# dusanerdeljan/stereo-depth

Measured on AMD Instinct MI355X. Metric: disparity maps/sec (stereo pairs/sec) at 1242x375 D=128, higher is better.
Workload: dtype f32

## Files before the change

### stereo-depth_amd/csrc/k_match_capture.h

```cpp
#pragma once
#include "k_capture_pixel0.h"
#include "k_match_fast.h"

namespace smx {

#ifndef SMX_CAP_TH
#define SMX_CAP_TH 24
#endif
constexpr int CAP_TH = SMX_CAP_TH;
constexpr int CAP_TH_SMALL = 8;

template <int TH, int PR, int PK16>
__global__ __launch_bounds__(64 * FA_WAVES, SMX_FA_OCC) void k_match_capture(MatchParams p) {
    constexpr int WGCOLS = FA_WGCOLS;
    constexpr int ND = PR - WGCOLS + 1;
    const BlockIdx3 blk = xcd_block_index();
    const int b = blk.z;
    if (p.gate == 1 && p.flags[b] == p.epoch) return;
    if (p.gate == 2 && p.flags[b] != p.epoch) return;

    extern __shared__ __attribute__((aligned(16))) unsigned short fsmem[];
    unsigned short *Lt = fsmem;
    unsigned short *Rt = fsmem + (TH + 22) * FA_PL;
    unsigned *bits = (unsigned *)(Rt + (TH + 22) * PR);
    const int BW = fast_bitwords(p.Dd);

    const int tid = threadIdx.x, lane = tid & 63, wv = tid >> 6;
    const int h = p.h, w = p.w, Dd = p.Dd;
    const int cwg0 = blk.x * FA_WAVES * FA_VALID;
    const int cw0 = cwg0 + wv * FA_VALID;
    const int wcol = wv * FA_VALID;
    const bool active = cw0 < w;
    const int x0 = blk.y * TH;
    const int col = cw0 - FA_HALO + lane;
    const float *Lp = p.Ld + (size_t)b * h * w;
    const float *Rp = p.Rd + (size_t)b * h * w;
    const float unit = p.unit;

    FastLane ln;
    ln.xch = (float *)(bits + FA_WAVES * BW) + wv * FA_XCH_FLOATS;
    ln.c255 = (unsigned)(255.0f * unit);
    ln.inv = 1.0f / (unit * unit * unit);
    ln.store_ok = active && lane >= FA_HALO && lane < FA_HALO + FA_VALID && col < w;
    ln.rows_ok = min(TH, h - x0);
    ln.plane = (size_t)p.B * h * w;
    ln.row0 = ((size_t)b * h + x0) * w;
    ln.colidx = ln.store_ok ? col : 0;
    ln.lptr = Lt + wcol + lane;

    fast_stage<(WGCOLS + 63) / 64, FA_WAVES>(Lt, FA_PL, Lp, h, w, x0 - FA_HALO, cwg0 - FA_HALO, TH + 22, WGCOLS, unit, wv, lane);
    for (int e = tid; e < FA_WAVES * BW; e += 64 * FA_WAVES) bits[e] = 0u;
    __syncthreads();

    unsigned upk[(TH + 1) / 2], vpk[(TH + 1) / 2];
#pragma unroll
    for (int o = 0; o < (TH + 1) / 2; ++o) { upk[o] = 0u; vpk[o] = 0u; }
    const bool all_needed = Dd > FA_BITWORDS * 32;
    unsigned *wbits = bits + wv * BW;
    const int left_ok = __builtin_amdgcn_update_dpp(0, ln.store_ok ? 1 : 0, 0x138, 0xf, 0xf, false);
#pragma unroll
    for (int o = 0; o < TH; ++o) {
        unsigned U = 0xffffu, V = 0xffffu;
        int u = -1, us = -1;
        bool has_succ = false;
        size_t pix = 0;
        if (ln.store_ok && o < ln.rows_ok) {
            pix = ln.row0 + (size_t)o * w + ln.colidx;
            u = (int)p.wta[pix];
            has_succ = (size_t)(x0 + o) * w + ln.colidx + 1 < (size_t)h * w;
            us = has_succ ? (int)p.wta[pix + 1] : -1;
        }
        const int lu = __builtin_amdgcn_update_dpp(-2, u, 0x138, 0xf, 0xf, false);
        const bool dup = left_ok && lu == u && us == u;
        if (ln.store_ok && o < ln.rows_ok) {
            U = (unsigned)u;
            if (has_succ) V = (unsigned)(2 * Dd - us);
            if (!all_needed && !dup) {
#pragma unroll
                for (int dl = -1; dl <= 1; ++dl) {
                    const int t = u + dl;
                    if (t <= Dd) { const int i = t == Dd ? 0 : t; atomicOr(&wbits[i], 1u << o); }
                    const int ts = us + dl;
                    if (has_succ && ts > Dd && ts <= 2 * Dd) { const int i = 2 * Dd - ts; atomicOr(&wbits[i], 1u << o); }
                }
            }
        }
        upk[o >> 1] |= U << (16 * (o & 1));
        vpk[o >> 1] |= V << (16 * (o & 1));
    }

    auto stage_right = [&](int d0, int nd) {
        __syncthreads();
        const int cbase = cwg0 - FA_HALO - (p.dmin + d0 + nd - 1);
        fast_stage<(PR + 63) / 64, FA_WAVES>(Rt, PR, Rp, h, w, x0 - FA_HALO, cbase, TH + 22, WGCOLS + nd - 1, unit, wv, lane);
        __syncthreads();
    };

    float best[TH];
    int arg[TH];
    for (int d0 = 0; d0 < Dd; d0 += ND) {
        const int nd = min(ND, Dd - d0);
        stage_right(d0, nd);
        if (active) {
            const unsigned *mybits = bits + wv * BW;
            auto march = [&](int dda, int ddb, unsigned rows) {
                const int ia = d0 + dda, ib = d0 + ddb;
                ln.rptr = Rt + wcol + lane + (nd - 1 - dda);
                fast_pass_pair<TH, PR, false, PK16, 2>(p, ln, ia, false, best, arg, Rt + wcol + lane + (nd - 1 - ddb), ib, upk,
                                                       ia == 0 ? Dd : -0x40000000, 0, 0, 0, vpk, nullptr, rows);
            };
            int pend = -1;
            unsigned pend_rows = 0u;
            SMX_FOR_EACH_NEEDED(mybits + d0, 0, nd, all_needed, lane, dd, rows, {
                if (pend < 0) { pend = dd; pend_rows = rows; }
                else { march(pend, dd, pend_rows | rows); pend = -1; }
            })
            if (pend >= 0) march(pend, pend, pend_rows);
        }
    }
    if (blk.x == 0 && blk.y == 0) {
        __syncthreads();
        capture_pixel0_body(p, b, (float *)fsmem, 64 * FA_WAVES);
    }
}

#ifdef SMX_TU_CAPTURE
template <int TH, int PR>
inline void launch_match_capture_t(int pk, const MatchParams &p, int n, hipStream_t s) {
    const dim3 grid((p.w + FA_VALID * FA_WAVES - 1) / (FA_VALID * FA_WAVES), (p.h + TH - 1) / TH, n), block(64 * FA_WAVES);
    const size_t lds = fast_lds_bytes<PR>(TH, p.Dd, false);
    if (pk == 2) hipLaunchKernelGGL((k_match_capture<TH, PR, 2>), grid, block, lds, s, p);
    else if (pk == 1) hipLaunchKernelGGL((k_match_capture<TH, PR, 1>), grid, block, lds, s, p);
    else hipLaunchKernelGGL((k_match_capture<TH, PR, 0>), grid, block, lds, s, p);
}

inline void launch_match_capture(const FastCaptureLaunch &cl, const MatchParams &p, int n, hipStream_t s) {
    if (cl.small) {
        if (!cl.wide) launch_match_capture_t<CAP_TH_SMALL, 256>(cl.pk, p, n, s);
        else launch_match_capture_t<CAP_TH_SMALL, 320>(cl.pk, p, n, s);
    } else {
        if (!cl.wide) launch_match_capture_t<CAP_TH, 256>(cl.pk, p, n, s);
        else launch_match_capture_t<CAP_TH, 320>(cl.pk, p, n, s);
    }
}

#endif

inline bool capture_applicable(int dmin, int Dd) { return dmin > 0 && dmin <= Dd && dmin + Dd < 0xfff0; }

}
```

### stereo-depth_amd/csrc/k_match_fast.h

```cpp
#pragma once
#include "smx_common.h"

namespace smx {

constexpr int FA_HALO = 11;
constexpr int FA_VALID = 64 - 2 * FA_HALO;
#ifndef SMX_FA_WAVES
#define SMX_FA_WAVES 4
#endif
constexpr int FA_WAVES = SMX_FA_WAVES;
#ifndef SMX_FA_DS_WAVES
#define SMX_FA_DS_WAVES 8
#endif
constexpr int FA_DS_WAVES = SMX_FA_DS_WAVES;
#ifndef SMX_FA_TH
#define SMX_FA_TH 24
#endif
constexpr int FA_TH = SMX_FA_TH;
#ifndef SMX_FA_TH_SMALL
#define SMX_FA_TH_SMALL 8
#endif
constexpr int FA_TH_SMALL = SMX_FA_TH_SMALL;
constexpr int FA_TH_SMALL_TALL = 12;
constexpr int FA_TH_SMALL_MID = 10;
#ifndef SMX_FA_PF
#define SMX_FA_PF 2
#endif
constexpr int FA_PF = SMX_FA_PF;
#ifndef SMX_FA_SB_PERIOD
#define SMX_FA_SB_PERIOD 2
#endif
#ifndef SMX_FA_OCC
#define SMX_FA_OCC 3
#endif
#ifndef SMX_FA_DS_OCC
#define SMX_FA_DS_OCC 4
#endif
constexpr int FA_WGCOLS = FA_VALID * FA_WAVES + 2 * FA_HALO;
#ifndef SMX_FA_WIDE_FROM
#define SMX_FA_WIDE_FROM (256 - FA_WGCOLS + 1)
#endif
constexpr int FA_WIDE_FROM = SMX_FA_WIDE_FROM;
constexpr int FA_MID_PITCH = 288;
#ifdef SMX_FA_NO_MID_PITCH
constexpr int FA_MID_UPTO = 0;
#else
constexpr int FA_MID_UPTO = FA_MID_PITCH - FA_WGCOLS + 1;
#endif
constexpr int FA_PL = (FA_VALID * FA_WAVES + 2 * FA_HALO + 7) & ~7;
constexpr int FA_BITWORDS = 64;
__host__ __device__ inline int fast_bitwords(int Dd) {
    return Dd > FA_BITWORDS * 32 ? 2 : ((Dd + 1) & ~1);
}
#define SMX_FOR_EACH_NEEDED(tbl, lo, hi, all_needed, lane, dd, rows, BODY)                                      \
    for (int g_ = (lo); g_ < (hi); g_ += 64) {                                                                  \
        const int idx_ = g_ + (lane);                                                                           \
        unsigned word_ = 0u;                                                                                    \
        if (idx_ < (hi)) word_ = (all_needed) ? ~0u : (tbl)[idx_];                                              \
        unsigned long long m_ = __ballot(word_ != 0u);                                                          \
        while (m_ != 0ull) {                                                                                    \
            const int k_ = __builtin_ctzll(m_);                                                                 \
            m_ &= m_ - 1ull;                                                                                    \
            const int dd = g_ + k_;                                                                             \
            const unsigned rows = (unsigned)__builtin_amdgcn_readlane((int)word_, k_);                          \
            BODY                                                                                                \
        }                                                                                                       \
    }

constexpr int FA_DENSE_MAX_TH = 27;
constexpr int FA_XROW = 64 + 12;
#ifndef SMX_FA_XCH_ROWS
#define SMX_FA_XCH_ROWS 2
#endif
constexpr int FA_XCH_ROWS = SMX_FA_XCH_ROWS;
constexpr int FA_XCH_FLOATS = 2 * FA_XCH_ROWS * FA_XROW;

__host__ __device__ constexpr int fast_merge_rows(int th) { return th > 8 ? (th + 1) / 2 : th; }

__host__ __device__ constexpr bool fast_prefix_exact(int th, int k_max) {
    return (long long)(th + 11) * 48195 * k_max * k_max < (1LL << 24);
}
__host__ __device__ constexpr bool fast_prefix_form(int th, int pr, bool p1only, bool dsplit, int pk16, bool argb, bool dense) {
#ifdef SMX_FA_NO_PREFIX
    return false;
#else
    if (pk16 != 2 || !fast_prefix_exact(th, 2)) return false;
    if (dsplit) return th == FA_TH_SMALL_TALL;
    (void)pr; (void)p1only; (void)argb; (void)dense;
    return true;
#endif
}

template <int PR> inline size_t fast_lds_bytes(int th, int Dd, bool dsplit = false) {
    const size_t nw = dsplit ? FA_DS_WAVES : FA_WAVES;
    return (size_t)(th + 22) * (FA_PL + PR) * sizeof(unsigned short) + nw * fast_bitwords(Dd) * sizeof(unsigned) +
           nw * FA_XCH_FLOATS * sizeof(float) + (dsplit ? nw * fast_merge_rows(th) * 64 * 2 * sizeof(float) : 0);
}

__device__ __forceinline__ float dpp_shr1(float v) {
    return __int_as_float(__builtin_amdgcn_update_dpp(0, __float_as_int(v), 0x138, 0xf, 0xf, true));
}
__device__ __forceinline__ float dpp_shl1(float v) {
    return __int_as_float(__builtin_amdgcn_update_dpp(0, __float_as_int(v), 0x130, 0xf, 0xf, true));
}
__device__ __forceinline__ unsigned dppu_sum3(unsigned v) {
    unsigned t = (unsigned)__builtin_amdgcn_update_dpp(0, (int)v, 0x138, 0xf, 0xf, true) + v;
    asm("" : "+v"(t));
    return t + (unsigned)__builtin_amdgcn_update_dpp(0, (int)v, 0x130, 0xf, 0xf, true);
}

__device__ __forceinline__ void store_u32off(float *base_uniform, unsigned off_elems, float v) {
    *(float *)((char *)base_uniform + (size_t)(off_elems * 4u)) = v;
}

__device__ __forceinline__ void atomic_or_u32off(unsigned *base_uniform, unsigned off_words, unsigned bits) {
    atomicOr((unsigned *)((char *)base_uniform + (size_t)(off_words * 4u)), bits);
}

template <int NK, int NW, bool ROUND = false>
__device__ __forceinline__ void fast_stage(unsigned short *tile, int pitch, const float *img, int h, int w,
                                           int row0, int col0, int rows, int cols, float unit, int wv, int lane) {
    int cidx[NK];
    {
        int c = wrapi(col0 + lane, w);
        const int cstep = 64 % w;
#pragma unroll
        for (int k = 0; k < NK; ++k) {
            cidx[k] = c;
            c += cstep;
            c = c >= w ? c - w : c;
        }
    }
    int ra = wrapi(row0 + wv, h);
    const int rstep = (2 * NW) % h, rhalf = NW % h;
    for (int r = wv; r < rows; r += 2 * NW) {
        const int r2 = r + NW;
        int rb = ra + rhalf;
        rb = rb >= h ? rb - h : rb;
        const float *src = img + (size_t)ra * w;
        const float *src2 = img + (size_t)(r2 < rows ? rb : ra) * w;
        float v[NK], v2[NK];
#pragma unroll
        for (int k = 0; k < NK; ++k) {
            const bool in = lane + 64 * k < cols;
            v[k] = in ? src[cidx[k]] : 0.f;
            v2[k] = in ? src2[cidx[k]] : 0.f;
        }
        unsigned short *dst = tile + r * pitch, *dst2 = tile + r2 * pitch;
#pragma unroll
        for (int k = 0; k < NK; ++k) {
            if (lane + 64 * k < cols) {
                dst[lane + 64 * k] = (unsigned short)(ROUND ? unit * v[k] + 0.5f : unit * v[k]);
                if (r2 < rows) dst2[lane + 64 * k] = (unsigned short)(ROUND ? unit * v2[k] + 0.5f : unit * v2[k]);
            }
        }
        ra += rstep;
        ra = ra >= h ? ra - h : ra;
    }
}

struct FastLane {
    const unsigned short *lptr, *rptr;
    float *xch;
    unsigned c255;
    float inv;
    bool store_ok;
    int rows_ok;
    int colidx;
    size_t row0;
    size_t plane;
    unsigned *cand;
    unsigned cand_off_a, cand_off_b;
    unsigned long long cand_mask_a, cand_mask_b;
    unsigned cand_rstride;
    int x0;
};

typedef float f32x2 __attribute__((ext_vector_type(2)));
typedef __attribute__((address_space(3))) f32x2 fa_lds_f32x2;

__device__ __forceinline__ void argb_update(int kbyte, int &word, float m, float best, int dsel) {
    if (kbyte == 0)
        asm volatile("v_cmp_gt_f32 vcc, %1, %2\n\tv_cndmask_b32_sdwa %0, %0, %3, vcc dst_sel:BYTE_0 dst_unused:UNUSED_PRESERVE src0_sel:BYTE_0 src1_sel:BYTE_0"
                     : "+v"(word) : "v"(m), "v"(best), "v"(dsel) : "vcc");
    else if (kbyte == 1)
        asm volatile("v_cmp_gt_f32 vcc, %1, %2\n\tv_cndmask_b32_sdwa %0, %0, %3, vcc dst_sel:BYTE_1 dst_unused:UNUSED_PRESERVE src0_sel:BYTE_1 src1_sel:BYTE_0"
                     : "+v"(word) : "v"(m), "v"(best), "v"(dsel) : "vcc");
    else if (kbyte == 2)
        asm volatile("v_cmp_gt_f32 vcc, %1, %2\n\tv_cndmask_b32_sdwa %0, %0, %3, vcc dst_sel:BYTE_2 dst_unused:UNUSED_PRESERVE src0_sel:BYTE_2 src1_sel:BYTE_0"
                     : "+v"(word) : "v"(m), "v"(best), "v"(dsel) : "vcc");
    else
        asm volatile("v_cmp_gt_f32 vcc, %1, %2\n\tv_cndmask_b32_sdwa %0, %0, %3, vcc dst_sel:BYTE_3 dst_unused:UNUSED_PRESERVE src0_sel:BYTE_3 src1_sel:BYTE_0"
                     : "+v"(word) : "v"(m), "v"(best), "v"(dsel) : "vcc");
}

template <int TH, int PR, bool P1ONLY, int PK16, int MODE = 0, bool ARGB = false, bool DENSE = false, bool PREFIX = false>
__device__ __forceinline__ void fast_pass_pair(const MatchParams &p, const FastLane &ln, int d,
                                               bool valid_b, float (&best)[TH], int (&arg)[TH],
                                               const unsigned short *rptr_b_in = nullptr, int db = 0,
                                               const unsigned *argpk = nullptr, int am_a = 0, int ap_a = 0,
                                               int am_b = 0, int ap_b = 0, const unsigned *vpk = nullptr,
                                               unsigned *hits = nullptr, unsigned rowmask = ~0u,
                                               float *dmb = nullptr, float *dma = nullptr, float *dcp = nullptr,
                                               float *dfirst = nullptr) {
    static_assert(!PREFIX || (PK16 == 2 && fast_prefix_exact(TH, 2)), "prefix form: K <= 2 and every prefix below 2^24");
    constexpr int NQ = TH + 20;
    constexpr int Q9 = PREFIX ? 11 : 12, Q21 = PREFIX ? 17 : 18;
    f32x2 s1 = {0.f, 0.f}, s2 = {0.f, 0.f};
    unsigned k1 = 0u, k2 = 0u;
    const unsigned c255pk = ln.c255 * 0x10001u;
    f32x2 r3[NQ], r9[NQ], r21[NQ];
    unsigned lv[TH + 22], rva[TH + 22], rvb[TH + 22];
    f32x2 vs = {0.f, 0.f}, cs = {0.f, 0.f}, hs = {0.f, 0.f};
    f32x2 t_m3 = {0.f, 0.f}, t_p3 = {0.f, 0.f}, u_m6 = {0.f, 0.f}, u_p6 = {0.f, 0.f};
    const int lane_ = threadIdx.x & 63;
#ifdef SMX_FA_ARGMAX2
    int dva = d, dvb = d + 1;
    if (ARGB && MODE == 0) asm volatile("" : "+v"(dva), "+v"(dvb));
#endif
    const unsigned short *rptr_b = (MODE == 0 || MODE == 3) ? ln.rptr - (valid_b ? 1 : 0) : rptr_b_in;
    (void)db;
#pragma unroll
    for (int rr_ = 0; rr_ < TH + 22 + FA_PF; ++rr_) {
        if (rr_ < TH + 22) {
            lv[rr_] = ln.lptr[rr_ * FA_PL];
            rva[rr_] = ln.rptr[rr_ * PR];
            rvb[rr_] = rptr_b[rr_ * PR];
        }
        if (rr_ >= FA_PF) {
            const int r = rr_ - FA_PF;
            f32x2 s0 = {0.f, 0.f};
            unsigned k0 = 0u;
            if (PK16) {
                const unsigned sa = __builtin_amdgcn_sad_u16(lv[r], rva[r], 0u);
                const unsigned sb = __builtin_amdgcn_sad_u16(lv[r], rvb[r], 0u);
                k0 = c255pk - ((sb << 16) | sa);
            } else {
                s0.x = (float)(ln.c255 - __builtin_amdgcn_sad_u16(lv[r], rva[r], 0u));
                s0.y = (float)(ln.c255 - __builtin_amdgcn_sad_u16(lv[r], rvb[r], 0u));
            }
            if (r >= 2) {
                const int q = r - 2;
                f32x2 x3;
                if (PK16 == 2) {
                    const unsigned v3 = (k2 + k1) + k0;
                    const unsigned cv = dppu_sum3(v3);
                    const unsigned y3 = dppu_sum3(cv);
                    x3.x = (float)(y3 & 0xffffu);
                    x3.y = (float)(y3 >> 16);
                } else if (PK16 == 1) {
                    const unsigned v3 = (k2 + k1) + k0;
                    const unsigned cvp = dppu_sum3(v3);
                    f32x2 cv;
                    cv.x = (float)(cvp & 0xffffu);
                    cv.y = (float)(cvp >> 16);
                    x3.x = (dpp_shr1(cv.x) + cv.x) + dpp_shl1(cv.x);
                    x3.y = (dpp_shr1(cv.y) + cv.y) + dpp_shl1(cv.y);
                } else {
                    const f32x2 v3 = (s2 + s1) + s0;
                    f32x2 cv;
                    cv.x = (dpp_shr1(v3.x) + v3.x) + dpp_shl1(v3.x);
                    cv.y = (dpp_shr1(v3.y) + v3.y) + dpp_shl1(v3.y);
                    x3.x = (dpp_shr1(cv.x) + cv.x) + dpp_shl1(cv.x);
                    x3.y = (dpp_shr1(cv.y) + cv.y) + dpp_shl1(cv.y);
                }
                if (PREFIX && q > 0) r3[q] = r3[q > 0 ? q - 1 : 0] + x3;
                else r3[q] = x3;
                if (q >= Q9) r9[q - 6] = (t_m3 + r3[q - 6]) + t_p3;
                if (q >= Q21) r21[q - 9] = (u_m6 + u_p6) + r3[q - 9];
#ifdef SMX_EXP_NOXCH
                if (q >= Q9 - 1 && q + 1 < NQ) { t_m3 = r3[q - 5]; t_p3 = r3[q - 4]; }
                if (q >= Q21 - 1 && q + 1 < NQ) { u_m6 = r9[q - 8]; u_p6 = r9[q - 7]; }
#else
                if (q >= Q9 - 1 && q + 1 < NQ) {
                    f32x2 *x3b = (f32x2 *)ln.xch + lane_;
                    x3b[6] = r3[q - 5];
                    __builtin_amdgcn_wave_barrier();
                    {
                        const volatile fa_lds_f32x2 *xr = (const volatile fa_lds_f32x2 *)x3b;
                        t_m3 = xr[3]; t_p3 = xr[9];
                    }
                }
                if (q >= Q21 - 1 && q + 1 < NQ) {
                    f32x2 *x9b = (f32x2 *)(ln.xch + (FA_XCH_ROWS > 1 ? 2 * FA_XROW : 0)) + lane_;
                    x9b[6] = r9[q - 8];
                    __builtin_amdgcn_wave_barrier();
                    {
                        const volatile fa_lds_f32x2 *xr = (const volatile fa_lds_f32x2 *)x9b;
                        u_m6 = xr[0]; u_p6 = xr[12];
                    }
                }
#endif
                if (PREFIX) {
                    if (q >= 20) {
                        vs = q >= 21 ? r3[q] - r3[q - 21] : r3[q];
                        cs = r9[q - 6] - r9[q - 15];
                        hs = r21[q - 9] - r21[q - 12];
                    }
                } else {
                    vs += r3[q];
                    if (q >= 21) vs -= r3[q - 21];
                    if (q >= 12) cs += r9[q - 6];
                    if (q >= 21) cs -= r9[q - 15];
                    if (q >= 18) hs += r21[q - 9];
                    if (q >= 21) hs -= r21[q - 12];
                }
                if (q >= 20) {
                    const int o = q - 20;
                    const f32x2 agg = (hs * vs) * cs;
                    if ((MODE == 1 || MODE == 2) && !((rowmask >> o) & 1u)) {
                    } else if (MODE == 2) {
                        unsigned upk_w = argpk[o >> 1], vpk_w = vpk[o >> 1];
                        asm volatile("" : "+v"(upk_w), "+v"(vpk_w));
                        const unsigned U = (upk_w >> (16 * (o & 1))) & 0xffffu;
                        const unsigned V = (vpk_w >> (16 * (o & 1))) & 0xffffu;
                        int ci = ln.colidx;
                        asm volatile("" : "+v"(ci));
                        const unsigned off = (unsigned)(o * p.w + ci);
                        float *cp = p.costs + ln.row0;
                        auto put = [&](unsigned dl1, unsigned o2, float v) {
                            const size_t pl = dl1 == 1u ? 0 : (dl1 == 2u ? 1 : 2);
                            cp[pl * ln.plane + o2] = v * ln.inv;
                        };
                        const unsigned a1 = (unsigned)(d + 1) - U, a2 = V + 1u - (unsigned)d, a3 = (unsigned)(am_a + 1) - U;
                        const unsigned b1 = (unsigned)(db + 1) - U, b2 = V + 1u - (unsigned)db;
                        if (a1 < 3u) put(a1, off, agg.x);
                        if (a2 < 3u) put(a2, off + 1u, agg.x);
                        if (a3 < 3u) put(a3, off, agg.x);
                        if (b1 < 3u) put(b1, off, agg.y);
                        if (b2 < 3u) put(b2, off + 1u, agg.y);
                    } else if (MODE == 4) {
                        best[o] = __builtin_fmaxf(__builtin_fmaxf(best[o], agg.x), agg.y);
                    } else if (MODE == 3) {
                        const bool okp = ln.store_ok && o < ln.rows_ok;
                        const unsigned long long ma = __ballot(okp && agg.x >= best[o]);
                        const unsigned long long mb = __ballot(okp && agg.y >= best[o]);
                        const unsigned tr = (unsigned)(((ln.x0 + o) >> 4) - (ln.x0 >> 4));
                        const unsigned h4 = ((ma & ln.cand_mask_a) != 0ull ? 1u : 0u) | ((ma & ln.cand_mask_b) != 0ull ? 2u : 0u) |
                                            ((mb & ln.cand_mask_a) != 0ull ? 4u : 0u) | ((mb & ln.cand_mask_b) != 0ull ? 8u : 0u);
                        *hits |= h4 << (4u * tr);
                    } else if (MODE == 1) {
                        const int a = (int)((argpk[o >> 1] >> (16 * (o & 1))) & 0xffffu);
                        int ci = ln.colidx;
                        asm volatile("" : "+v"(ci));
                        const unsigned off = (unsigned)(o * p.w + ci);
                        const bool xa = a == am_a, xb = a == ap_a;
                        if (xa || a == am_b) store_u32off(p.costs + ln.row0 + ln.plane, off, (xa ? agg.x : agg.y) * ln.inv);
                        if (xb || a == ap_b) store_u32off(p.costs + ln.row0 + 2 * ln.plane, off, (xb ? agg.x : agg.y) * ln.inv);
                    } else {
                        if constexpr (DENSE) {
                            const float after_d = valid_b ? agg.y : __builtin_nanf("");
                            dma[o] = (dma[o] != dma[o]) ? agg.x : dma[o];
                            const bool ca = (agg.x > best[o]) | (d == 0);
                            const float b1 = __builtin_fmaxf(best[o], agg.x);
                            dmb[o] = ca ? dcp[o] : dmb[o];
                            dma[o] = ca ? after_d : dma[o];
                            const bool cb = agg.y > b1;
                            dmb[o] = cb ? agg.x : dmb[o];
                            dma[o] = cb ? __builtin_nanf("") : dma[o];
                            dcp[o] = agg.y;
                            if (dfirst) dfirst[o] = agg.x;
                        }
#if !defined(SMX_FA_ARGMAX2)
                        const float m = __builtin_fmaxf(__builtin_fmaxf(best[o], agg.x), agg.y);
                        const int dsel = (agg.x == m) ? d : d + 1;
#ifndef SMX_EXP_NOARG
                        if (ARGB) {
                            argb_update(o & 3, arg[o >> 2], m, best[o], dsel);
                        } else {
                            const bool changed = m > best[o];
                            arg[o] = changed ? dsel : arg[o];
                        }
#else
                        (void)dsel;
#endif
                        best[o] = m;
#else
                        if (ARGB) {
                            argb_update(o & 3, arg[o >> 2], agg.x, best[o], dva);
                            best[o] = __builtin_fmaxf(best[o], agg.x);
                            argb_update(o & 3, arg[o >> 2], agg.y, best[o], dvb);
                            best[o] = __builtin_fmaxf(best[o], agg.y);
                        } else {
                            const float m = __builtin_fmaxf(__builtin_fmaxf(best[o], agg.x), agg.y);
                            const int dsel = (agg.x == m) ? d : d + 1;
                            arg[o] = m > best[o] ? dsel : arg[o];
                            best[o] = m;
                        }
#endif
                    }
                }
            }
            s2 = s1;
            s1 = s0;
            k2 = k1;
            k1 = k0;
        }
        if ((rr_ % SMX_FA_SB_PERIOD) == SMX_FA_SB_PERIOD - 1)
            __builtin_amdgcn_sched_barrier(0);
    }
}

constexpr int FA_STAT_WG_STRIDE_DS = 16;
template <bool DSPLIT>
__device__ __forceinline__ void fast_stats_report(const MatchParams &p, int b, int wg_lin, int wv, int marches, bool window) {
    if (!p.fast_stats || b % p.fast_stride != 0) return;
    if (DSPLIT && wg_lin % FA_STAT_WG_STRIDE_DS != 0) return;
    const bool win = window && (!DSPLIT || wv == 0);
    const unsigned long long v = ((unsigned long long)(unsigned)marches << 24) | (win ? 1ull : 0ull);
    if (v != 0ull) (void)__hip_atomic_fetch_add(p.fast_stats, v, __ATOMIC_RELAXED, __HIP_MEMORY_SCOPE_AGENT);
}

template <int TU, int NH, int PR, int PK16, bool PREFIX, class StageRight>
__device__ __forceinline__ void fast_stacked_tail(const MatchParams &p, const BlockIdx3 &blk, const FastLane &ln, const float (&best)[TU * NH],
                                                  const int (&argb)[TU * NH], const unsigned short *Rt, unsigned *bits, int wcol, int x0,
                                                  bool active, StageRight &&stage_right) {
    constexpr int ND = PR - FA_WGCOLS + 1;
    const int lane = threadIdx.x & 63, wv = threadIdx.x >> 6;
    const int h = p.h, w = p.w, Dd = p.Dd, BW = fast_bitwords(Dd);
    const bool all_needed = Dd > FA_BITWORDS * 32;
    unsigned *wbits = bits + wv * BW;
#pragma unroll
    for (int hh = 0; hh < NH; ++hh) {
        float bh[TU];
        int ah[TU];
#pragma unroll
        for (int o = 0; o < TU; ++o) {
            bh[o] = best[hh * TU + o];
            ah[o] = (argb[(hh * TU + o) >> 2] >> (8 * ((hh * TU + o) & 3))) & 0xff;
        }
        FastLane lh = ln;
        lh.lptr = ln.lptr + hh * TU * FA_PL;
        lh.row0 = ln.row0 + (size_t)(hh * TU) * w;
        lh.rows_ok = max(0, min(TU, h - x0 - hh * TU));
        const unsigned short *Rh = Rt + hh * TU * PR;
        unsigned dup_left = 0u;
#ifndef SMX_FA_NO_DEDUP
        if (!all_needed) {
#pragma unroll
            for (int o = 0; o < TU; ++o) {
                const int la = __builtin_amdgcn_update_dpp(-1, ah[o], 0x138, 0xf, 0xf, false);
                dup_left |= (la == ah[o] ? 1u : 0u) << o;
            }
            const int left_ok = __builtin_amdgcn_update_dpp(0, lh.store_ok ? 1 : 0, 0x138, 0xf, 0xf, false);
            if (!left_ok) dup_left = 0u;
        }
#endif
        if (lh.store_ok) {
#pragma unroll
            for (int o = 0; o < TU; ++o) {
                if (o < lh.rows_ok) {
                    const unsigned off = (unsigned)(o * w + lh.colidx);
                    store_u32off(p.wta + lh.row0, off, (float)ah[o] + (float)p.dmin);
                    const bool nv = !(bh[o] > SMX_FLT_MIN);
                    store_u32off(p.costs + lh.row0, off, nv ? 0.0f : bh[o] * lh.inv);
                    if (!all_needed && !((dup_left >> o) & 1u)) {
                        const int dn = (ah[o] + 1 == Dd) ? 0 : ah[o] + 1;
                        const int dp = (ah[o] == 0) ? Dd - 1 : ah[o] - 1;
                        atomicOr(&wbits[dn], 1u << o);
                        atomicOr(&wbits[dp], 1u << o);
                    }
                }
            }
        }
        int marches2 = 0;
        unsigned argpk[(TU + 1) / 2];
#pragma unroll
        for (int o = 0; o < (TU + 1) / 2; ++o) argpk[o] = 0u;
#pragma unroll
        for (int o = 0; o < TU; ++o)
            argpk[o >> 1] |= ((lh.store_ok && o < lh.rows_ok) ? (unsigned)ah[o] : 0xffffu) << (16 * (o & 1));
        for (int d0 = 0; d0 < Dd; d0 += ND) {
            const int nd = min(ND, Dd - d0);
            if (Dd > ND) stage_right(d0, nd);
            else __syncthreads();
            if (active) {
                auto march = [&](int dda, int ddb, unsigned rows) {
                    const int da = d0 + dda, db = d0 + ddb;
                    ++marches2;
                    lh.rptr = Rh + wcol + lane + (nd - 1 - dda);
                    fast_pass_pair<TU, PR, false, PK16, 1, false, false, PREFIX>(p, lh, da, false, bh, ah, Rh + wcol + lane + (nd - 1 - ddb), db, argpk,
                                                           da == 0 ? Dd - 1 : da - 1, da + 1 == Dd ? 0 : da + 1,
                                                           db == 0 ? Dd - 1 : db - 1, db + 1 == Dd ? 0 : db + 1, nullptr, nullptr, rows);
                };
                int pend = -1;
                unsigned pend_rows = 0u;
                SMX_FOR_EACH_NEEDED(wbits + d0, 0, nd, all_needed, lane, dd, rows, {
                    if (pend < 0) { pend = dd; pend_rows = rows; }
                    else { march(pend, dd, pend_rows | rows); pend = -1; }
                })
                if (pend >= 0) march(pend, pend, pend_rows);
            }
        }
        if (lane == 0) fast_stats_report<false>(p, blk.z, (int)(blk.x + gridDim.x * blk.y), wv, marches2, active && lh.rows_ok > 0);
        if (hh + 1 < NH)
            for (int e = lane; e < BW; e += 64) wbits[e] = 0u;
    }
}

template <int TH, int PR, bool P1ONLY, bool DSPLIT, int PK16, bool ARGB = false, bool DENSE = false>
__device__ __forceinline__ void match_fast_body(const MatchParams &p, const BlockIdx3 &blk) {
    static_assert(!DENSE || !P1ONLY, "the dense form is a pass 1 with neighbours: min_disparity = 0");
    static_assert(!DENSE || !DSPLIT || !ARGB, "latency shape: one register per winner");
    constexpr int NW = DSPLIT ? FA_DS_WAVES : FA_WAVES;
    constexpr int WGCOLS = DSPLIT ? 64 : FA_WGCOLS;
    constexpr int ND = PR - WGCOLS + 1;
    constexpr int NH = TH > 32 ? 2 : 1;
    constexpr int TU = TH / NH;
    constexpr bool PREFIX = fast_prefix_form(TH, PR, P1ONLY, DSPLIT, PK16, ARGB, DENSE);
    static_assert(NH == 1 || (TH == 2 * TU && TU <= 32 && ARGB && !DSPLIT && !DENSE && !P1ONLY),
                  "stacked bands: two unit bands, byte-packed winners, throughput shape, sparse form");
    const int b = blk.z;

    extern __shared__ __attribute__((aligned(16))) unsigned short fsmem[];
    unsigned short *Lt = fsmem;
    unsigned short *Rt = fsmem + (TH + 22) * FA_PL;
    unsigned *bits = (unsigned *)(Rt + (TH + 22) * PR);
    const int BW = fast_bitwords(p.Dd);

    const int tid = threadIdx.x;
    const int lane = tid & 63;
    const int wv = tid >> 6;
    const int h = p.h, w = p.w, Dd = p.Dd;
    const int cwg0 = blk.x * (DSPLIT ? 1 : FA_WAVES) * FA_VALID;
    const int cw0 = cwg0 + (DSPLIT ? 0 : wv * FA_VALID);
    const int wcol = DSPLIT ? 0 : wv * FA_VALID;
    const bool active = cw0 < w;
    const int x0 = blk.y * TH;
    const int col = cw0 - FA_HALO + lane;
    const float *Lp = p.Ld + (size_t)b * h * w;
    const float *Rp = p.Rd + (size_t)b * h * w;
    const float unit = p.unit;

    FastLane ln;
    ln.xch = (float *)(bits + NW * BW) + wv * FA_XCH_FLOATS;
    ln.c255 = (unsigned)(255.0f * unit);
    ln.inv = 1.0f / (unit * unit * unit);
    ln.store_ok = active && lane >= FA_HALO && lane < FA_HALO + FA_VALID && col < w;
    ln.rows_ok = min(TH, h - x0);
    ln.plane = (size_t)p.B * h * w;
    ln.row0 = ((size_t)b * h + x0) * w;
    ln.colidx = ln.store_ok ? col : 0;
    ln.lptr = Lt + wcol + lane;

    float best[TH];
    int arg[TH];
#pragma unroll
    for (int o = 0; o < TH; ++o) { best[o] = SMX_FLT_MIN; arg[o] = 0; }
    float dmb[DENSE ? TH : 1], dma[DENSE ? TH : 1], dcp[DENSE ? TH : 1];
    float dfirst[DENSE && DSPLIT ? TH : 1];
#pragma unroll
    for (int o = 0; o < (DENSE ? TH : 1); ++o) { dmb[o] = 0.f; dma[o] = 0.f; dcp[o] = 0.f; }
#pragma unroll
    for (int o = 0; o < (DENSE && DSPLIT ? TH : 1); ++o) dfirst[o] = 0.f;

    fast_stage<(WGCOLS + 63) / 64, NW>(Lt, FA_PL, Lp, h, w, x0 - FA_HALO, cwg0 - FA_HALO, TH + 22, WGCOLS, unit, wv, lane);
    for (int e = tid; e < NW * BW; e += 64 * NW) bits[e] = 0u;

    auto stage_right = [&](int d0, int nd) {
        __syncthreads();
        const int cbase = cwg0 - FA_HALO - (p.dmin + d0 + nd - 1);
        fast_stage<(PR + 63) / 64, NW>(Rt, PR, Rp, h, w, x0 - FA_HALO, cbase, TH + 22, WGCOLS + nd - 1, unit, wv, lane);
        __syncthreads();
    };

    for (int d0 = 0; d0 < Dd; d0 += ND) {
        const int nd = min(ND, Dd - d0);
        stage_right(d0, nd);
        if (active) {
            const int q4 = ((nd + 2 * NW - 1) / (2 * NW)) * 2;
            const int dd_lo = DSPLIT ? min(nd, wv * q4) : 0;
            const int dd_hi = DSPLIT ? min(nd, dd_lo + q4) : nd;
            for (int dd = dd_lo; dd < dd_hi; dd += 2) {
                ln.rptr = Rt + wcol + lane + (nd - 1 - dd);
                if constexpr (DENSE)
                    fast_pass_pair<TH, PR, P1ONLY, PK16, 0, ARGB, true, PREFIX>(p, ln, d0 + dd, dd + 1 < dd_hi, best, arg, nullptr, 0, nullptr,
                                                                         0, 0, 0, 0, nullptr, nullptr, ~0u, dmb, dma, dcp,
                                                                         DSPLIT && dd == dd_lo ? dfirst : nullptr);
                else
                    fast_pass_pair<TH, PR, P1ONLY, PK16, 0, ARGB, false, PREFIX>(p, ln, d0 + dd, dd + 1 < dd_hi, best, arg);
            }
        }
    }
    if constexpr (NH > 1) {
        fast_stacked_tail<TU, NH, PR, PK16, PREFIX>(p, blk, ln, best, arg, Rt, bits, wcol, x0, active, stage_right);
        return;
    }
    if (ARGB) {
        int packed[(TH + 3) / 4];
#pragma unroll
        for (int o = 0; o < (TH + 3) / 4; ++o) packed[o] = arg[o];
#pragma unroll
        for (int o = 0; o < TH; ++o) arg[o] = (packed[o >> 2] >> (8 * (o & 3))) & 0xff;
    }
    float *mrg = (float *)(bits + NW * BW) + NW * FA_XCH_FLOATS;
    if constexpr (DSPLIT && DENSE) {
        constexpr int MR = fast_merge_rows(TH), R2 = (NW * MR * 2) / (NW * 6);
        static_assert(R2 >= 1 && R2 <= NW, "merge buffer: at least one row of six values per wave");
        const int q4 = ((Dd + 2 * NW - 1) / (2 * NW)) * 2;
        const int nk = (Dd + q4 - 1) / q4;
#pragma unroll 1
        for (int o0 = 0; o0 < TH; o0 += R2) {
            __syncthreads();
#pragma unroll
            for (int o = 0; o < TH; ++o) {
                if (o >= o0 && o < o0 + R2) {
                    float *q = mrg + ((size_t)(wv * R2 + (o - o0)) * 64 + lane) * 6;
                    q[0] = best[o]; q[1] = __int_as_float(arg[o]); q[2] = dmb[o]; q[3] = dma[o]; q[4] = dfirst[o]; q[5] = dcp[o];
                }
            }
            __syncthreads();
            const int j = wv;
            if (j < R2 && o0 + j < ln.rows_ok && ln.store_ok) {
                auto M = [&](int k, int f) { return mrg[((size_t)(k * R2 + j) * 64 + lane) * 6 + f]; };
                float bb = SMX_FLT_MIN;
                int aa = 0, kw = 0;
                for (int k = 0; k < nk; ++k) {
                    const float bk = M(k, 0);
                    const bool g = bk > bb;
                    aa = g ? __float_as_int(M(k, 1)) : aa;
                    kw = g ? k : kw;
                    bb = g ? bk : bb;
                }
                float mb = M(kw, 2), ma = M(kw, 3);
                if (aa == kw * q4) mb = M(kw > 0 ? kw - 1 : nk - 1, 5);
                if (ma != ma) ma = M(kw + 1 < nk ? kw + 1 : 0, 4);
                const unsigned off = (unsigned)((o0 + j) * w + ln.colidx);
                store_u32off(p.wta + ln.row0, off, (float)aa + (float)p.dmin);
                store_u32off(p.costs + ln.row0, off, !(bb > SMX_FLT_MIN) ? 0.0f : bb * ln.inv);
                store_u32off(p.costs + ln.row0 + ln.plane, off, ma * ln.inv);
                store_u32off(p.costs + ln.row0 + 2 * ln.plane, off, mb * ln.inv);
            }
        }
        return;
    }
    if (DSPLIT) {
        constexpr int MR = fast_merge_rows(TH);
#pragma unroll
        for (int o0 = 0; o0 < TH; o0 += MR) {
            __syncthreads();
#pragma unroll
            for (int o = o0; o < o0 + MR && o < TH; ++o) {
                mrg[((wv * MR + (o - o0)) * 64 + lane) * 2] = best[o];
                mrg[((wv * MR + (o - o0)) * 64 + lane) * 2 + 1] = __int_as_float(arg[o]);
            }
            __syncthreads();
#pragma unroll
            for (int o = o0; o < o0 + MR && o < TH; ++o) {
                float bb = SMX_FLT_MIN;
                int aa = 0;
#pragma unroll
                for (int k = 0; k < NW; ++k) {
                    const float bk = mrg[((k * MR + (o - o0)) * 64 + lane) * 2];
                    const int ak = __float_as_int(mrg[((k * MR + (o - o0)) * 64 + lane) * 2 + 1]);
                    const bool g = bk > bb;
                    aa = g ? ak : aa;
                    bb = g ? bk : bb;
                }
                best[o] = bb;
                arg[o] = aa;
            }
        }
    }

    const bool all_needed = Dd > FA_BITWORDS * 32;
    unsigned dup_left = 0u;
#ifndef SMX_FA_NO_DEDUP
    if (!DENSE && !P1ONLY && !all_needed) {
#pragma unroll
        for (int o = 0; o < TH; ++o) {
            const int la = __builtin_amdgcn_update_dpp(-1, arg[o], 0x138, 0xf, 0xf, false);
            dup_left |= (la == arg[o] ? 1u : 0u) << o;
        }
        const int left_ok = __builtin_amdgcn_update_dpp(0, ln.store_ok ? 1 : 0, 0x138, 0xf, 0xf, false);
        if (!left_ok) dup_left = 0u;
    }
#endif
    if (ln.store_ok) {
        unsigned *wbits = bits + (DSPLIT ? 0 : wv) * BW;
#pragma unroll
        for (int o = 0; o < TH; ++o) {
            if (o < ln.rows_ok && (!DSPLIT || o % NW == wv)) {
                const unsigned off = (unsigned)(o * w + ln.colidx);
                store_u32off(p.wta + ln.row0, off, (float)arg[o] + (float)p.dmin);
                const bool nv = !(best[o] > SMX_FLT_MIN);
                store_u32off(p.costs + ln.row0, off, nv ? 0.0f : best[o] * ln.inv);
                if constexpr (DENSE) {
                    store_u32off(p.costs + ln.row0 + 2 * ln.plane, off, (arg[o] == 0 ? dcp[o] : dmb[o]) * ln.inv);
                    if (dma[o] != dma[o]) {
                        if (!all_needed) atomicOr(&wbits[0], 1u << o);
                    } else {
                        store_u32off(p.costs + ln.row0 + ln.plane, off, dma[o] * ln.inv);
                    }
                } else
                if (!P1ONLY && !all_needed && !((dup_left >> o) & 1u)) {
                    const int dn = (arg[o] + 1 == Dd) ? 0 : arg[o] + 1;
                    const int dp = (arg[o] == 0) ? Dd - 1 : arg[o] - 1;
                    atomicOr(&wbits[dn], 1u << o);
                    atomicOr(&wbits[dp], 1u << o);
                }
            }
        }
    }
    if (P1ONLY) return;

    int marches2 = 0;
    unsigned argpk[(TH + 1) / 2];
#pragma unroll
    for (int o = 0; o < (TH + 1) / 2; ++o) argpk[o] = 0u;
#pragma unroll
    for (int o = 0; o < TH; ++o)
        argpk[o >> 1] |= ((ln.store_ok && o < ln.rows_ok) ? (unsigned)arg[o] : 0xffffu) << (16 * (o & 1));
    for (int d0 = 0; d0 < (DENSE ? 1 : Dd); d0 += ND) {
        const int nd = min(ND, Dd - d0);
        if (Dd > ND) stage_right(d0, nd);
        else __syncthreads();
        if (active) {
            const unsigned *mybits = bits + (DSPLIT ? 0 : wv) * BW;
            const int q4 = ((nd + 2 * NW - 1) / (2 * NW)) * 2;
            const int dd_lo = DSPLIT ? min(nd, wv * q4) : 0;
            const int dd_hi = DSPLIT ? min(nd, dd_lo + q4) : nd;
            auto march = [&](int dda, int ddb, unsigned rows) {
                const int da = d0 + dda, db = d0 + ddb;
                ++marches2;
                ln.rptr = Rt + wcol + lane + (nd - 1 - dda);
                fast_pass_pair<TH, PR, false, PK16, 1, false, false, PREFIX>(p, ln, da, false, best, arg, Rt + wcol + lane + (nd - 1 - ddb), db, argpk,
                                                       da == 0 ? Dd - 1 : da - 1, da + 1 == Dd ? 0 : da + 1,
                                                       db == 0 ? Dd - 1 : db - 1, db + 1 == Dd ? 0 : db + 1, nullptr, nullptr, rows);
            };
            int pend = -1;
            unsigned pend_rows = 0u;
#ifndef SMX_EXP_NOPASS2
            if constexpr (DSPLIT) {
                (void)dd_lo; (void)dd_hi;
                int seen = 0;
                SMX_FOR_EACH_NEEDED(mybits + d0, 0, nd, all_needed, lane, dd, rows, {
                    const bool mine = (seen >> 1) % NW == wv;
                    ++seen;
                    if (mine) {
                        if (pend < 0) { pend = dd; pend_rows = rows; }
                        else { march(pend, dd, pend_rows | rows); pend = -1; }
                    }
                })
            } else {
                SMX_FOR_EACH_NEEDED(mybits + d0, dd_lo, dd_hi, all_needed, lane, dd, rows, {
                    if (pend < 0) { pend = dd; pend_rows = rows; }
                    else { march(pend, dd, pend_rows | rows); pend = -1; }
                })
            }
#endif
            if (pend >= 0) march(pend, pend, pend_rows);
        }
    }
    if constexpr (!DENSE) {
        if (lane == 0) fast_stats_report<DSPLIT>(p, b, (int)(blk.x + gridDim.x * blk.y), wv, marches2, active);
    }
}

#ifdef SMX_FA_NUM_VGPR
#define SMX_FA_VGPR_ATTR __attribute__((amdgpu_num_vgpr(SMX_FA_NUM_VGPR)))
#else
#define SMX_FA_VGPR_ATTR
#endif
template <int TH, int PR, bool P1ONLY, bool DSPLIT, int PK16, bool ARGB, bool DENSE = false>
__global__ __launch_bounds__(64 * (DSPLIT ? FA_DS_WAVES : FA_WAVES), DENSE ? 2 : (DSPLIT ? (TH >= FA_TH_SMALL_TALL ? 2 : SMX_FA_DS_OCC) : SMX_FA_OCC)) SMX_FA_VGPR_ATTR void k_match_fast(MatchParams p) {
    const BlockIdx3 blk = xcd_block_index();
    if ((p.gate == 1 && p.flags[blk.z] == p.epoch) || (p.gate == 2 && p.flags[blk.z] != p.epoch)) {
        return;
    }
    match_fast_body<TH, PR, P1ONLY, DSPLIT, PK16, ARGB, DENSE>(p, blk);
}

inline int fast_pk(int unit) { return unit <= 4 ? 2 : (unit <= 16 ? 1 : 0); }
inline bool fast_small_wide(int Dd) { return Dd > 256 - 64 + 1; }

template <int TH, int PR, bool P1ONLY, bool DSPLIT, bool ARGB, bool DENSE>
inline void launch_match_fast_k(int pk, dim3 grid, dim3 block, size_t lds, const MatchParams &p, hipStream_t s) {
    if (pk == 2) hipLaunchKernelGGL((k_match_fast<TH, PR, P1ONLY, DSPLIT, 2, ARGB, DENSE>), grid, block, lds, s, p);
    else if (pk == 1) hipLaunchKernelGGL((k_match_fast<TH, PR, P1ONLY, DSPLIT, 1, ARGB, DENSE>), grid, block, lds, s, p);
    else hipLaunchKernelGGL((k_match_fast<TH, PR, P1ONLY, DSPLIT, 0, ARGB, DENSE>), grid, block, lds, s, p);
}

template <int TH, int PR, bool DSPLIT, bool ARGB>
inline void launch_match_fast_a(const FastLaunch &fl, const MatchParams &p, int n, hipStream_t s) {
    const int win_per_wg = DSPLIT ? 1 : FA_WAVES;
    const dim3 grid((p.w + FA_VALID * win_per_wg - 1) / (FA_VALID * win_per_wg), (p.h + TH - 1) / TH, n);
    const size_t lds = fast_lds_bytes<PR>(TH, p.Dd, DSPLIT);
    const dim3 block(64 * (DSPLIT ? FA_DS_WAVES : FA_WAVES));
#ifdef SMX_FA_FORCE_TH
    if (lds > 64 * 1024) {
        (void)hipFuncSetAttribute(reinterpret_cast<const void *>(&k_match_fast<TH, PR, false, DSPLIT, 2, ARGB>),
                                  hipFuncAttributeMaxDynamicSharedMemorySize, (int)lds);
    }
#endif
    if (fl.form == FAST_DENSE_SMALL) {
        if constexpr (DSPLIT && TH == FA_TH_SMALL_TALL) launch_match_fast_k<TH, PR, false, true, false, true>(fl.pk, grid, block, lds, p, s);
    } else if (fl.form == FAST_DENSE) {
        if constexpr (!DSPLIT && ARGB && TH <= FA_DENSE_MAX_TH) launch_match_fast_k<TH, PR, false, false, ARGB, true>(fl.pk, grid, block, lds, p, s);
    } else if (fl.form == FAST_PASS1_ONLY) {
        launch_match_fast_k<TH, PR, true, DSPLIT, ARGB, false>(fl.pk, grid, block, lds, p, s);
    } else {
        launch_match_fast_k<TH, PR, false, DSPLIT, ARGB, false>(fl.pk, grid, block, lds, p, s);
    }
}

template <int TH, int PR, bool DSPLIT>
inline void launch_match_fast_t(const FastLaunch &fl, const MatchParams &p, int n, hipStream_t s) {
    if constexpr (DSPLIT) {
        launch_match_fast_a<TH, PR, true, false>(fl, p, n, s);
    } else if constexpr (PR == 256 || PR == FA_MID_PITCH) {
        launch_match_fast_a<TH, PR, false, true>(fl, p, n, s);
    } else {
        if (fl.argb) launch_match_fast_a<TH, PR, false, true>(fl, p, n, s);
        else launch_match_fast_a<TH, PR, false, false>(fl, p, n, s);
    }
}

__host__ __device__ constexpr int fast_tall_pitch(int Dd) { return Dd <= FA_WIDE_FROM ? 256 : (Dd <= FA_MID_UPTO ? FA_MID_PITCH : 320); }

template <int TH>
inline void launch_match_fast_tall(const FastLaunch &fl, const MatchParams &p, int n, hipStream_t s) {
    if (fl.pitch == 256) launch_match_fast_t<TH, 256, false>(fl, p, n, s);
    else if (fl.pitch == FA_MID_PITCH) launch_match_fast_t<TH, FA_MID_PITCH, false>(fl, p, n, s);
    else launch_match_fast_t<TH, 320, false>(fl, p, n, s);
}

constexpr int FA_STACK = 2;
constexpr int FA_STACK_TH = FA_STACK * FA_TH;
template <int PR> inline bool fast_stack_fits(int Dd) {
    const size_t granule = 1280, lds = fast_lds_bytes<PR>(FA_STACK_TH, Dd);
    return 2 * ((lds + granule - 1) / granule * granule) <= 160 * 1024;
}
inline bool fast_stack_instantiated(int pitch, int Dd) { return pitch == 256 && fast_stack_fits<256>(Dd); }

template <int PR>
inline void launch_match_fast_stacked(const FastLaunch &fl, const MatchParams &p, int n, hipStream_t s) {
    const dim3 grid((p.w + FA_VALID * FA_WAVES - 1) / (FA_VALID * FA_WAVES), (p.h + FA_STACK_TH - 1) / FA_STACK_TH, n);
    const size_t lds = fast_lds_bytes<PR>(FA_STACK_TH, p.Dd);
    const dim3 block(64 * FA_WAVES);
    if (fl.pk == 2) hipLaunchKernelGGL((k_match_fast<FA_STACK_TH, PR, false, false, 2, true, false>), grid, block, lds, s, p);
    else if (fl.pk == 1) hipLaunchKernelGGL((k_match_fast<FA_STACK_TH, PR, false, false, 1, true, false>), grid, block, lds, s, p);
    else hipLaunchKernelGGL((k_match_fast<FA_STACK_TH, PR, false, false, 0, true, false>), grid, block, lds, s, p);
}
template <int PR>
inline hipError_t fast_stacked_raise_lds_caps() {
    const int cap = (int)fast_lds_bytes<PR>(FA_STACK_TH, PR - FA_WGCOLS + 1);
    const void *kernels[3] = {reinterpret_cast<const void *>(&k_match_fast<FA_STACK_TH, PR, false, false, 2, true, false>),
                              reinterpret_cast<const void *>(&k_match_fast<FA_STACK_TH, PR, false, false, 1, true, false>),
                              reinterpret_cast<const void *>(&k_match_fast<FA_STACK_TH, PR, false, false, 0, true, false>)};
    for (const void *k : kernels)
        if (hipError_t e = hipFuncSetAttribute(k, hipFuncAttributeMaxDynamicSharedMemorySize, cap); e != hipSuccess) return e;
    return hipSuccess;
}

struct FastPlan {
    bool small;
    int th;
    bool wide;
    int stack = 1;
};

inline FastPlan match_fast_plan(const MatchParams &p, int n, int cus, int stack_opt = -1) {
    FastPlan pl{};
    const long wgs_tall = (long)((p.w + FA_VALID * FA_WAVES - 1) / (FA_VALID * FA_WAVES)) * ((p.h + FA_TH - 1) / FA_TH) * n;
    pl.small = 8 * wgs_tall < (p.on_lanes ? 8L : 13L) * cus;
    if (pl.small) {
        pl.th = FA_TH_SMALL;
        pl.wide = fast_small_wide(p.Dd);
        const long windows = (long)((p.w + FA_VALID - 1) / FA_VALID) * n;
        const long wg_small = windows * ((p.h + FA_TH_SMALL - 1) / FA_TH_SMALL), wg_tall = windows * ((p.h + FA_TH_SMALL_TALL - 1) / FA_TH_SMALL_TALL);
        if (wg_small > cus && wg_tall <= cus) {
            pl.th = FA_TH_SMALL_TALL;
#ifndef SMX_FA_NO_MID
#ifdef SMX_FA_MID_P1
        } else {
#else
        } else if (!p.pass1_only) {
#endif
            const long wg_mid = windows * ((p.h + FA_TH_SMALL_MID - 1) / FA_TH_SMALL_MID), slots = 2L * cus;
            const long r_small = (wg_small + slots - 1) / slots, r_mid = (wg_mid + slots - 1) / slots;
            if (r_mid * (FA_TH_SMALL_MID + 22) < r_small * (FA_TH_SMALL + 22)) pl.th = FA_TH_SMALL_MID;
#endif
        }
        return pl;
    }
    pl.wide = p.Dd > FA_WIDE_FROM;
    const int cand[3] = {24, 27, 32};
    int best = 24;
    long best_rows = -1;
    for (int th : cand) {
        const int pr = fast_tall_pitch(p.Dd);
        const size_t lds = pr == 256 ? fast_lds_bytes<256>(th, p.Dd) : (pr == FA_MID_PITCH ? fast_lds_bytes<FA_MID_PITCH>(th, p.Dd) : fast_lds_bytes<320>(th, p.Dd));
        const size_t granule = 1280;
        const bool three_per_cu = 3 * ((lds + granule - 1) / granule * granule) <= 160 * 1024;
        const long rows = (long)((p.h + th - 1) / th) * (th + 22) * (th == 32 ? 106 : 100) * (three_per_cu ? 100 : 130);
        if (best_rows < 0 || rows < best_rows) { best_rows = rows; best = th; }
    }
    pl.th = best;
#ifdef SMX_FA_FORCE_TH
    pl.th = SMX_FA_FORCE_TH;
#endif
    if (stack_opt != 0 && !p.dense && !p.pass1_only && fast_stack_instantiated(fast_tall_pitch(p.Dd), p.Dd)) {
        const long rows_stack = (long)((p.h + FA_STACK_TH - 1) / FA_STACK_TH) * (FA_STACK_TH + 22);
        if (stack_opt == 1 || (p.on_lanes && rows_stack < (long)((p.h + pl.th - 1) / pl.th) * (pl.th + 22))) {
            pl.th = FA_TH;
            pl.stack = FA_STACK;
        }
    }
    return pl;
}

}
```

### stereo-depth_amd/csrc/k_prologue.h

```cpp
#pragma once
#include "smx_common.h"

namespace smx {

enum { IN_GRAY_F32 = 0, IN_RGB_F32 = 1, IN_GRAY_U8 = 2, IN_RGB_U8 = 3 };

template <int MODE>
__device__ __forceinline__ float load_gray(const void *img, size_t plane, size_t idx, int fp_conv) {
    if (MODE == IN_RGB_F32 || MODE == IN_RGB_U8) {
        float r, g, b;
        if (MODE == IN_RGB_F32) {
            const float *p = (const float *)img;
            r = p[idx]; g = p[plane + idx]; b = p[2 * plane + idx];
        } else {
            const uint8_t *p = (const uint8_t *)img;
            r = (float)p[idx]; g = (float)p[plane + idx]; b = (float)p[2 * plane + idx];
        }
        if (fp_conv != 0) return sum3_products(0.2989f, r, 0.5870f, g, 0.1140f, b, fp_conv);
        float R = 0.2989f * r;
        float G = 0.5870f * g;
        float B = 0.1140f * b;
        return (R + G) + B;
    } else if (MODE == IN_GRAY_U8) {
        return (float)((const uint8_t *)img)[idx];
    } else {
        return ((const float *)img)[idx];
    }
}

template <int MODE>
__global__ __launch_bounds__(256) void k_prologue(const void *left, const void *right,
                                                  float *gray_l, float *gray_r,
                                                  float *down_l, float *down_r, int *flags,
                                                  uint8_t *g8_l, uint8_t *g8_r, int *flags2,
                                                  int H, int W, int K, int h, int w, int grid_capable,
                                                  int pitch8, int padl, int padr, int epoch,
                                                  int gpitch, int gpadl, int fp_conv) {
    const int y = blockIdx.x * 64 + threadIdx.x;
    const int x = blockIdx.y * 4 + threadIdx.y;
    const int b = blockIdx.z;
    const size_t plane = (size_t)H * W;
    const size_t in_elems = (MODE == IN_RGB_F32 || MODE == IN_RGB_U8) ? 3 * plane : plane;
    const size_t in_bytes = (MODE == IN_GRAY_U8 || MODE == IN_RGB_U8) ? 1 : 4;
    bool bad = (grid_capable == 0);
    bool bad8 = false;
    if (x < h && y < w) {
        const float area = (float)(K * K);
        const float unit = area;
#pragma unroll
        for (int side = 0; side < 2; ++side) {
            const char *base = (const char *)(side ? right : left) + (size_t)b * in_elems * in_bytes;
            float *gout = (side ? gray_r : gray_l);
            uint8_t *g8 = (side ? g8_r : g8_l);
            float sum = 0.0f;
            uint32_t pk = 0u;
            for (int i = 0; i < K; ++i) {
                int xi = x * K + i;
                const bool xin = xi < H;
                if (!xin) xi = H - 1;
                for (int j = 0; j < K; ++j) {
                    int yj = y * K + j;
                    const bool yin = yj < W;
                    if (!yin) yj = W - 1;
                    const size_t idx = (size_t)xi * W + yj;
                    const float v = load_gray<MODE>(base, plane, idx, fp_conv);
                    if (MODE == IN_RGB_F32) bad8 = bad8 || !(v >= 0.0f && v <= 255.0f);
                    if (MODE != IN_GRAY_F32 && xin && yin) {
                        float *grow = gout + ((size_t)b * H + xi) * gpitch + gpadl;
                        grow[yj] = v;
                        if (gpadl > 0) {
                            if (yj >= W - gpadl) grow[yj - W] = v;
                            if (yj < padr) grow[W + yj] = v;
                        }
                    }
                    if ((MODE == IN_GRAY_F32 || MODE == IN_GRAY_U8) && pitch8 > 0 && xin && yin) {
                        if (MODE == IN_GRAY_F32) bad8 = bad8 || !(v == rintf(v) && v >= 0.0f && v <= 255.0f);
                        uint8_t *row8 = g8 + ((size_t)b * H + xi) * pitch8;
                        if (K == 2) {
                            if (j == 0) pk = (uint32_t)(uint8_t)v;
                            else if (yj & 1) *(uint16_t *)(row8 + padl + yj - 1) = (uint16_t)(pk | ((uint32_t)(uint8_t)v << 8));
                            if (j == 0 && yj + 1 >= W) row8[padl + yj] = (uint8_t)v;
                        } else {
                            row8[padl + yj] = (uint8_t)v;
                        }
                        if (yj >= W - padl) row8[yj - (W - padl)] = (uint8_t)v;
                        if (yj < padr) row8[padl + W + yj] = (uint8_t)v;
                    }
                    sum += v;
                }
            }
            const float pooled = grid_capable ? sum * (1.0f / area) : sum / area;
            (side ? down_r : down_l)[((size_t)b * h + x) * w + y] = pooled;
            const float s = pooled * unit;
            bad = bad || !(s == rintf(s) && pooled >= 0.0f && pooled <= 255.0f);
        }
    }
    const unsigned long long m = __ballot(bad);
    if (m != 0ull && (int)threadIdx.x == __ffsll((long long)m) - 1) flags[b] = epoch;
    if (MODE == IN_GRAY_F32 || MODE == IN_RGB_F32) {
        const unsigned long long m8 = __ballot(bad8);
        if (m8 != 0ull && (int)threadIdx.x == __ffsll((long long)m8) - 1) flags2[b] = epoch;
    }
}

template <int MODE>
__global__ __launch_bounds__(256) void k_prologue_k2(const void *left, const void *right,
                                                     float *gray_l, float *gray_r,
                                                     float *down_l, float *down_r, int *flags,
                                                     uint8_t *g8_l, uint8_t *g8_r, int *flags2,
                                                     int H, int W, int h, int w,
                                                     int pitch8, int padl, int padr, int epoch,
                                                     int gpitch, int gpadl) {
    const int yp = (blockIdx.x * 64 + threadIdx.x) * 2;
    const int x = blockIdx.y * 4 + threadIdx.y;
    const int b = blockIdx.z;
    const size_t plane = (size_t)H * W;
    bool bad = false, bad8 = false;
    if (x < h && yp < w) {
        const int Y0 = yp * 2;
        const int ncol = min(4, W - Y0);
        const int x0 = x * 2, x1 = min(x * 2 + 1, H - 1);
        const bool row1_in = x * 2 + 1 < H;
#pragma unroll
        for (int side = 0; side < 2; ++side) {
            const void *img = side ? right : left;
            float v0[4], v1[4];
            if (MODE == IN_GRAY_F32) {
                const float *p0 = (const float *)img + (size_t)b * plane + (size_t)x0 * W + Y0;
                const float *p1 = (const float *)img + (size_t)b * plane + (size_t)x1 * W + Y0;
                if (ncol == 4) {
                    __builtin_memcpy(v0, __builtin_assume_aligned(p0, 4), 16);
                    __builtin_memcpy(v1, __builtin_assume_aligned(p1, 4), 16);
                } else {
                    v0[0] = p0[0]; v0[1] = p0[1]; v1[0] = p1[0]; v1[1] = p1[1];
                    v0[2] = v0[3] = v1[2] = v1[3] = 0.f;
                }
            } else {
                const uint8_t *p0 = (const uint8_t *)img + (size_t)b * plane + (size_t)x0 * W + Y0;
                const uint8_t *p1 = (const uint8_t *)img + (size_t)b * plane + (size_t)x1 * W + Y0;
#pragma unroll
                for (int j = 0; j < 4; ++j) {
                    v0[j] = (j < ncol) ? (float)p0[j] : 0.f;
                    v1[j] = (j < ncol) ? (float)p1[j] : 0.f;
                }
                float *g = (side ? gray_r : gray_l) + (size_t)b * H * gpitch + gpadl;
#pragma unroll
                for (int j = 0; j < 4; ++j) {
                    if (j < ncol) {
                        g[(size_t)x0 * gpitch + Y0 + j] = v0[j];
                        if (row1_in) g[(size_t)(x0 + 1) * gpitch + Y0 + j] = v1[j];
                    }
                }
            }
            float pooled[2];
            pooled[0] = (((v0[0] + v0[1]) + v1[0]) + v1[1]) * 0.25f;
            pooled[1] = (((v0[2] + v0[3]) + v1[2]) + v1[3]) * 0.25f;
            float *dn = (side ? down_r : down_l) + ((size_t)b * h + x) * w + yp;
            dn[0] = pooled[0];
            if (ncol == 4) dn[1] = pooled[1];
#pragma unroll
            for (int k = 0; k < 2; ++k) {
                if (k == 0 || ncol == 4) {
                    const float s4 = pooled[k] * 4.0f;
                    bad = bad || !(s4 == rintf(s4) && pooled[k] >= 0.0f && pooled[k] <= 255.0f);
                }
            }
            if (pitch8 > 0) {
                uint8_t *g8 = (side ? g8_r : g8_l);
                uint32_t w0 = 0u, w1 = 0u;
#pragma unroll
                for (int j = 0; j < 4; ++j) {
                    if (j < ncol) {
                        if (MODE == IN_GRAY_F32)
                            bad8 = bad8 || !(v0[j] == rintf(v0[j]) && v0[j] >= 0.f && v0[j] <= 255.f) ||
                                   (row1_in && !(v1[j] == rintf(v1[j]) && v1[j] >= 0.f && v1[j] <= 255.f));
                        w0 |= (uint32_t)(uint8_t)v0[j] << (8 * j);
                        w1 |= (uint32_t)(uint8_t)v1[j] << (8 * j);
                    }
                }
                uint8_t *r0 = g8 + ((size_t)b * H + x0) * pitch8, *r1 = r0 + pitch8;
                if (ncol == 4) {
                    *(uint32_t *)(r0 + padl + Y0) = w0;
                    if (row1_in) *(uint32_t *)(r1 + padl + Y0) = w1;
                } else {
                    *(uint16_t *)(r0 + padl + Y0) = (uint16_t)w0;
                    if (row1_in) *(uint16_t *)(r1 + padl + Y0) = (uint16_t)w1;
                }
                if (Y0 + 3 >= W - padl || Y0 < padr) {
#pragma unroll
                    for (int j = 0; j < 4; ++j) {
                        const int yj = Y0 + j;
                        if (j < ncol) {
                            const uint8_t a = (uint8_t)(w0 >> (8 * j)), c = (uint8_t)(w1 >> (8 * j));
                            if (yj >= W - padl) { r0[yj - (W - padl)] = a; if (row1_in) r1[yj - (W - padl)] = c; }
                            if (yj < padr) { r0[padl + W + yj] = a; if (row1_in) r1[padl + W + yj] = c; }
                        }
                    }
                }
            }
        }
    }
    const unsigned long long m = __ballot(bad);
    if (m != 0ull && (int)threadIdx.x == __ffsll((long long)m) - 1) flags[b] = epoch;
    if (MODE == IN_GRAY_F32) {
        const unsigned long long m8 = __ballot(bad8);
        if (m8 != 0ull && (int)threadIdx.x == __ffsll((long long)m8) - 1) flags2[b] = epoch;
    }
}

template <int MODE>
__global__ __launch_bounds__(256) void k_prologue_k4(const void *left, const void *right,
                                                     float *gray_l, float *gray_r,
                                                     float *down_l, float *down_r, int *flags,
                                                     uint8_t *g8_l, uint8_t *g8_r, int *flags2,
                                                     int H, int W, int h, int w,
                                                     int pitch8, int padl, int padr, int epoch,
                                                     int gpitch, int gpadl, int fp_conv) {
    constexpr bool RGB = MODE == IN_RGB_F32 || MODE == IN_RGB_U8;
    constexpr bool U8 = MODE == IN_GRAY_U8 || MODE == IN_RGB_U8;
    const int y = blockIdx.x * 64 + threadIdx.x;
    const int x = blockIdx.y * 4 + threadIdx.y;
    const int b = blockIdx.z;
    const size_t plane = (size_t)H * W;
    const size_t pair_elems = RGB ? 3 * plane : plane;
    bool bad = false, bad8 = false;
    if (x < h && y < w) {
        const int Y0 = y * 4;
#pragma unroll
        for (int side = 0; side < 2; ++side) {
            const void *img = side ? right : left;
            float v[4][4];
            bool rin[4];
#pragma unroll
            for (int i = 0; i < 4; ++i) {
                rin[i] = x * 4 + i < H;
                const int xi = rin[i] ? x * 4 + i : H - 1;
                const size_t at = (size_t)b * pair_elems + (size_t)xi * W + Y0;
                float c[RGB ? 3 : 1][4];
#pragma unroll
                for (int ch = 0; ch < (RGB ? 3 : 1); ++ch) {
                    if (!U8) {
                        const float *p = (const float *)img + at + ch * plane;
                        __builtin_memcpy(c[ch], __builtin_assume_aligned(p, 4), 16);
                    } else {
                        const uint8_t *p = (const uint8_t *)img + at + ch * plane;
                        uint32_t wd;
                        __builtin_memcpy(&wd, __builtin_assume_aligned(p, 4), 4);
#pragma unroll
                        for (int j = 0; j < 4; ++j) c[ch][j] = (float)((wd >> (8 * j)) & 0xffu);
                    }
                }
#pragma unroll
                for (int j = 0; j < 4; ++j) {
                    if (RGB) {
                        if (fp_conv != 0) {
                            v[i][j] = sum3_products(0.2989f, c[0][j], 0.5870f, c[RGB ? 1 : 0][j], 0.1140f, c[RGB ? 2 : 0][j], fp_conv);
                        } else {
                            const float R = 0.2989f * c[0][j];
                            const float G = 0.5870f * c[RGB ? 1 : 0][j];
                            const float B = 0.1140f * c[RGB ? 2 : 0][j];
                            v[i][j] = (R + G) + B;
                        }
                        if (MODE == IN_RGB_F32) bad8 = bad8 || !(v[i][j] >= 0.0f && v[i][j] <= 255.0f);
                    } else {
                        v[i][j] = c[0][j];
                    }
                }
                if (MODE != IN_GRAY_F32 && rin[i]) {
                    float *grow = (side ? gray_r : gray_l) + ((size_t)b * H + xi) * gpitch + gpadl;
                    __builtin_memcpy(__builtin_assume_aligned(grow + Y0, 16), v[i], 16);
                    if (RGB && gpadl > 0 && (Y0 + 3 >= W - gpadl || Y0 < padr)) {
#pragma unroll
                        for (int j = 0; j < 4; ++j) {
                            const int yj = Y0 + j;
                            if (yj >= W - gpadl) grow[yj - W] = v[i][j];
                            if (yj < padr) grow[W + yj] = v[i][j];
                        }
                    }
                }
            }
            float sum = 0.0f;
#pragma unroll
            for (int i = 0; i < 4; ++i) {
#pragma unroll
                for (int j = 0; j < 4; ++j) sum += v[i][j];
            }
            const float pooled = sum * 0.0625f;
            (side ? down_r : down_l)[((size_t)b * h + x) * w + y] = pooled;
            const float s16 = pooled * 16.0f;
            bad = bad || !(s16 == rintf(s16) && pooled >= 0.0f && pooled <= 255.0f);
            if (!RGB && pitch8 > 0) {
                uint8_t *g8 = (side ? g8_r : g8_l);
#pragma unroll
                for (int i = 0; i < 4; ++i) {
                    if (!rin[i]) continue;
                    uint32_t wd = 0u;
#pragma unroll
                    for (int j = 0; j < 4; ++j) {
                        if (MODE == IN_GRAY_F32) bad8 = bad8 || !(v[i][j] == rintf(v[i][j]) && v[i][j] >= 0.f && v[i][j] <= 255.f);
                        wd |= (uint32_t)(uint8_t)v[i][j] << (8 * j);
                    }
                    uint8_t *r8 = g8 + ((size_t)b * H + x * 4 + i) * pitch8;
                    *(uint32_t *)(r8 + padl + Y0) = wd;
                    if (Y0 + 3 >= W - padl || Y0 < padr) {
#pragma unroll
                        for (int j = 0; j < 4; ++j) {
                            const int yj = Y0 + j;
                            const uint8_t a = (uint8_t)(wd >> (8 * j));
                            if (yj >= W - padl) r8[yj - (W - padl)] = a;
                            if (yj < padr) r8[padl + W + yj] = a;
                        }
                    }
                }
            }
        }
    }
    const unsigned long long m = __ballot(bad);
    if (m != 0ull && (int)threadIdx.x == __ffsll((long long)m) - 1) flags[b] = epoch;
    if (MODE == IN_GRAY_F32 || MODE == IN_RGB_F32) {
        const unsigned long long m8 = __ballot(bad8);
        if (m8 != 0ull && (int)threadIdx.x == __ffsll((long long)m8) - 1) flags2[b] = epoch;
    }
}

}
```

### stereo-depth_amd/csrc/smx_common.h

```cpp
#pragma once

#include <hip/hip_runtime.h>
#include <stdint.h>

#define SMX_FLT_MIN 1.17549435e-38f

namespace smx {

__device__ __forceinline__ int wrapi(int g, int n) {
    g %= n;
    return g < 0 ? g + n : g;
}

__device__ __forceinline__ int pad_index_ref(int index, int n) {
    if (index >= 0 && index < n) return index;
    if (index < 0) return n + index;
    if (index == n) return 0;
    return n - index;
}

__device__ __forceinline__ float sum3_products(float a1, float b1, float a2, float b2, float a3, float b3, int conv) {
    float inner;
    if (conv == 1 || conv == 4) inner = __builtin_fmaf(a1, b1, a2 * b2);
    else if (conv == 2 || conv == 5) inner = __builtin_fmaf(a2, b2, a1 * b1);
    else inner = a1 * b1 + a2 * b2;
    if (conv >= 1 && conv <= 3) return __builtin_fmaf(a3, b3, inner);
    return inner + a3 * b3;
}

__device__ __forceinline__ float quadratic_peak_conv(float x1, float y1, float x2, float y2,
                                                     float x3, float y3, int conv) {
    float denominator = (x1 - x2) * (x2 - x3) * (x1 - x3);
    float min_value;
    if (y1 > y2) {
        min_value = (y1 > y3) ? x1 : x3;
    } else {
        min_value = (y2 > y3) ? x2 : x3;
    }
    if (denominator != 0) {
        const float a = sum3_products(x3, y2 - y1, x2, y1 - y3, x1, y3 - y2, conv);
        const float b = sum3_products(x1 * x1, y2 - y3, x3 * x3, y1 - y2, x2 * x2, y3 - y1, conv);
        if (a < 0) {
            min_value = -b / (2 * a);
        }
    }
    return min_value;
}

__device__ __forceinline__ float quadratic_peak(float x1, float y1, float x2, float y2,
                                                float x3, float y3) {
    float denominator = (x1 - x2) * (x2 - x3) * (x1 - x3);
    float min_value;
    if (y1 > y2) {
        min_value = (y1 > y3) ? x1 : x3;
    } else {
        min_value = (y2 > y3) ? x2 : x3;
    }
    if (denominator != 0) {
        float a = x3 * (y2 - y1) + x2 * (y1 - y3) + x1 * (y3 - y2);
        float b = x1 * x1 * (y2 - y3) + x3 * x3 * (y1 - y2) + x2 * x2 * (y3 - y1);
        if (a < 0) {
            min_value = -b / (2 * a);
        }
    }
    return min_value;
}

__device__ __forceinline__ float quadratic_peak_unit(float x1, float y1, float y2, float y3, int conv) {
    const float x2 = x1 + 1.0f, x3 = x1 - 1.0f;
    float min_value;
    if (y1 > y2) {
        min_value = (y1 > y3) ? x1 : x3;
    } else {
        min_value = (y2 > y3) ? x2 : x3;
    }
    float a, b;
    if (conv == 0) {
        a = x3 * (y2 - y1) + x2 * (y1 - y3) + x1 * (y3 - y2);
        b = x1 * x1 * (y2 - y3) + x3 * x3 * (y1 - y2) + x2 * x2 * (y3 - y1);
    } else {
        a = sum3_products(x3, y2 - y1, x2, y1 - y3, x1, y3 - y2, conv);
        b = sum3_products(x1 * x1, y2 - y3, x3 * x3, y1 - y2, x2 * x2, y3 - y1, conv);
    }
    if (a < 0) min_value = -b / (2 * a);
    return min_value;
}

struct WtaState {
    float best, m0, mb, ma, cprev, first;
    int arg;
    bool pend;
    __device__ __forceinline__ void init() {
        best = SMX_FLT_MIN; m0 = 0.f; mb = 0.f; ma = 0.f; cprev = 0.f; first = 0.f;
        arg = 0; pend = false;
    }
    __device__ __forceinline__ void step(int d, float c) {
        if (d == 0) { first = c; m0 = c; pend = true; }
        else if (pend) { ma = c; pend = false; }
        if (c > best) {
            best = c; arg = d; m0 = c; mb = cprev; pend = true;
        }
        cprev = c;
    }
    __device__ __forceinline__ void finish() {
        if (arg == 0) mb = cprev;
        if (pend) ma = first;
    }
};

struct BlockIdx3 { unsigned x, y, z; };
__device__ __forceinline__ BlockIdx3 xcd_block_index() {
    const unsigned nx = gridDim.x, ny = gridDim.y, nz = gridDim.z;
    const unsigned total = nx * ny * nz, per = total >> 3;
    const unsigned lin = blockIdx.x + nx * (blockIdx.y + ny * blockIdx.z);
    const unsigned t = lin < (per << 3) ? (lin & 7u) * per + (lin >> 3) : lin;
    BlockIdx3 b;
    b.x = t % nx;
    const unsigned q = t / nx;
    b.y = q % ny;
    b.z = q / ny;
    return b;
}

struct WtaSlice {
    float best, m0, mb, ma, cprev, first;
    int arg;
    bool pend;
    __device__ __forceinline__ void init(int lo) {
        best = SMX_FLT_MIN; m0 = 0.f; mb = 0.f; ma = 0.f; cprev = 0.f; first = 0.f;
        arg = lo; pend = false;
    }
    __device__ __forceinline__ void step(int d, int lo, float c) {
        if (d == lo) { first = c; m0 = c; pend = true; }
        else if (pend) { ma = c; pend = false; }
        if (c > best) {
            best = c; arg = d; m0 = c; mb = cprev; pend = true;
        }
        cprev = c;
    }
};

enum { SMX_SL_BEST = 0, SMX_SL_ARG, SMX_SL_M0, SMX_SL_MA, SMX_SL_MB, SMX_SL_FIRST, SMX_SL_LAST, SMX_SL_PEND, SMX_SLICE_WORDS };

struct MatchParams {
    const float *Ld, *Rd;
    float *wta;
    float *costs;
    float *vol;
    const int *flags;
    int epoch;
    int B, h, w, dmin, Dd;
    int rn, rs, rm, rl;
    int gate;
    int nd_chunk;
    float unit;
    int nsplit;
    int pairs;
    float *slices;
    int pass1_only;
    int dense;
    int dense_small;
    unsigned long long *fast_stats;
    int fast_stride;
    int on_lanes;
    unsigned *tickets;
};

enum GateFlag { GATE_GRID_FLAG = 0, GATE_RANGE_FLAG };
enum ExactKernel { EXACT_GENERIC = 0, EXACT_GENERIC_VOLUME, EXACT_TILED };
struct ExactLaunch {
    int kernel = EXACT_GENERIC;
    int split = 1;
    int rows_per_thread = 4;
    int nd_chunk = 0;
    size_t lds_bytes = 0;
    size_t slice_floats = 0;
    int gate = 0, gate_flag = GATE_GRID_FLAG;
};
struct ExactCaptureLaunch { int split = 1, rows_per_thread = 4, nd_chunk = 0; size_t lds_bytes = 0; int gate = 0; };
enum FastForm { FAST_SPARSE = 0, FAST_PASS1_ONLY, FAST_DENSE, FAST_DENSE_SMALL, FAST_FORMS };
struct FastLaunch {
    int th = 0;
    bool small = false;
    int pitch = 0;
    int pk = 0;
    bool argb = false;
    int form = FAST_SPARSE;
    int gate = 0;
    int stack = 1;
};
struct FastCaptureLaunch { bool small = false, wide = false; int pk = 0, gate = 0; };
struct AutoLaunch { int th = 0; bool wide = false; int pk = 0, nsplit = 1, nd_chunk = 0; size_t lds_bytes = 0; };
struct FilterLaunch { int th = 0; bool wide = false; int pk = 0; };
enum PrologueKernel { PROLOGUE_GENERIC = 0, PROLOGUE_K2, PROLOGUE_K4 };
struct PrologueLaunch { int in_mode = 0, kernel = PROLOGUE_GENERIC; };
enum RefineKind {
    REFINE_FLOAT = 0,
    REFINE_INT = 1,
    REFINE_INT_V = 2,
    REFINE_AUTO = 3,
    REFINE_AUTO_V = 4
};
struct RefineLaunch {
    int kind = REFINE_FLOAT;
    int kt = 0;
    bool apron = false;
    bool sad_exact = true;
};
enum FillKernel { FILL_4 = 0, FILL_POW2, FILL_GENERIC };
struct FillLaunch {
    int kernel = FILL_GENERIC, K = 1;
    int px = 8;
    int log2k = 0;
};

}
```

### stereo-depth_amd/csrc/smx_engine.hip

```cpp
#include <hip/hip_runtime.h>

#include <cstdarg>
#include <cstdio>
#include <cstdlib>
#include <cstring>
#include <mutex>
#include <new>
#include <string>
#include <vector>

#include "../../include/stereo_mi355x.h"
#include "k_fill.h"
#include "k_match_exact.h"
#include "k_match_exact2.h"
#include "k_match_auto.h"
#include "k_match_filter.h"
#include "k_match_capture.h"
#include "k_match_fast.h"
#include "k_prologue.h"
#include "k_refine.h"
#include "smx_common.h"
#include "smx_launch.h"
#include "smx_plan.h"
#include "smx_route.h"
#include "smx_status.h"

namespace {

using smx::check_lr_scalars, smx::DeviceGuard, smx::fail, smx::ranges_overlap;

int compute_dims(const smx_config *c, smx_dims *d) {
    if (c->height == 0 || c->width == 0 || c->downscale_factor == 0)
        return fail(SMX_ERR_INVALID_CONFIG, "height, width and downscale_factor must be positive");
    if (c->height > (1u << 15) || c->width > (1u << 15) || c->downscale_factor > 64)
        return fail(SMX_ERR_INVALID_CONFIG, "image larger than 32768 or downscale_factor > 64");
    if (c->min_disparity < 0 || c->max_disparity < c->min_disparity)
        return fail(SMX_ERR_INVALID_CONFIG, "need 0 <= min_disparity <= max_disparity");
    if (c->small_mbm_radius < 0 || c->mid_mbm_radius < 0 || c->large_mbm_radius < 0)
        return fail(SMX_ERR_INVALID_CONFIG, "block-matching radii must be non-negative");
    if (c->small_mbm_radius > c->large_mbm_radius || c->mid_mbm_radius > c->large_mbm_radius)
        return fail(SMX_ERR_INVALID_CONFIG,
                    "small_mbm_radius and mid_mbm_radius must not exceed large_mbm_radius "
                    "(the reference's shared tile has a halo of large_mbm_radius)");
    if (c->ncc_patch_radius > 16 || c->sad_patch_radius > 32 || c->large_mbm_radius > 32)
        return fail(SMX_ERR_INVALID_CONFIG, "patch radius out of the supported range");
    const int K = (int)c->downscale_factor;
    d->H = (int)c->height;
    d->W = (int)c->width;
    d->K = K;
    d->h = (d->H + K - 1) / K;
    d->w = (d->W + K - 1) / K;
    d->dmin = c->min_disparity / K;
    d->dmax = c->max_disparity / K;
    d->Dd = d->dmax - d->dmin + 1;
    return SMX_OK;
}

}

using smx::HostHints, smx::ContentSwitch, smx::LaneLedger;

struct smx_engine {
    smx_config cfg;
    smx_dims dm;
    int B;
    smx::EngineFacts facts;
    float *gray_l = nullptr, *gray_r = nullptr;
    float *down_l = nullptr, *down_r = nullptr;
    float *wta = nullptr, *refined = nullptr;
    float *costs = nullptr;
    float *vol = nullptr;
    float *slices = nullptr;
    unsigned *tickets = nullptr;
    int *flags = nullptr;
    int epoch = 0;
    uint8_t *gray8_l = nullptr, *gray8_r = nullptr;
    unsigned *cand = nullptr;
    struct LastCall {
        smx::CallFacts call;
        smx::RangePlan plan;
        int first = 0;
    } last_call;
    int next_small_lane = 0;
    const float *last_gray_l = nullptr, *last_gray_r = nullptr;
    int last_gpitch = 0;
    bool last_gray_owned = false;
    size_t last_gplane = 0;
    int opt_lane_priority = 1;
    bool opt_debug_hints = false;
    HostHints *hints = nullptr, *hints_dev = nullptr;
    smx::RouteState route;
    unsigned *stats_dev = nullptr;
    unsigned long long *fast_stats_dev = nullptr;
    std::vector<hipEvent_t> prof_events;
    std::vector<unsigned char> prof_used;
    int prof_calls = 0, prof_max = 0;
    bool prof_on = false;
    static constexpr int LANES = 2;
    hipStream_t lane_stream[LANES] = {};
    hipEvent_t ev_join[LANES] = {};
    hipEvent_t ev_cross[LANES] = {};
    hipEvent_t ev_caller = nullptr;
    bool caller_tail_live = false;
    bool caller_calls_unrecorded = false;
    hipStream_t last_caller_stream = nullptr;
    LaneLedger ledger;
    bool detached_pending = false;
    int overlap_min = 0;
    void *lr_in_l = nullptr, *lr_in_r = nullptr;
    size_t lr_pair_bytes = 0;
    float *lr_raw = nullptr;
};
static_assert(ContentSwitch::LANES == smx_engine::LANES && LaneLedger::LANES == smx_engine::LANES, "one report word and one ledger entry per stream lane");

namespace {

void free_events(smx_engine *e) {
    for (hipEvent_t ev : e->prof_events) (void)hipEventDestroy(ev);
    e->prof_events.clear();
    e->prof_used.clear();
    e->prof_calls = e->prof_max = 0;
    e->prof_on = false;
}

void free_buffers(smx_engine *e) {
    void *ptrs[] = {e->gray_l, e->gray_r, e->down_l, e->down_r, e->wta,     e->refined,  e->costs,
                    e->vol,    e->flags,  e->gray8_l, e->gray8_r, e->slices, e->cand,    e->stats_dev, e->tickets, e->fast_stats_dev,
                    e->lr_in_l, e->lr_in_r, e->lr_raw};
    for (void *p : ptrs)
        if (p) (void)hipFree(p);
    if (e->hints) (void)hipHostFree(e->hints);
    e->hints = e->hints_dev = nullptr;
}

struct SlotTimer {
    smx_engine *e;
    hipStream_t s;
    int lane, slot;
    bool on;
    SlotTimer(smx_engine *e_, hipStream_t s_, int lane_, int slot_) : e(e_), s(s_), lane(lane_), slot(slot_) {
        on = e->prof_on && e->prof_calls < e->prof_max;
        if (on) (void)hipEventRecord(e->prof_events[index() * 2], s);
    }
    size_t index() const { return ((size_t)e->prof_calls * smx_engine::LANES + lane) * SMX_KERNEL_SLOTS + slot; }
    ~SlotTimer() {
        if (on) {
            (void)hipEventRecord(e->prof_events[index() * 2 + 1], s);
            e->prof_used[index()] = 1;
        }
    }
};

using smx::SMX_EXACT2_LDS_CAP;
hipError_t raise_lds_caps(int device) {
    static std::mutex mu;
    static std::vector<int> done;
    std::lock_guard<std::mutex> lock(mu);
    for (int d : done)
        if (d == device) return hipSuccess;
    if (hipError_t e = smx::exact_raise_lds_caps(SMX_EXACT2_LDS_CAP + (int)((smx::E2_CAPBITS + 2 * smx::E2_SPARSE_WORDS) * sizeof(unsigned)));
        e != hipSuccess) return e;
    if (hipError_t e = smx::match_auto_raise_caps(); e != hipSuccess) return e;
    if (hipError_t e = smx::fast_stack_raise_caps(); e != hipSuccess) return e;
    done.push_back(device);
    return hipSuccess;
}

bool env_is(const char *name, char c) {
    const char *v = std::getenv(name);
    return v && v[0] == c;
}

struct PairView {
    float *gray_l, *gray_r, *down_l, *down_r, *wta, *refined, *costs, *vol;
    int *flags, *flags2;
    uint8_t *gray8_l, *gray8_r;
    unsigned *cand;
};
PairView view_from(const smx_engine *e, int first) {
    const smx_dims &d = e->dm;
    const smx::EngineFacts &ef = e->facts;
    const size_t f = (size_t)first, hw = (size_t)d.h * d.w;
    PairView v{};
    v.gray_l = e->gray_l + f * d.H * ef.gpitch;
    v.gray_r = e->gray_r + f * d.H * ef.gpitch;
    v.down_l = e->down_l + f * hw;
    v.down_r = e->down_r + f * hw;
    v.wta = e->wta + f * hw;
    v.refined = e->refined + f * hw;
    v.costs = e->costs + f * hw;
    v.vol = e->vol ? e->vol + f * hw * d.Dd : nullptr;
    v.flags = e->flags + first;
    v.flags2 = e->flags + e->B + first;
    v.gray8_l = e->gray8_l ? e->gray8_l + f * d.H * ef.pitch8 : nullptr;
    v.gray8_r = e->gray8_r ? e->gray8_r + f * d.H * ef.pitch8 : nullptr;
    v.cand = e->cand ? e->cand + f * ef.cand_tiles_x * ef.cand_tiles_y * ef.cand_cw : nullptr;
    return v;
}

int join_into(smx_engine *e, hipStream_t s) {
    for (int k = 0; k < smx_engine::LANES; ++k) {
        if (!e->lane_stream[k] || !e->ev_join[k]) continue;
        SMX_HIP(hipEventRecord(e->ev_join[k], e->lane_stream[k]));
        SMX_HIP(hipStreamWaitEvent(s, e->ev_join[k], 0));
    }
    e->detached_pending = false;
    return SMX_OK;
}

bool stream_capturing(hipStream_t s) {
    hipStreamCaptureStatus st = hipStreamCaptureStatusNone;
    if (hipStreamIsCapturing(s, &st) != hipSuccess) {
        (void)hipGetLastError();
        return false;
    }
    return st != hipStreamCaptureStatusNone;
}

void read_hints(smx_engine *e) {
    if (!e->hints) return;
    const bool was_dense = e->route.fast.on;
    if (e->route.read_hints(*e->hints) && e->opt_debug_hints)
        std::fprintf(stderr, "[smx] fast kernel: second pass / first pass = %.3f (dense %d)\n", e->route.fast.last, was_dense ? 1 : 0);
}

smx::PrologueArgs prologue_args(const smx_engine *e, const PairView &v, bool owns_gray, const void *left, const void *right) {
    const smx_dims &d = e->dm;
    const smx::EngineFacts &f = e->facts;
    smx::PrologueArgs a{};
    a.left = left; a.right = right; a.gray_l = owns_gray ? v.gray_l : nullptr; a.gray_r = owns_gray ? v.gray_r : nullptr;
    a.down_l = v.down_l; a.down_r = v.down_r;
    a.flags = v.flags; a.flags2 = v.flags2; a.g8_l = v.gray8_l; a.g8_r = v.gray8_r;
    a.H = d.H; a.W = d.W; a.K = d.K; a.h = d.h; a.w = d.w; a.grid_capable = f.grid_capable ? 1 : 0;
    a.pitch8 = f.pitch8; a.padl = f.padl; a.padr = f.padr; a.epoch = e->epoch; a.gpitch = f.gpitch; a.gpadl = f.gpadl;
    a.fp_conv = SMX_FP_STEP1(e->cfg.fp_convention);
    return a;
}
smx::RangeParams range_params(const smx_engine *e, const PairView &v, const smx::CallFacts &call, const smx::RangePlan &pl, int lane, int first) {
    const smx_dims &d = e->dm;
    const smx::EngineFacts &f = e->facts;
    smx::RangeParams b;
    smx::MatchParams &mp = b.mp;
    mp.Ld = v.down_l; mp.Rd = v.down_r; mp.wta = v.wta; mp.costs = v.costs; mp.vol = v.vol;
    mp.flags = v.flags; mp.epoch = e->epoch; mp.B = e->B; mp.h = d.h; mp.w = d.w; mp.dmin = d.dmin; mp.Dd = d.Dd;
    mp.rn = (int)e->cfg.ncc_patch_radius; mp.rs = e->cfg.small_mbm_radius;
    mp.rm = e->cfg.mid_mbm_radius; mp.rl = e->cfg.large_mbm_radius;
    mp.unit = (float)(d.K * d.K);
    mp.on_lanes = call.on_lanes ? 1 : 0;
    mp.tickets = e->tickets ? e->tickets + (size_t)first * f.e2_tiles : nullptr;
    mp.pass1_only = pl.capture_follows ? 1 : 0;
    mp.slices = e->slices ? e->slices + (size_t)lane * f.slices_floats : nullptr;
    b.range_flags = v.flags2;
    b.fast_stats = e->fast_stats_dev + lane;
    return b;
}
struct GrayView { const float *l, *r; int pitch; size_t plane; };
GrayView gray_view(smx_engine *e, const PairView &v, bool owns_gray, int first, const void *left, const void *right) {
    const smx::EngineFacts &f = e->facts;
    GrayView g{owns_gray ? v.gray_l + f.gpadl : (const float *)left, owns_gray ? v.gray_r + f.gpadl : (const float *)right,
               owns_gray ? f.gpitch : e->dm.W, 0};
    g.plane = (size_t)e->dm.H * g.pitch;
    e->last_gray_l = g.l - (size_t)first * g.plane;
    e->last_gray_r = g.r - (size_t)first * g.plane;
    e->last_gray_owned = owns_gray;
    e->last_gpitch = g.pitch;
    e->last_gplane = g.plane;
    return g;
}
smx::RefineParams refine_params(const smx_engine *e, const PairView &v, const smx::RangePlan &pl, const GrayView &g) {
    const smx_dims &d = e->dm;
    const smx::EngineFacts &f = e->facts;
    smx::RefineParams rp{};
    rp.Lg = g.l; rp.Rg = g.r; rp.gpitch = g.pitch; rp.gplane = g.plane; rp.wta = v.wta; rp.costs = v.costs; rp.vol = v.vol;
    rp.refined = v.refined; rp.B = e->B; rp.H = d.H; rp.W = d.W; rp.K = d.K; rp.h = d.h;
    rp.w = d.w; rp.Dd = d.Dd; rp.R = (int)e->cfg.sad_patch_radius;
    rp.flags2 = v.flags2;
    rp.epoch = e->epoch;
    rp.L8 = v.gray8_l; rp.R8 = v.gray8_r; rp.pitch8 = f.pitch8; rp.padl = f.padl;
    rp.fp_conv = SMX_FP_PARABOLA(e->cfg.fp_convention);
    rp.sad_exact = pl.refine.sad_exact ? 1 : 0;
    if (pl.refine.kind == smx::REFINE_AUTO) rp.grid_flags = v.flags;
    if (pl.refine_reports_grid) rp.grid_hint = &e->hints_dev->grid;
    return rp;
}
smx::FillParams fill_params(smx_engine *e, const PairView &v, const smx::RangePlan &pl, int lane, const GrayView &g, float *out) {
    const smx_dims &d = e->dm;
    smx::FillParams fp{};
    fp.Lg = g.l; fp.lpitch = g.pitch; fp.lplane = g.plane; fp.refined = v.refined; fp.out = out; fp.B = e->B; fp.H = d.H; fp.W = d.W;
    fp.K = d.K; fp.h = d.h; fp.w = d.w; fp.thr = (float)e->cfg.threshold;
    fp.log2k = pl.fill.log2k;
    if (pl.fill_publishes) {
        fp.fast_stats = e->fast_stats_dev + lane;
        fp.fast_stats_host = &e->hints_dev->fast_density[lane];
        fp.fast_seq = e->route.fast.next_seq();
        fp.fast_pass1 = (d.Dd + 1) / 2;
    }
    return fp;
}

void enqueue_exact(const smx::RangeParams &b, const smx::RangePlan &pl, int n, hipStream_t s) {
    smx::launch_exact(pl.exact, smx::exact_params(b, pl.exact, n), n, s);
    if (pl.capture_follows) smx::launch_exact2_capture(pl.exact_capture, smx::exact_capture_params(b, pl.exact_capture), n, s);
}
void enqueue_fast(const smx::RangeParams &b, const smx::RangePlan &pl, int n, hipStream_t s) {
    smx::launch_match_fast(pl.fast_launch, smx::fast_params(b, pl, pl.fast_launch.gate), n, s);
    if (pl.capture_follows) smx::launch_match_capture_tu(pl.fast_capture, smx::fast_params(b, pl, pl.fast_capture.gate), n, s);
}

int enqueue_range(smx_engine *e, const smx::CallFacts &call, const smx::RangePlan &pl, int lane, int first, int n,
                  const void *left, const void *right, float *out, hipStream_t s) {
    const smx::EngineFacts &f = e->facts;
    const PairView v = view_from(e, first);
    const GrayView g = gray_view(e, v, pl.owns_gray, first, left, right);
    {
        SlotTimer tm(e, s, lane, SMX_KERNEL_PROLOGUE);
        smx::launch_prologue(pl.prologue, prologue_args(e, v, pl.owns_gray, left, right), n, s);
    }
    if (pl.status != SMX_OK) return fail(pl.status, "%s", pl.refusal);
    if (pl.exact.slice_floats > f.slices_floats)
        return fail(SMX_ERR_HIP, "internal: slice buffer too small for the disparity split of %d pairs", n);

    const smx::RangeParams b = range_params(e, v, call, pl, lane, first);
    switch (pl.route) {
    case smx::AGG_FILTERED: {
        smx::FilterParams fp{};
        fp.cand = v.cand; fp.tiles_x = f.cand_tiles_x; fp.tiles_y = f.cand_tiles_y; fp.cw = f.cand_cw;
        fp.two_e = f.filter_two_e; fp.range_flags = v.flags2;
        {
            SlotTimer tm(e, s, lane, SMX_KERNEL_MATCH_FAST);
            if (pl.gated_dense_first) smx::launch_exact(pl.exact, smx::exact_params(b, pl.exact, n), n, s);
            smx::launch_match_filter_tu(pl.filter, smx::filter_params(b, f), fp, n, s);
        }
        SlotTimer tm(e, s, lane, SMX_KERNEL_MATCH_EXACT);
        smx::launch_exact2_sparse(smx::sparse_params(b, f), n, v.cand, f.cand_cw, (const int *)v.flags2, e->stats_dev + 2 * lane,
                                  &e->hints_dev->filter_density[lane], e->route.filt.next_seq(), s);
        if (pl.capture_follows) smx::launch_exact2_capture(pl.exact_capture, smx::exact_capture_params(b, pl.exact_capture), n, s);
        break;
    }
    case smx::AGG_EXACT: {
        SlotTimer tm(e, s, lane, SMX_KERNEL_MATCH_EXACT);
        enqueue_exact(b, pl, n, s);
        break;
    }
    case smx::AGG_FAST: {
        SlotTimer tm(e, s, lane, SMX_KERNEL_MATCH_FAST);
        enqueue_fast(b, pl, n, s);
        break;
    }
    case smx::AGG_AUTO_ONE_LAUNCH: {
        SlotTimer tm(e, s, lane, SMX_KERNEL_MATCH_FAST);
        smx::launch_match_auto_small_tu(pl.auto_launch, smx::auto_params(b, pl, n), n, s);
        break;
    }
    default: {
        {
            SlotTimer tm(e, s, lane, SMX_KERNEL_MATCH_EXACT);
            enqueue_exact(b, pl, n, s);
        }
        SlotTimer tm(e, s, lane, SMX_KERNEL_MATCH_FAST);
        enqueue_fast(b, pl, n, s);
        break;
    }
    }
    e->last_call.plan = pl;
    {
        SlotTimer tm(e, s, lane, SMX_KERNEL_REFINE);
        smx::launch_refine(pl.refine, refine_params(e, v, pl, g), n, s);
    }
    {
        SlotTimer tm(e, s, lane, SMX_KERNEL_FILL);
        smx::launch_fill(pl.fill, fill_params(e, v, pl, lane, g, out), n, s);
    }
    SMX_HIP(hipGetLastError());
    return SMX_OK;
}

struct LanePool {
    int device;
    int users;
    hipStream_t stream[smx_engine::LANES];
};
std::mutex g_lane_mu;
std::vector<LanePool> g_lane_pools;

int acquire_lane_streams(smx_engine *e) {
    std::lock_guard<std::mutex> lock(g_lane_mu);
    for (LanePool &p : g_lane_pools)
        if (p.device == e->cfg.device_id) {
            p.users++;
            for (int k = 0; k < smx_engine::LANES; ++k) e->lane_stream[k] = p.stream[k];
            return SMX_OK;
        }
    LanePool p{};
    p.device = e->cfg.device_id;
    p.users = 1;
    int prio_least = 0, prio_greatest = 0;
    (void)hipDeviceGetStreamPriorityRange(&prio_least, &prio_greatest);
    for (int k = 0; k < smx_engine::LANES; ++k) {
        const hipError_t err = (e->opt_lane_priority && prio_greatest != prio_least)
                                   ? hipStreamCreateWithPriority(&p.stream[k], hipStreamNonBlocking, prio_greatest)
                                   : hipStreamCreateWithFlags(&p.stream[k], hipStreamNonBlocking);
        if (err != hipSuccess) {
            for (int j = 0; j < k; ++j) (void)hipStreamDestroy(p.stream[j]);
            return fail(SMX_ERR_HIP, "creating the stream lanes failed: %s", hipGetErrorString(err));
        }
    }
    g_lane_pools.push_back(p);
    for (int k = 0; k < smx_engine::LANES; ++k) e->lane_stream[k] = p.stream[k];
    return SMX_OK;
}

void release_lane_streams(smx_engine *e) {
    if (!e->lane_stream[0]) return;
    std::lock_guard<std::mutex> lock(g_lane_mu);
    for (size_t i = 0; i < g_lane_pools.size(); ++i) {
        LanePool &p = g_lane_pools[i];
        if (p.device != e->cfg.device_id || p.stream[0] != e->lane_stream[0]) continue;
        if (--p.users == 0) {
            for (int k = 0; k < smx_engine::LANES; ++k) (void)hipStreamDestroy(p.stream[k]);
            g_lane_pools.erase(g_lane_pools.begin() + (long)i);
        }
        break;
    }
    for (int k = 0; k < smx_engine::LANES; ++k) e->lane_stream[k] = nullptr;
}

int create_lanes(smx_engine *e) {
    if (!e->lane_stream[0]) {
        if (int rc = acquire_lane_streams(e)) return rc;
        for (int k = 0; k < smx_engine::LANES; ++k) {
            SMX_HIP(hipEventCreateWithFlags(&e->ev_join[k], hipEventDisableTiming));
            SMX_HIP(hipEventCreateWithFlags(&e->ev_cross[k], hipEventDisableTiming));
        }
    }
    if (!e->ev_caller) SMX_HIP(hipEventCreateWithFlags(&e->ev_caller, hipEventDisableTiming));
    if (e->caller_calls_unrecorded) {
        hipStream_t last = e->last_caller_stream;
        if (stream_capturing(last))
            return fail(SMX_ERR_UNSUPPORTED, "stream capture: the stream of the engine's last call is being captured; "
                                             "the first SMX_STREAM_ENGINE call cannot be ordered behind it");
        if (hipEventRecord(e->ev_caller, last) == hipSuccess) {
            e->caller_tail_live = true;
        } else {
            (void)hipGetLastError();
            SMX_HIP(hipDeviceSynchronize());
        }
        e->caller_calls_unrecorded = false;
    }
    return SMX_OK;
}

int enqueue(smx_engine *e, int in_mode, int n, const void *left, const void *right, float *out, void *stream) {
    if (!e) return fail(SMX_ERR_INVALID_ARG, "engine is NULL");
    if (!left || !right || !out) return fail(SMX_ERR_INVALID_ARG, "left, right and out must be non-NULL");
    if (n < 1 || n > e->B)
        return fail(SMX_ERR_INVALID_ARG, "batch size %d outside [1, max_batch=%d]", n, e->B);
    DeviceGuard guard(e->cfg.device_id);
    if (!guard.ok) return fail(SMX_ERR_HIP, "cannot select HIP device %d", e->cfg.device_id);
    const smx_dims &d = e->dm;
    const bool detached = stream == SMX_STREAM_ENGINE;
    const bool capturing = !detached && stream_capturing((hipStream_t)stream);
    if (capturing && (e->detached_pending || e->epoch == 0x7fffffff))
        return fail(SMX_ERR_UNSUPPORTED,
                    "stream capture: the engine has work on its own streams that is not joined yet (call smx_join on a "
                    "stream outside the capture first), or its call counter is about to wrap");
    if (detached) {
        if (int rc = create_lanes(e)) return rc;
        if (e->caller_tail_live) {
            for (int k = 0; k < smx_engine::LANES; ++k) SMX_HIP(hipStreamWaitEvent(e->lane_stream[k], e->ev_caller, 0));
            e->caller_tail_live = false;
        }
    } else if (e->detached_pending) {
        if (int rc = join_into(e, (hipStream_t)stream)) return rc;
    }
    if (e->epoch == 0x7fffffff) {
        e->epoch = 0;
        SMX_HIP(hipDeviceSynchronize());
        SMX_HIP(hipMemsetAsync(e->flags, 0, sizeof(int) * 2 * (size_t)e->B, nullptr));
        SMX_HIP(hipStreamSynchronize(nullptr));
    }
    e->epoch++;
    read_hints(e);
    const smx::EngineFacts &f = e->facts;
    const bool split = detached && e->overlap_min > 0 && n >= e->overlap_min;
    const int n0 = split ? (n + 1) / 2 : n;
    smx::CallFacts call;
    call.in_mode = in_mode;
    call.on_lanes = detached;
    call.u8_aligned = (((uintptr_t)left | (uintptr_t)right) & 3u) == 0;
    call.route = e->route.decide_call(smx::call_kind(f, in_mode, detached, n0, n - n0), f.opt.fast_dense, f.exact_filter);
    e->last_call.call = call;
    e->last_call.first = 0;
    const size_t out_pair_bytes = (size_t)d.H * d.W * sizeof(float);
    auto lane_enter = [&](int k, int lo, int hi, const float *out_first, int pairs) -> int {
        const uintptr_t olo = (uintptr_t)out_first, ohi = olo + (size_t)pairs * out_pair_bytes;
        if (e->ledger.enter(k, lo, hi, olo, ohi)) {
            const int o = 1 - k;
            SMX_HIP(hipEventRecord(e->ev_cross[o], e->lane_stream[o]));
            SMX_HIP(hipStreamWaitEvent(e->lane_stream[k], e->ev_cross[o], 0));
        }
        return SMX_OK;
    };
    int rc;
    if (split) {
        const bool rgb = in_mode == smx::IN_RGB_F32 || in_mode == smx::IN_RGB_U8;
        const bool u8 = in_mode == smx::IN_GRAY_U8 || in_mode == smx::IN_RGB_U8;
        const size_t in_pair = (size_t)d.H * d.W * (rgb ? 3 : 1) * (u8 ? 1 : sizeof(float));
        if (int lrc = lane_enter(1, n0, n, out + (size_t)n0 * d.H * d.W, n - n0)) return lrc;
        rc = enqueue_range(e, call, smx::plan_range(f, call, n - n0, false), 1, n0, n - n0, (const char *)left + n0 * in_pair,
                           (const char *)right + n0 * in_pair, out + (size_t)n0 * d.H * d.W, e->lane_stream[1]);
        if (rc == SMX_OK) rc = lane_enter(0, 0, n0, out, n0);
        if (rc == SMX_OK) rc = enqueue_range(e, call, smx::plan_range(f, call, n0, false), 0, 0, n0, left, right, out, e->lane_stream[0]);
    } else {
        int lane = 0, first = 0;
        if (detached && 2 * n <= e->B) {
            lane = e->next_small_lane;
            e->next_small_lane ^= 1;
            first = lane * (e->B / 2);
        }
        e->last_call.first = first;
        if (detached)
            if (int lrc = lane_enter(lane, first, first + n, out, n)) return lrc;
        rc = enqueue_range(e, call, smx::plan_range(f, call, n, true), lane, first, n, left, right, out,
                           detached ? e->lane_stream[lane] : (hipStream_t)stream);
        if (!detached && !capturing) {
            if (e->ev_caller) {
                SMX_HIP(hipEventRecord(e->ev_caller, (hipStream_t)stream));
                e->caller_tail_live = true;
            } else {
                e->caller_calls_unrecorded = true;
                e->last_caller_stream = (hipStream_t)stream;
            }
        }
    }
    if (detached) e->detached_pending = true;
    if (e->prof_on && e->prof_calls < e->prof_max) e->prof_calls++;
    return rc;
}

int enqueue_lr(smx_engine *e, int in_mode, int n, const void *left, const void *right, float *out, float *right_out,
               float max_diff, float invalid, void *stream) {
    if (int rc = check_lr_scalars(max_diff, invalid)) return rc;
    if (!e) return fail(SMX_ERR_INVALID_ARG, "engine is NULL");
    if (!left || !right || !out) return fail(SMX_ERR_INVALID_ARG, "left, right and out must be non-NULL");
    if (n < 1 || 2L * n > e->B)
        return fail(SMX_ERR_INVALID_ARG,
                    "LR batch size %d: the check runs the mirrored problem too, i.e. 2n = %ld internal pairs, which must "
                    "lie in [2, max_batch=%d] (n <= max_batch / 2)", n, 2L * n, e->B);
    if (stream == SMX_STREAM_ENGINE)
        return fail(SMX_ERR_UNSUPPORTED, "LR calls run on a caller's stream only (SMX_STREAM_ENGINE is not supported)");
    const smx_dims &d = e->dm;
    const bool rgb = in_mode == smx::IN_RGB_F32 || in_mode == smx::IN_RGB_U8;
    const bool u8 = in_mode == smx::IN_GRAY_U8 || in_mode == smx::IN_RGB_U8;
    const int planes = rgb ? 3 : 1, es = u8 ? 1 : (int)sizeof(float);
    const size_t hw = (size_t)d.H * d.W, pair_bytes = hw * planes * es;
    const size_t in_bytes = (size_t)n * pair_bytes, out_bytes = (size_t)n * hw * sizeof(float);
    if (ranges_overlap(left, in_bytes, out, out_bytes) || ranges_overlap(right, in_bytes, out, out_bytes) ||
        ranges_overlap(left, in_bytes, right_out, out_bytes) || ranges_overlap(right, in_bytes, right_out, out_bytes) ||
        ranges_overlap(out, out_bytes, right_out, out_bytes))
        return fail(SMX_ERR_INVALID_ARG, "LR call: the inputs, out and right_out must not overlap");
    DeviceGuard guard(e->cfg.device_id);
    if (!guard.ok) return fail(SMX_ERR_HIP, "cannot select HIP device %d", e->cfg.device_id);
    hipStream_t s = (hipStream_t)stream;
    const bool capturing = stream_capturing(s);
    if (!e->lr_raw || e->lr_pair_bytes < pair_bytes) {
        if (capturing)
            return fail(SMX_ERR_UNSUPPORTED, "stream capture: the LR scratch of this input format is not allocated yet "
                                             "(make one LR call outside capture first)");
        if (e->lr_pair_bytes < pair_bytes) {
            if (e->lr_in_l || e->lr_in_r) {
                SMX_HIP(hipDeviceSynchronize());
                (void)hipFree(e->lr_in_l);
                (void)hipFree(e->lr_in_r);
                e->lr_in_l = e->lr_in_r = nullptr;
                e->lr_pair_bytes = 0;
            }
            SMX_HIP(hipMalloc(&e->lr_in_l, (size_t)e->B * pair_bytes));
            SMX_HIP(hipMalloc(&e->lr_in_r, (size_t)e->B * pair_bytes));
            e->lr_pair_bytes = pair_bytes;
        }
        if (!e->lr_raw) SMX_HIP(hipMalloc((void **)&e->lr_raw, (size_t)e->B * hw * sizeof(float)));
    }
    if (capturing && (e->detached_pending || e->epoch == 0x7fffffff))
        return fail(SMX_ERR_UNSUPPORTED,
                    "stream capture: the engine has work on its own streams that is not joined yet (call smx_join on a "
                    "stream outside the capture first), or its call counter is about to wrap");
    smx::launch_lr_pack(es, left, right, e->lr_in_l, e->lr_in_r, (long)n * planes * d.H, d.W, s);
    SMX_HIP(hipGetLastError());
    if (int rc = enqueue(e, in_mode, 2 * n, e->lr_in_l, e->lr_in_r, e->lr_raw, stream)) return rc;
    smx::launch_lr_check(true, e->lr_raw, e->lr_raw + (size_t)n * hw, out, right_out, n, d.H, d.W, max_diff, invalid, s);
    SMX_HIP(hipGetLastError());
    return SMX_OK;
}

}

static thread_local std::string g_last_error;

int smx::fail(int code, const char *fmt, ...) {
    char buf[512];
    va_list ap;
    va_start(ap, fmt);
    vsnprintf(buf, sizeof(buf), fmt, ap);
    va_end(ap);
    g_last_error = buf;
    return code;
}

extern "C" {

int smx_abi_version(void) { return SMX_ABI_VERSION; }

const char *smx_last_error(void) { return g_last_error.c_str(); }

void smx_config_default(smx_config *cfg) {
    if (!cfg) return;
    std::memset(cfg, 0, sizeof(*cfg));
    cfg->height = 1080;
    cfg->width = 1920;
    cfg->downscale_factor = 2;
    cfg->min_disparity = 75;
    cfg->max_disparity = 262;
    cfg->ncc_patch_radius = 1;
    cfg->sad_patch_radius = 5;
    cfg->threshold = 5;
    cfg->small_mbm_radius = 1;
    cfg->mid_mbm_radius = 4;
    cfg->large_mbm_radius = 10;
    cfg->device_id = 0;
    cfg->max_batch = 1;
    cfg->match_mode = SMX_MATCH_AUTO;
}

int smx_get_dims(const smx_config *cfg, smx_dims *dims) {
    if (!cfg || !dims) return fail(SMX_ERR_INVALID_ARG, "cfg and dims must be non-NULL");
    return compute_dims(cfg, dims);
}

static int overlap_min_pairs_default(const smx::EngineFacts &f) {
    const char *v = std::getenv("SMX_OVERLAP_MIN_PAIRS");
    if (v && *v) {
        const int k = std::atoi(v);
        return k < 0 ? 0 : (k == 1 ? 2 : k);
    }
    int n_tall = 1;
    while (n_tall < 4096 && smx::range_fast_plan(f, false, n_tall).small) ++n_tall;
    return 2 * n_tall;
}

static void destroy_lanes(smx_engine *e) {
    for (int k = 0; k < smx_engine::LANES; ++k) {
        if (e->ev_join[k]) (void)hipEventDestroy(e->ev_join[k]);
        if (e->ev_cross[k]) (void)hipEventDestroy(e->ev_cross[k]);
        e->ev_join[k] = e->ev_cross[k] = nullptr;
    }
    release_lane_streams(e);
    if (e->ev_caller) (void)hipEventDestroy(e->ev_caller);
    e->ev_caller = nullptr;
}

int smx_create(const smx_config *cfg, smx_engine **out_engine) {
    if (!cfg || !out_engine) return fail(SMX_ERR_INVALID_ARG, "cfg and out_engine must be non-NULL");
    *out_engine = nullptr;
    smx_dims d;
    int rc = compute_dims(cfg, &d);
    if (rc) return rc;
    if (cfg->match_mode < SMX_MATCH_AUTO || cfg->match_mode > SMX_MATCH_FAST_GRID)
        return fail(SMX_ERR_INVALID_CONFIG, "unknown match_mode %d", cfg->match_mode);
    if (!SMX_FP_VALID(cfg->fp_convention))
        return fail(SMX_ERR_INVALID_CONFIG, "unknown fp_convention %d (smx_fp_convention: 0 .. %d, or SMX_FP_MIXED of two)",
                    cfg->fp_convention, SMX_FP_CONVENTIONS - 1);
    for (int v : cfg->reserved)
        if (v != 0) return fail(SMX_ERR_INVALID_CONFIG, "reserved fields must be 0");
    int ndev = 0;
    SMX_HIP(hipGetDeviceCount(&ndev));
    if (ndev <= 0)
        return fail(SMX_ERR_HIP, "no HIP device visible: libstereo_mi355x has no CPU fallback");
    if (cfg->device_id < 0 || cfg->device_id >= ndev)
        return fail(SMX_ERR_INVALID_CONFIG, "device_id %d outside [0, %d)", cfg->device_id, ndev);

    smx_engine *e = new (std::nothrow) smx_engine();
    if (!e) return fail(SMX_ERR_OUT_OF_MEMORY, "host allocation failed");
    e->cfg = *cfg;
    e->dm = d;
    e->B = cfg->max_batch > 0 ? cfg->max_batch : 1;
    {
        int nd = 0;
        const size_t need = smx::exact_tile_lds(*cfg, d.Dd, &nd);
        if (need > 64 * 1024) {
            delete e;
            return fail(SMX_ERR_UNSUPPORTED,
                        "radii too large for the LDS tile: ncc_patch_radius %u + large_mbm_radius %d need %zu bytes "
                        "of the 65536 available to the exact-order kernel",
                        cfg->ncc_patch_radius, cfg->large_mbm_radius, need);
        }
    }

    DeviceGuard guard(cfg->device_id);
    if (!guard.ok) {
        delete e;
        return fail(SMX_ERR_HIP, "cannot select HIP device %d", cfg->device_id);
    }
    int cus = 0;
    if (hipDeviceGetAttribute(&cus, hipDeviceAttributeMultiprocessorCount, cfg->device_id) != hipSuccess || cus <= 0) cus = 256;
    smx::PlanOptions opt;
    opt.fast_dense = env_is("SMX_FAST_DENSE", '1') ? 1 : (env_is("SMX_FAST_DENSE", '0') ? 0 : -1);
    opt.fast_stack = env_is("SMX_FAST_STACK", '1') ? 1 : (env_is("SMX_FAST_STACK", '0') ? 0 : -1);
    opt.fast_dense_small = env_is("SMX_FAST_DENSE_SMALL", '1') ? 1 : (env_is("SMX_FAST_DENSE_SMALL", '0') ? 0 : -1);
    e->opt_lane_priority = env_is("SMX_LANE_PRIORITY", '0') ? 0 : 1;
    e->opt_debug_hints = std::getenv("SMX_DEBUG_HINTS") != nullptr;
    if (const char *v = std::getenv("SMX_TEST_EPOCH_START")) {
        const long k = std::atol(v);
        if (k > 0 && k < 0x7fffffffL) e->epoch = (int)k;
    }
    e->facts = smx::derive_facts(*cfg, d, cus, opt);
    const smx::EngineFacts &f = e->facts;
    e->overlap_min = cfg->overlap_min_pairs < 0 ? 0
                     : (cfg->overlap_min_pairs > 0 ? (cfg->overlap_min_pairs < 2 ? 2 : cfg->overlap_min_pairs) : overlap_min_pairs_default(f));
    const size_t B = (size_t)e->B, hw = (size_t)d.h * d.w;
    hipError_t err = hipSuccess;
    auto alloc = [&](void **p, size_t bytes) {
        if (err == hipSuccess) err = hipMalloc(p, bytes);
        if (err == hipSuccess) err = hipMemset(*p, 0, bytes);
    };
    alloc((void **)&e->gray_l, B * (size_t)d.H * f.gpitch * sizeof(float));
    alloc((void **)&e->gray_r, B * (size_t)d.H * f.gpitch * sizeof(float));
    alloc((void **)&e->down_l, B * hw * sizeof(float));
    alloc((void **)&e->down_r, B * hw * sizeof(float));
    alloc((void **)&e->wta, B * hw * sizeof(float));
    alloc((void **)&e->refined, B * hw * sizeof(float));
    alloc((void **)&e->costs, 3 * B * hw * sizeof(float));
    alloc((void **)&e->flags, 2 * B * sizeof(int));
    alloc((void **)&e->fast_stats_dev, smx_engine::LANES * sizeof(unsigned long long));
    if (f.has_u8_planes()) {
        alloc((void **)&e->gray8_l, B * (size_t)d.H * f.pitch8);
        alloc((void **)&e->gray8_r, B * (size_t)d.H * f.pitch8);
    }
    if (f.has_tickets()) alloc((void **)&e->tickets, B * (size_t)f.e2_tiles * sizeof(unsigned));
    if (f.has_slices()) {
        alloc((void **)&e->slices, smx_engine::LANES * f.slices_floats * sizeof(float));
    }
    if (f.filter_ok) {
        alloc((void **)&e->cand, B * (size_t)f.cand_tiles_x * f.cand_tiles_y * f.cand_cw * sizeof(unsigned));
        alloc((void **)&e->stats_dev, 2 * smx_engine::LANES * sizeof(unsigned));
    }
    if (f.has_volume) alloc((void **)&e->vol, B * hw * (size_t)d.Dd * sizeof(float));
    if (err == hipSuccess) {
        err = hipHostMalloc((void **)&e->hints, sizeof(HostHints), hipHostMallocDefault);
        if (err == hipSuccess) {
            std::memset(e->hints, 0, sizeof(HostHints));
            err = hipHostGetDevicePointer((void **)&e->hints_dev, e->hints, 0);
        }
    }
    if (err == hipSuccess) err = hipStreamSynchronize(nullptr);
    if (err != hipSuccess) {
        free_buffers(e);
        delete e;
        return fail(err == hipErrorOutOfMemory ? SMX_ERR_OUT_OF_MEMORY : SMX_ERR_HIP,
                    "device allocation failed: %s", hipGetErrorString(err));
    }
    if (hipError_t aerr = raise_lds_caps(cfg->device_id); aerr != hipSuccess) {
        free_buffers(e);
        delete e;
        return fail(SMX_ERR_HIP, "hipFuncSetAttribute(MaxDynamicSharedMemorySize) failed: %s", hipGetErrorString(aerr));
    }
    *out_engine = e;
    return SMX_OK;
}

void smx_destroy(smx_engine *e) {
    if (!e) return;
    {
        DeviceGuard guard(e->cfg.device_id);
        (void)hipDeviceSynchronize();
        destroy_lanes(e);
        free_events(e);
        free_buffers(e);
    }
    delete e;
}

int smx_compute_rgb(smx_engine *e, const float *l, const float *r, float *out, void *stream) {
    return enqueue(e, smx::IN_RGB_F32, 1, l, r, out, stream);
}
int smx_compute_rgb_u8(smx_engine *e, const uint8_t *l, const uint8_t *r, float *out, void *stream) {
    return enqueue(e, smx::IN_RGB_U8, 1, l, r, out, stream);
}
int smx_compute_gray(smx_engine *e, const float *l, const float *r, float *out, void *stream) {
    return enqueue(e, smx::IN_GRAY_F32, 1, l, r, out, stream);
}
int smx_compute_gray_u8(smx_engine *e, const uint8_t *l, const uint8_t *r, float *out, void *stream) {
    return enqueue(e, smx::IN_GRAY_U8, 1, l, r, out, stream);
}
int smx_compute_gray_batch(smx_engine *e, int n, const float *l, const float *r, float *out, void *stream) {
    return enqueue(e, smx::IN_GRAY_F32, n, l, r, out, stream);
}
int smx_compute_rgb_batch(smx_engine *e, int n, const float *l, const float *r, float *out, void *stream) {
    return enqueue(e, smx::IN_RGB_F32, n, l, r, out, stream);
}
int smx_compute_gray_u8_batch(smx_engine *e, int n, const uint8_t *l, const uint8_t *r, float *out, void *stream) {
    return enqueue(e, smx::IN_GRAY_U8, n, l, r, out, stream);
}
int smx_compute_rgb_u8_batch(smx_engine *e, int n, const uint8_t *l, const uint8_t *r, float *out, void *stream) {
    return enqueue(e, smx::IN_RGB_U8, n, l, r, out, stream);
}

int smx_compute_lr_gray_batch(smx_engine *e, int n, const float *l, const float *r, float *out, float *right_out,
                              float max_diff, float invalid, void *stream) {
    return enqueue_lr(e, smx::IN_GRAY_F32, n, l, r, out, right_out, max_diff, invalid, stream);
}
int smx_compute_lr_gray_u8_batch(smx_engine *e, int n, const uint8_t *l, const uint8_t *r, float *out, float *right_out,
                                 float max_diff, float invalid, void *stream) {
    return enqueue_lr(e, smx::IN_GRAY_U8, n, l, r, out, right_out, max_diff, invalid, stream);
}
int smx_compute_lr_rgb_batch(smx_engine *e, int n, const float *l, const float *r, float *out, float *right_out,
                             float max_diff, float invalid, void *stream) {
    return enqueue_lr(e, smx::IN_RGB_F32, n, l, r, out, right_out, max_diff, invalid, stream);
}
int smx_compute_lr_rgb_u8_batch(smx_engine *e, int n, const uint8_t *l, const uint8_t *r, float *out, float *right_out,
                                float max_diff, float invalid, void *stream) {
    return enqueue_lr(e, smx::IN_RGB_U8, n, l, r, out, right_out, max_diff, invalid, stream);
}

size_t smx_stage_bytes(const smx_engine *e, int stage) {
    if (!e) return 0;
    const smx_dims &d = e->dm;
    const size_t HW = (size_t)d.H * d.W * sizeof(float), hw = (size_t)d.h * d.w * sizeof(float);
    switch (stage) {
        case SMX_STAGE_GRAY_LEFT: case SMX_STAGE_GRAY_RIGHT: return HW;
        case SMX_STAGE_DOWN_LEFT: case SMX_STAGE_DOWN_RIGHT: return hw;
        case SMX_STAGE_WTA: case SMX_STAGE_REFINED: return hw;
        case SMX_STAGE_MBM_COSTS: return 3 * hw;
        case SMX_STAGE_AGG_VOLUME: return e->vol ? hw * (size_t)d.Dd : 0;
        case SMX_STAGE_GRID_FLAG: return sizeof(int);
        default: return 0;
    }
}

int smx_get_intermediate(smx_engine *e, int stage, int pair, void *dst, size_t bytes, void *stream) {
    if (!e || !dst) return fail(SMX_ERR_INVALID_ARG, "engine and dst must be non-NULL");
    if (pair < 0 || pair >= e->B) return fail(SMX_ERR_INVALID_ARG, "pair_index out of range");
    if (stream == SMX_STREAM_ENGINE) return fail(SMX_ERR_INVALID_ARG, "smx_get_intermediate needs a caller stream");
    if (e->detached_pending && stream_capturing((hipStream_t)stream))
        return fail(SMX_ERR_UNSUPPORTED, "stream capture: the engine has unjoined work on its own streams");
    if (e->detached_pending) {
        DeviceGuard jg(e->cfg.device_id);
        if (!jg.ok) return fail(SMX_ERR_HIP, "cannot select HIP device %d", e->cfg.device_id);
        if (int rc = join_into(e, (hipStream_t)stream)) return rc;
    }
    const size_t need = smx_stage_bytes(e, stage);
    if (need == 0) return fail(SMX_ERR_INVALID_ARG, "stage %d not available for this engine", stage);
    if (bytes != need) return fail(SMX_ERR_INVALID_ARG, "stage %d needs %zu bytes, got %zu", stage, need, bytes);
    DeviceGuard guard(e->cfg.device_id);
    if (!guard.ok) return fail(SMX_ERR_HIP, "cannot select HIP device %d", e->cfg.device_id);
    hipStream_t s = (hipStream_t)stream;
    const smx_dims &d = e->dm;
    if (pair + e->last_call.first >= e->B) return fail(SMX_ERR_INVALID_ARG, "pair_index out of range");
    const size_t hw = (size_t)d.h * d.w, p = (size_t)(pair + e->last_call.first);
    const void *src = nullptr;
    switch (stage) {
        case SMX_STAGE_GRAY_LEFT:
        case SMX_STAGE_GRAY_RIGHT: {
            const float *g = stage == SMX_STAGE_GRAY_LEFT ? e->last_gray_l : e->last_gray_r;
            if (!g) return fail(SMX_ERR_INVALID_ARG, "no call has been made yet");
            if (!e->last_gray_owned)
                return fail(SMX_ERR_INVALID_ARG,
                            "the f32 gray entry keeps no gray planes: steps 6-9 read the caller's own buffers, which "
                            "the engine does not own after the call");
            SMX_HIP(hipMemcpy2DAsync(dst, (size_t)d.W * sizeof(float), g + p * e->last_gplane,
                                     (size_t)e->last_gpitch * sizeof(float), (size_t)d.W * sizeof(float), d.H,
                                     hipMemcpyDefault, s));
            return SMX_OK;
        }
        case SMX_STAGE_DOWN_LEFT: src = e->down_l + p * hw; break;
        case SMX_STAGE_DOWN_RIGHT: src = e->down_r + p * hw; break;
        case SMX_STAGE_WTA: src = e->wta + p * hw; break;
        case SMX_STAGE_REFINED: src = e->refined + p * hw; break;
        case SMX_STAGE_AGG_VOLUME: src = e->vol + p * hw * (size_t)d.Dd; break;
        case SMX_STAGE_GRID_FLAG:
            smx::launch_flag_to_bool(e->flags + p, e->epoch, (int *)dst, s);
            SMX_HIP(hipGetLastError());
            return SMX_OK;
        case SMX_STAGE_MBM_COSTS: {
            for (int k = 0; k < 3; ++k)
                SMX_HIP(hipMemcpyAsync((char *)dst + k * hw * sizeof(float),
                                       e->costs + ((size_t)k * e->B + p) * hw, hw * sizeof(float),
                                       hipMemcpyDefault, s));
            return SMX_OK;
        }
        default: return fail(SMX_ERR_INVALID_ARG, "unknown stage %d", stage);
    }
    SMX_HIP(hipMemcpyAsync(dst, src, bytes, hipMemcpyDefault, s));
    return SMX_OK;
}

int smx_get_match_geometry(const smx_engine *e, int n, smx_match_geometry *g) {
    if (!e || !g || n < 1) return fail(SMX_ERR_INVALID_ARG, "smx_get_match_geometry: NULL argument or n < 1");
    std::memset(g, 0, sizeof(*g));
    const bool on_lanes = e->last_call.call.on_lanes;
    if (on_lanes && smx_overlap_lanes(e, n) == 2) n = (n + 1) / 2;
    smx::match_geometry(e->facts, on_lanes, n, g);
    return SMX_OK;
}

int smx_build_features(void) { return 0; }

int smx_get_route_info(smx_engine *e, smx_route_info *info) {
    if (!e || !info) return fail(SMX_ERR_INVALID_ARG, "smx_get_route_info: NULL argument");
    read_hints(e);
    std::memset(info, 0, sizeof(*info));
    info->filter_available = e->facts.filter_ok ? 1 : 0;
    info->route_dense = e->route.filt.on ? 1 : 0;
    info->last_call_filtered = e->last_call.call.route.use_filter ? 1 : 0;
    info->probe_period = e->route.filt.period;
    info->candidate_density = e->route.filt.last;
    info->offgrid_hint = e->route.grid_hint;
    info->compute_units = e->facts.cus;
    info->fast_dense = e->route.fast.on ? 1 : 0;
    return SMX_OK;
}

int smx_last_match_mode(const smx_engine *e) {
    return e ? e->last_call.plan.mode : SMX_ERR_INVALID_ARG;
}

int smx_join(smx_engine *e, void *stream) {
    if (!e || stream == SMX_STREAM_ENGINE) return fail(SMX_ERR_INVALID_ARG, "smx_join: engine NULL or no caller stream");
    if (!e->detached_pending) return SMX_OK;
    DeviceGuard guard(e->cfg.device_id);
    if (!guard.ok) return fail(SMX_ERR_HIP, "cannot select HIP device %d", e->cfg.device_id);
    if (stream_capturing((hipStream_t)stream))
        return fail(SMX_ERR_UNSUPPORTED, "stream capture: smx_join would make the captured stream wait for work outside the capture");
    return join_into(e, (hipStream_t)stream);
}

int smx_overlap_lanes(const smx_engine *e, int n) {
    if (!e || n < 1) return SMX_ERR_INVALID_ARG;
    return (e->overlap_min > 0 && n >= e->overlap_min && n <= e->B) ? smx_engine::LANES : 1;
}

int smx_profile_begin(smx_engine *e, int max_calls) {
    if (!e || max_calls < 1 || max_calls > 4096)
        return fail(SMX_ERR_INVALID_ARG, "smx_profile_begin: engine NULL or max_calls outside [1, 4096]");
    DeviceGuard guard(e->cfg.device_id);
    if (!guard.ok) return fail(SMX_ERR_HIP, "cannot select HIP device %d", e->cfg.device_id);
    free_events(e);
    const size_t n = (size_t)max_calls * smx_engine::LANES * SMX_KERNEL_SLOTS * 2;
    e->prof_events.reserve(n);
    for (size_t i = 0; i < n; ++i) {
        hipEvent_t ev;
        SMX_HIP(hipEventCreate(&ev));
        e->prof_events.push_back(ev);
    }
    e->prof_used.assign((size_t)max_calls * smx_engine::LANES * SMX_KERNEL_SLOTS, 0);
    e->prof_max = max_calls;
    e->prof_calls = 0;
    e->prof_on = true;
    return SMX_OK;
}

int smx_profile_end(smx_engine *e, float mean_ms[SMX_KERNEL_SLOTS], int launches[SMX_KERNEL_SLOTS]) {
    if (!e || !mean_ms || !launches) return fail(SMX_ERR_INVALID_ARG, "smx_profile_end: NULL argument");
    if (!e->prof_on) return fail(SMX_ERR_INVALID_ARG, "smx_profile_end without smx_profile_begin");
    DeviceGuard guard(e->cfg.device_id);
    if (!guard.ok) return fail(SMX_ERR_HIP, "cannot select HIP device %d", e->cfg.device_id);
    double sum[SMX_KERNEL_SLOTS] = {0};
    for (int k = 0; k < SMX_KERNEL_SLOTS; ++k) launches[k] = 0;
    for (int c = 0; c < e->prof_calls * smx_engine::LANES; ++c) {
        for (int k = 0; k < SMX_KERNEL_SLOTS; ++k) {
            if (!e->prof_used[(size_t)c * SMX_KERNEL_SLOTS + k]) continue;
            hipEvent_t a = e->prof_events[((size_t)c * SMX_KERNEL_SLOTS + k) * 2];
            hipEvent_t b = e->prof_events[((size_t)c * SMX_KERNEL_SLOTS + k) * 2 + 1];
            SMX_HIP(hipEventSynchronize(b));
            float ms = 0.f;
            SMX_HIP(hipEventElapsedTime(&ms, a, b));
            sum[k] += ms;
            launches[k]++;
        }
    }
    for (int k = 0; k < SMX_KERNEL_SLOTS; ++k) mean_ms[k] = launches[k] ? (float)(sum[k] / launches[k]) : 0.f;
    free_events(e);
    return SMX_OK;
}

}
```

### stereo-depth_amd/csrc/smx_launch.h

```cpp
#pragma once
#include <hip/hip_runtime.h>
#include <stdint.h>

#include "smx_common.h"

namespace smx {

struct RefineParams;
struct FillParams;
struct FilterParams;

struct PrologueArgs {
    const void *left, *right;
    float *gray_l, *gray_r, *down_l, *down_r;
    int *flags, *flags2;
    uint8_t *g8_l, *g8_r;
    int H, W, K, h, w, grid_capable, pitch8, padl, padr, epoch, gpitch, gpadl;
    int fp_conv;
};
void launch_prologue(const PrologueLaunch &x, const PrologueArgs &a, int n, hipStream_t s);
void launch_refine(const RefineLaunch &x, const RefineParams &p, int n, hipStream_t s);
void launch_fill(const FillLaunch &x, const FillParams &p, int n, hipStream_t s);
void launch_flag_to_bool(const int *flag, int epoch, int *out, hipStream_t s);
void launch_metrics(int n, const float *est, const float *gt, const uint8_t *mask, size_t pixels, float max_disparity,
                    const float thresholds[4], double *out_sums, hipStream_t s);
void launch_points(const float *disp, int H, int W, float bf, float invalid, float *depth, float *points, int *count_dev,
                   int *workspace, hipStream_t s);

void launch_exact(const ExactLaunch &x, const MatchParams &p, int n, hipStream_t s);
void launch_exact2_capture(const ExactCaptureLaunch &x, const MatchParams &p, int n, hipStream_t s);
void launch_exact2_sparse(const MatchParams &p, int n, unsigned *cand, int cw, const int *range_flags, unsigned *stats_dev,
                          unsigned long long *stats_host, unsigned seq, hipStream_t s);
hipError_t exact_raise_lds_caps(int cap_bytes);

void launch_match_fast(const FastLaunch &fl, const MatchParams &p, int n, hipStream_t s);
void launch_match_fast_tall_24(const FastLaunch &fl, const MatchParams &p, int n, hipStream_t s);
void launch_match_fast_tall_27(const FastLaunch &fl, const MatchParams &p, int n, hipStream_t s);
void launch_match_fast_tall_32(const FastLaunch &fl, const MatchParams &p, int n, hipStream_t s);
void launch_match_fast_stack(const FastLaunch &fl, const MatchParams &p, int n, hipStream_t s);
hipError_t fast_stack_raise_caps();
void launch_match_auto_small_tu(const AutoLaunch &al, const MatchParams &p, int n, hipStream_t s);
hipError_t match_auto_raise_caps();

void launch_match_capture_tu(const FastCaptureLaunch &cl, const MatchParams &p, int n, hipStream_t s);

void launch_match_filter_tu(const FilterLaunch &fl, const MatchParams &p, const FilterParams &f, int n, hipStream_t s);
void launch_match_filter_24(const FilterLaunch &fl, const MatchParams &p, const FilterParams &f, int n, hipStream_t s);
void launch_match_filter_27(const FilterLaunch &fl, const MatchParams &p, const FilterParams &f, int n, hipStream_t s);
void launch_match_filter_32(const FilterLaunch &fl, const MatchParams &p, const FilterParams &f, int n, hipStream_t s);

void launch_lr_pack(int elem_bytes, const void *l, const void *r, void *pl, void *pr, long rows, int W, hipStream_t s);
void launch_lr_check(bool mirrored, const float *left, const float *right, float *out, float *right_out, int n, int H, int W,
                     float max_diff, float invalid, hipStream_t s);

void launch_filter_speckles(int n, int H, int W, const float *in, float *out, int max_size, float max_diff, float invalid,
                            void *workspace, hipStream_t s);
void launch_fill_invalid(int n, int H, int W, const float *in, float *out, float invalid, void *workspace, hipStream_t s);

size_t median_workspace_bytes(int n, int H, int W);
void launch_weighted_median(int n, int H, int W, const float *in, const float *holes, const float *guide, float *out,
                            int radius, const uint16_t *range, const uint16_t *spatial, float invalid, hipStream_t s);

void launch_wls(int n, int H, int W, const float *in, const float *conf, const float *guide, float *out, int iterations,
                const float *lambdas, const float *range, float min_weight, float invalid, void *workspace,
                hipStream_t s);

void launch_confidence(int n, int H, int W, const float *left, const float *right, const float *guide, int radius,
                       float lr_scale, float texture_scale, float invalid, float *out, hipStream_t s);

void launch_temporal(int n, int H, int W, const float *disp, const float *conf, const float *guide,
                     const float *prev_guide, float *state_disp, float *state_weight, float *guide_out, float *out,
                     int radius, float threshold, float decay, float max_diff, float max_weight, float min_weight,
                     float invalid, hipStream_t s);

void launch_remap_pairs(int n, int C, bool f32, int Hi, int Wi, int Ho, int Wo, const void *in_l, const void *in_r,
                        const int32_t *map_l, const int32_t *map_r, void *out_l, void *out_r, bool replicate,
                        float border_value, hipStream_t s);

void launch_synthesis(int n, int C, bool f32, int D, int h, int w, int S, const float *prob, const void *left, float *out,
                      hipStream_t s);

void launch_sgm(int n, int C, bool f32, int H, int W, const void *left, const void *right, int dmin, int D, int paths,
                int P1, int P2, int uniqueness, float lr_max_diff, bool subpixel, float invalid, float *out,
                float *gray_out, float *right_out, void *workspace, hipStream_t s);

void launch_reproject(int n, int H, int W, const float *disp, const float q[16], const float *conf, float min_conf,
                      float zmin, float zmax, float invalid, const void *image, int channels, bool img_f32,
                      float *points, uint8_t *colors, int32_t *indices, float *xyz_map, int32_t *offsets,
                      void *workspace, hipStream_t s);
hipError_t launch_voxel_downsample(int n, int capacity, const float *points, const uint8_t *colors,
                                   const int32_t *offsets, float voxel_size, int min_points, float *out_points,
                                   uint8_t *out_colors, int32_t *out_counts, int32_t *out_offsets, int32_t *dropped,
                                   void *workspace, hipStream_t s);
void launch_scan(const int *in, int *out, long L, int *block_sums, const int *gate, int pass, hipStream_t s);

void launch_tsdf_integrate(int nx, int ny, int nz, const float origin[3], float voxel_size, float truncation,
                           float max_weight, float *tsdf, float *weight, uint8_t *color, int n, int H, int W,
                           const float *disp, const float q[16], const float p[16], const float *world_to_camera,
                           const float *conf, float min_conf, float zmin, float zmax, float invalid, const void *image,
                           int channels, bool img_f32, void *workspace, hipStream_t s);
void launch_tsdf_extract(int nx, int ny, int nz, const float origin[3], float voxel_size, const float *tsdf,
                         const float *weight, const uint8_t *color, float min_weight, int capacity, float *points,
                         float *normals, uint8_t *colors, int32_t *count, void *workspace, hipStream_t s);
void launch_tsdf_triangles(int nx, int ny, int nz, const float *tsdf, const float *weight, float min_weight,
                           int capacity, int32_t *triangles, int32_t *count, void *workspace, hipStream_t s);

void launch_tsdf_raycast(int nx, int ny, int nz, const float origin[3], float voxel_size, const float *tsdf,
                         const float *weight, const uint8_t *color, float min_weight, int n, int H, int W,
                         const float q[16], const float *camera_to_world, float step, float zmin, int M, float invalid,
                         float *disp, float *depth, float *normals, uint8_t *colors, float *out_weight, void *workspace,
                         hipStream_t s);

void launch_track_camera(int n, int H, int W, const float *disp, const float *confidence, const float q[16],
                         float min_confidence, float zmin, float zmax, float invalid, int Hm, int Wm,
                         const float *model_depth, const float *model_normals, const float qm[16], const float pm[16],
                         const float *model_camera_to_world, const float *model_world_to_camera, const float *pose_in,
                         int pairs, const int32_t *schedule, float max_distance, int min_inliers, float min_pivot,
                         float rot_eps, float trans_eps, float *pose_out, int32_t *info, float *rms,
                         double *normal_equations, void *workspace, hipStream_t s);

}
```

### stereo-depth_amd/csrc/smx_plan.h

```cpp
#pragma once

#include "../../include/stereo_mi355x.h"
#include "k_match_auto.h"
#include "k_match_capture.h"
#include "k_match_exact.h"
#include "k_match_exact2.h"
#include "k_match_fast.h"
#include "k_match_filter.h"
#include "k_prologue.h"
#include "smx_common.h"
#include "smx_launch.h"
#include "smx_route.h"

namespace smx {

constexpr int SMX_EXACT2_LDS_CAP = 80 * 1024;

struct PlanOptions {
    int fast_dense = -1;
    int fast_dense_small = -1;
    int fast_stack = -1;
};

struct EngineFacts {
    int match_mode = SMX_MATCH_AUTO, exact_filter = 0;
    int B = 1, h = 0, w = 0, dmin = 0, Dd = 0, K = 1;
    int sad_patch_radius = 5;
    int cus = 256;
    PlanOptions opt;
    bool grid_capable = false;
    bool default_radii = false;
    bool fast_ok = false;
    bool filter_ok = false;
    bool capture = false;
    bool has_volume = false;
    int kt = 0;
    int pitch8 = 0, padl = 0, padr = 0;
    int gpitch = 0, gpadl = 0;
    bool prologue_k2 = false;
    bool prologue_k4 = false;
    bool sad_exact = true;
    int exact_nd = 0, exact2_nd = 0;
    size_t exact_lds = 0, exact2_lds = 0;
    int e2_tiles = 0;
    size_t slices_floats = 0;
    int cand_tiles_x = 0, cand_tiles_y = 0, cand_cw = 0;
    int filter_unit = 0;
    float filter_two_e = 0.f;
    bool filter_words = false, fast_words = false;

    bool has_u8_planes() const { return pitch8 != 0; }
    bool has_tickets() const { return default_radii; }
    bool has_slices() const { return slices_floats != 0; }
};

inline size_t exact_tile_lds(const smx_config &cfg, int Dd, int *nd) {
    *nd = Dd;
    while (*nd > 1 && exact_lds_floats((int)cfg.ncc_patch_radius, cfg.large_mbm_radius, *nd) * sizeof(float) > 64 * 1024)
        *nd = (*nd + 1) / 2;
    return exact_lds_floats((int)cfg.ncc_patch_radius, cfg.large_mbm_radius, *nd) * sizeof(float);
}

inline EngineFacts derive_facts(const smx_config &cfg, const smx_dims &d, int cus, PlanOptions opt) {
    EngineFacts f;
    f.match_mode = cfg.match_mode; f.exact_filter = cfg.exact_filter;
    f.B = cfg.max_batch > 0 ? cfg.max_batch : 1;
    f.h = d.h; f.w = d.w; f.dmin = d.dmin; f.Dd = d.Dd; f.K = d.K;
    f.sad_patch_radius = (int)cfg.sad_patch_radius;
    f.cus = cus;
    f.opt = opt;
    const int K = d.K;
    f.grid_capable = (K == 1 || K == 2 || K == 4 || K == 8);
    f.default_radii = cfg.ncc_patch_radius == 1 && cfg.small_mbm_radius == 1 && cfg.mid_mbm_radius == 4 &&
                      cfg.large_mbm_radius == 10;
    f.fast_ok = f.grid_capable && f.default_radii;
    f.exact_lds = exact_tile_lds(cfg, d.Dd, &f.exact_nd);
    int nd2 = d.Dd;
    while (nd2 > 1 && exact2_lds_floats(nd2) * sizeof(float) > (size_t)SMX_EXACT2_LDS_CAP) nd2 = (nd2 + 1) / 2;
    f.exact2_nd = nd2;
    f.exact2_lds = exact2_lds_floats(nd2) * sizeof(float);
    {
        const int padl = (8 + K * (d.dmax + 2) + 3) & ~3, padr = (32 + K + 3) & ~3;
        f.kt = (cfg.sad_patch_radius == 5 && (K == 1 || K == 2 || K == 4)) ? K : 0;
        if (f.kt != 0 && padl <= d.W && padr <= d.W) {
            f.padl = padl; f.padr = padr;
            f.pitch8 = (padl + d.W + padr + 3) & ~3;
            f.gpitch = f.pitch8;
            f.gpadl = padl;
        } else {
            f.gpitch = d.W;
            f.gpadl = 0;
        }
    }
    f.prologue_k2 = K == 2 && (d.W & 1) == 0;
    f.prologue_k4 = K == 4 && (d.W & 3) == 0 && f.grid_capable && (f.gpitch & 3) == 0 && (f.gpadl & 3) == 0 && (f.pitch8 & 3) == 0 &&
                    (f.padl & 3) == 0 && (f.gpadl == 0 || f.gpadl == f.padl);
    f.sad_exact = (long long)K * ((long long)cfg.min_disparity / K + d.Dd) <= 271;
    if (f.default_radii) {
        MatchParams sp{};
        sp.h = d.h; sp.w = d.w; sp.Dd = d.Dd;
        f.slices_floats = slice_region_floats(sp, f.B, cus, f.fast_ok);
        f.e2_tiles = ((d.w + E2_TW - 1) / E2_TW) * ((d.h + E2_TH - 1) / E2_TH);
    }
    f.capture = capture_applicable(d.dmin, d.Dd) && f.default_radii;
    f.has_volume = d.dmin > 0 && !f.capture;
    static_assert(FILTER_TILE_H == E2_TH && FILTER_TILE_W == E2_TW, "the filter marks exact-order tiles");
    f.filter_ok = cfg.exact_filter >= 0 && f.fast_ok && f.default_radii && K * K <= 64 &&
                  filter_cand_words(d.Dd) <= E2_SPARSE_WORDS && !f.has_volume;
    if (f.filter_ok) {
        f.cand_tiles_x = (d.w + E2_TW - 1) / E2_TW;
        f.cand_tiles_y = (d.h + E2_TH - 1) / E2_TH;
        f.cand_cw = filter_cand_words(d.Dd);
        f.filter_unit = K * K;
        f.filter_two_e = (float)(2.0 * filter_error_bound_units((double)f.filter_unit) * (1.0 + 1e-6));
    }
    f.filter_words = f.filter_ok;
    f.fast_words = true;
    return f;
}

struct CallFacts {
    int in_mode = IN_GRAY_F32;
    bool on_lanes = false;
    bool u8_aligned = true;
    CallRoute route{false, true, -1};
};

enum AggRoute {
    AGG_FILTERED = 0,
    AGG_EXACT,
    AGG_FAST,
    AGG_AUTO_ONE_LAUNCH,
    AGG_AUTO_GATED,
    AGG_ROUTES
};

struct RangePlan {
    int status = SMX_OK;
    const char *refusal = nullptr;
    int mode = SMX_MATCH_EXACT_ORDER;
    AggRoute route = AGG_EXACT;
    bool gated_dense_first = false;
    bool exact_split = false;
    bool capture_follows = false;
    FastPlan fast{};
    bool dense = false, dense_small = false;
    bool reports = false;
    int stride = 0;
    bool fill_publishes = false;
    bool owns_gray = true;
    bool refine_reports_grid = false;
    PrologueLaunch prologue{};
    RefineLaunch refine{};
    FillLaunch fill{};
    ExactLaunch exact{};
    ExactCaptureLaunch exact_capture{};
    FastLaunch fast_launch{};
    FastCaptureLaunch fast_capture{};
    AutoLaunch auto_launch{};
    FilterLaunch filter{};

    bool has_fast_launch() const { return route == AGG_FAST || route == AGG_AUTO_ONE_LAUNCH || route == AGG_AUTO_GATED; }
};

inline bool is_rgb(int in_mode) { return in_mode == IN_RGB_F32 || in_mode == IN_RGB_U8; }

inline MatchParams plan_params(const EngineFacts &f, bool on_lanes) {
    MatchParams mp{};
    mp.B = f.B; mp.h = f.h; mp.w = f.w; mp.dmin = f.dmin; mp.Dd = f.Dd;
    mp.on_lanes = on_lanes ? 1 : 0;
    mp.pass1_only = f.capture ? 1 : 0;
    return mp;
}
inline FastPlan range_fast_plan(const EngineFacts &f, bool on_lanes, int n) { return match_fast_plan(plan_params(f, on_lanes), n, f.cus, f.opt.fast_stack); }

inline ExactLaunch exact_launch(const EngineFacts &f, bool on_lanes, int n, bool allow_split) {
    ExactLaunch x;
    if (!f.default_radii || f.has_volume) {
        x.kernel = f.has_volume ? EXACT_GENERIC_VOLUME : EXACT_GENERIC;
        x.nd_chunk = f.exact_nd;
        x.lds_bytes = f.exact_lds;
        return x;
    }
    x.kernel = EXACT_TILED;
    x.nd_chunk = f.exact2_nd;
    x.lds_bytes = f.exact2_lds;
    x.split = allow_split ? exact_split(f.e2_tiles, n, f.Dd, f.cus) : 1;
    if (x.split > 1) {
        x.slice_floats = (size_t)x.split * SMX_SLICE_WORDS * n * f.h * f.w;
        const int per = (f.Dd + x.split - 1) / x.split;
        if (x.nd_chunk > per) x.nd_chunk = per;
        const long wgs = (long)f.e2_tiles * n * x.split, slots = 2L * f.cus;
        x.rows_per_thread = on_lanes && 2 * wgs > slots && wgs < 2 * slots ? 4 : 2;
    }
    return x;
}

inline ExactCaptureLaunch exact_capture_launch(const EngineFacts &f, int n, bool allow_split) {
    ExactCaptureLaunch x;
    x.split = allow_split ? capture_split(f.e2_tiles, n, f.Dd, f.cus) : 1;
    x.rows_per_thread = allow_split ? 2 : 4;
    x.nd_chunk = f.exact2_nd;
    x.lds_bytes = exact2_capture_lds_bytes(f.exact2_nd);
    return x;
}

inline FastLaunch fast_launch(const EngineFacts &f, const FastPlan &pl, bool dense, bool dense_small) {
    FastLaunch x;
    x.small = pl.small;
    x.th = pl.th;
    x.pk = fast_pk(f.K * f.K);
    bool dense_here;
    if (pl.small) {
        x.pitch = pl.wide ? 320 : 256;
        dense_here = dense_small && pl.th == FA_TH_SMALL_TALL && f.Dd <= x.pitch - 64 + 1;
    } else {
        x.pitch = fast_tall_pitch(f.Dd);
        x.argb = x.pitch != 320 || f.Dd <= 256;
        if (pl.th == 32 && dense && !f.capture && f.Dd <= 256) x.th = FA_DENSE_MAX_TH;
        dense_here = dense && x.argb && x.th <= FA_DENSE_MAX_TH;
    }
    x.form = f.capture ? FAST_PASS1_ONLY : (!dense_here ? FAST_SPARSE : (pl.small ? FAST_DENSE_SMALL : FAST_DENSE));
    x.stack = pl.stack;
    return x;
}

inline FastCaptureLaunch fast_capture_launch(const EngineFacts &f, const FastPlan &pl) {
    return FastCaptureLaunch{pl.small, f.Dd > FA_WIDE_FROM, fast_pk(f.K * f.K)};
}

inline AutoLaunch auto_launch(const EngineFacts &f, const MatchParams &mp, int th) {
    AutoLaunch x;
    x.th = th;
    x.wide = fast_small_wide(f.Dd);
    x.pk = fast_pk(f.K * f.K);
    x.nsplit = match_auto_nsplit(mp, th);
    x.nd_chunk = f.exact2_nd;
    const int per = (f.Dd + x.nsplit - 1) / x.nsplit;
    if (x.nd_chunk > per) x.nd_chunk = per;
    x.lds_bytes = x.wide ? fast_lds_bytes<320>(th, f.Dd, true) : fast_lds_bytes<256>(th, f.Dd, true);
    const size_t exact_lds = exact2_lds_floats(x.nd_chunk) * sizeof(float);
    if (exact_lds > x.lds_bytes) x.lds_bytes = exact_lds;
    return x;
}

inline FilterLaunch filter_launch(const EngineFacts &f, const MatchParams &mp, int n) {
    const FilterPlan pl = filter_plan(mp, n, f.cus);
    return FilterLaunch{pl.th, pl.wide, fast_pk(f.filter_unit)};
}

inline PrologueLaunch prologue_launch(const EngineFacts &f, const CallFacts &call) {
    const bool u8 = call.in_mode == IN_GRAY_U8 || call.in_mode == IN_RGB_U8;
    PrologueLaunch x;
    x.in_mode = call.in_mode;
    if (f.prologue_k2 && !is_rgb(call.in_mode)) x.kernel = PROLOGUE_K2;
    else if (f.prologue_k4 && (!u8 || call.u8_aligned)) x.kernel = PROLOGUE_K4;
    return x;
}

inline FillLaunch fill_launch(const EngineFacts &f, bool on_lanes, int n) {
    FillLaunch x;
    x.K = f.K;
    x.kernel = f.K == 1 || f.K == 2 || f.K == 4 ? FILL_4 : ((f.K & (f.K - 1)) == 0 ? FILL_POW2 : FILL_GENERIC);
    x.px = on_lanes && n > 4 ? 4 : 8;
    while ((1 << x.log2k) < f.K) x.log2k++;
    return x;
}

inline RangePlan plan_range(const EngineFacts &f, const CallFacts &call, int n, bool whole_call) {
    RangePlan p;
    p.owns_gray = call.in_mode != IN_GRAY_F32;
    p.prologue = prologue_launch(f, call);
    if (f.match_mode == SMX_MATCH_FAST_GRID && !f.fast_ok) {
        p.status = SMX_ERR_UNSUPPORTED;
        p.refusal = "SMX_MATCH_FAST_GRID needs downscale_factor in {1,2,4,8}, ncc radius 1 and "
                    "block-matching radii 1/4/10";
        return p;
    }
    if (f.has_volume && f.match_mode == SMX_MATCH_FAST_GRID) {
        p.status = SMX_ERR_UNSUPPORTED;
        p.refusal = "SMX_MATCH_FAST_GRID cannot serve min_disparity/K > disparity count or "
                    "non-default radii with min_disparity > 0 (aggregated volume needed)";
        return p;
    }
    const bool rgb = is_rgb(call.in_mode);
    p.mode = f.match_mode;
    if (f.has_volume) p.mode = SMX_MATCH_EXACT_ORDER;
    if (p.mode == SMX_MATCH_AUTO) {
        if (!f.fast_ok) p.mode = SMX_MATCH_EXACT_ORDER;
        else if (call.in_mode == IN_GRAY_U8) p.mode = SMX_MATCH_FAST_GRID;
        else if (rgb) p.mode = SMX_MATCH_EXACT_ORDER;
    }
    const MatchParams mp = plan_params(f, call.on_lanes);
    p.fast = match_fast_plan(mp, n, f.cus, f.opt.fast_stack);
    const bool small = p.fast.small;
    p.capture_follows = f.capture;

    if (p.mode == SMX_MATCH_EXACT_ORDER && f.filter_ok && rgb && !small && f.default_radii && call.route.use_filter) {
        p.route = AGG_FILTERED;
        p.gated_dense_first = call.in_mode == IN_RGB_F32;
        p.filter = filter_launch(f, mp, n);
    } else if (p.mode == SMX_MATCH_EXACT_ORDER) {
        p.route = AGG_EXACT;
        p.exact_split = whole_call;
    } else if (p.mode == SMX_MATCH_FAST_GRID) {
        p.route = AGG_FAST;
    } else {
        const bool one_launch = f.default_radii && small && call.route.grid_hint == 0 && !f.capture && !f.has_volume && f.has_tickets() &&
                                f.has_slices() && match_auto_small_applicable(mp, p.fast.th, n, f.slices_floats);
        if (one_launch) {
            p.route = AGG_AUTO_ONE_LAUNCH;
            p.auto_launch = auto_launch(f, mp, p.fast.th);
        } else {
            p.route = AGG_AUTO_GATED;
            p.exact_split = whole_call && small && call.route.grid_hint != 0;
        }
    }

    if (p.has_fast_launch() && !mp.pass1_only && f.Dd <= FA_BITWORDS * 32) {
        const bool tall12 = small && p.fast.th == FA_TH_SMALL_TALL;
        if (!small || tall12) {
            if (!(tall12 && f.opt.fast_dense_small == 1) && f.fast_words && f.opt.fast_dense < 0) {
                p.stride = n > 4 ? (n + 3) / 4 : 1;
                const long wgs_pair = tall12 ? (long)((f.w + FA_VALID - 1) / FA_VALID) * ((f.h + p.fast.th - 1) / p.fast.th)
                                             : (long)((f.w + FA_VALID * FA_WAVES - 1) / (FA_VALID * FA_WAVES)) * ((f.h + 23) / 24) * FA_WAVES;
                p.reports = ((n + p.stride - 1) / p.stride) * wgs_pair < (1L << 23);
            }
            const bool dense = tall12 && f.opt.fast_dense_small >= 0 ? f.opt.fast_dense_small == 1 : call.route.fast_dense;
            if (dense) (tall12 ? p.dense_small : p.dense) = true;
            else p.fill_publishes = p.reports;
        }
    }
    if (p.dense && p.fast.stack > 1) {
        MatchParams md = mp;
        md.dense = 1;
        p.fast = match_fast_plan(md, n, f.cus, f.opt.fast_stack);
    }

    if (p.route == AGG_FILTERED || p.route == AGG_EXACT || p.route == AGG_AUTO_GATED) {
        p.exact = exact_launch(f, call.on_lanes, n, p.exact_split);
        if (p.capture_follows) p.exact_capture = exact_capture_launch(f, n, p.exact_split);
    }
    if (p.route == AGG_FAST || p.route == AGG_AUTO_GATED) {
        p.fast_launch = fast_launch(f, p.fast, p.dense, p.dense_small);
        if (p.capture_follows) p.fast_capture = fast_capture_launch(f, p.fast);
    }
    if (p.route == AGG_FILTERED) {
        p.exact.gate = 2;
        p.exact.gate_flag = GATE_RANGE_FLAG;
    } else if (p.route == AGG_AUTO_GATED) {
        p.exact.gate = p.exact_capture.gate = 2;
        p.fast_launch.gate = p.fast_capture.gate = 1;
    }

    p.refine.kt = f.kt;
    p.refine.sad_exact = f.sad_exact;
    if (f.kt == 0 || !f.has_u8_planes() || rgb) {
        p.refine.kind = REFINE_FLOAT;
        p.refine.apron = p.owns_gray && f.gpadl > 0 && call.in_mode != IN_GRAY_U8;
    } else if (call.in_mode == IN_GRAY_U8) {
        p.refine.kind = n > 4 ? REFINE_INT_V : REFINE_INT;
    } else if (n <= 4) {
        p.refine.kind = REFINE_AUTO;
        p.refine_reports_grid = whole_call;
    } else {
        p.refine.kind = REFINE_AUTO_V;
    }
    p.fill = fill_launch(f, call.on_lanes, n);
    return p;
}

struct RangeParams {
    MatchParams mp{};
    const int *range_flags = nullptr;
    unsigned long long *fast_stats = nullptr;
};
inline MatchParams exact_params(const RangeParams &b, const ExactLaunch &x, int n) {
    MatchParams p = b.mp;
    p.gate = x.gate;
    if (x.gate_flag == GATE_RANGE_FLAG) p.flags = b.range_flags;
    p.nd_chunk = x.nd_chunk;
    if (x.split > 1) {
        p.nsplit = x.split;
        p.pairs = n;
        p.tickets = nullptr;
    }
    return p;
}
inline MatchParams exact_capture_params(const RangeParams &b, const ExactCaptureLaunch &x) {
    MatchParams p = b.mp;
    p.gate = x.gate;
    p.nd_chunk = x.nd_chunk;
    p.nsplit = x.split;
    return p;
}
inline MatchParams fast_params(const RangeParams &b, const RangePlan &pl, int gate) {
    MatchParams p = b.mp;
    p.gate = gate;
    p.dense = pl.dense ? 1 : 0;
    p.dense_small = pl.dense_small ? 1 : 0;
    if (pl.fill_publishes) {
        p.fast_stats = b.fast_stats;
        p.fast_stride = pl.stride;
    }
    return p;
}
inline MatchParams auto_params(const RangeParams &b, const RangePlan &pl, int n) {
    MatchParams p = fast_params(b, pl, 0);
    p.nsplit = pl.auto_launch.nsplit;
    p.pairs = n;
    p.nd_chunk = pl.auto_launch.nd_chunk;
    return p;
}
inline MatchParams filter_params(const RangeParams &b, const EngineFacts &f) {
    MatchParams p = b.mp;
    p.unit = (float)f.filter_unit;
    return p;
}
inline MatchParams sparse_params(const RangeParams &b, const EngineFacts &f) {
    MatchParams p = b.mp;
    p.nd_chunk = f.exact2_nd;
    return p;
}

inline CallKind call_kind(const EngineFacts &f, int in_mode, bool on_lanes, int n0, int n1) {
    CallKind k{};
    CallFacts call;
    call.in_mode = in_mode;
    call.on_lanes = on_lanes;
    for (int n : {n0, n1}) {
        if (n < 1) continue;
        const RangePlan p = plan_range(f, call, n, n1 < 1);
        if (p.status != SMX_OK) continue;
        if (p.route == AGG_FILTERED && f.filter_words) k.filter_reports = true;
        if (p.has_fast_launch() && p.reports) k.fast_reports = true;
    }
    return k;
}

inline void match_geometry(const EngineFacts &f, bool on_lanes, int n, smx_match_geometry *g) {
    if (!f.fast_ok) {
        g->kernel = SMX_KERNEL_EXACT_ONLY;
        return;
    }
    const FastPlan pl = range_fast_plan(f, on_lanes, n);
    g->kernel = pl.small ? SMX_KERNEL_FAST_SPLIT : SMX_KERNEL_FAST_WINDOW;
    g->band_rows = pl.th * pl.stack;
    g->waves_per_workgroup = pl.small ? FA_DS_WAVES : FA_WAVES;
    const int cols_per_wg = FA_VALID * (pl.small ? 1 : FA_WAVES);
    const long wgs = (long)((f.w + cols_per_wg - 1) / cols_per_wg) * ((f.h + g->band_rows - 1) / g->band_rows);
    g->rows_marched = g->band_rows + 22;
    g->workgroups = (int)(wgs * n);
    const long waves = wgs * g->waves_per_workgroup;
    const double lane_rows = (double)waves * 64.0 * g->rows_marched / (g->kernel == SMX_KERNEL_FAST_SPLIT ? (double)FA_DS_WAVES : 1.0);
    g->useful_fraction = (double)f.h * f.w / lane_rows;
    g->columns_per_wave = (double)f.w * ((f.h + g->band_rows - 1) / g->band_rows) /
                          ((double)waves / (g->kernel == SMX_KERNEL_FAST_SPLIT ? (double)FA_DS_WAVES : 1.0));
}

}
```

### stereo-depth_amd/csrc/tu_stages.hip

```cpp
#include "k_fill.h"
#include "k_metrics.h"
#include "k_points.h"
#include "k_prologue.h"
#include "k_refine.h"
#include "smx_launch.h"

namespace smx {

namespace {
__global__ void k_flag_to_bool(const int *flag, int epoch, int *out) { *out = (*flag == epoch) ? 1 : 0; }

template <int MODE>
void prologue_t(int kernel, const PrologueArgs &a, int n, hipStream_t s) {
    const dim3 block(64, 4), grid((a.w + 63) / 64, (a.h + 3) / 4, n);
    switch (kernel) {
        case PROLOGUE_K2: {
            constexpr int M2 = (MODE == IN_GRAY_U8) ? IN_GRAY_U8 : IN_GRAY_F32;
            hipLaunchKernelGGL((k_prologue_k2<M2>), dim3((a.w + 127) / 128, grid.y, n), block, 0, s, a.left, a.right, a.gray_l, a.gray_r,
                               a.down_l, a.down_r, a.flags, a.g8_l, a.g8_r, a.flags2, a.H, a.W, a.h, a.w,
                               a.pitch8, a.padl, a.padr, a.epoch, a.gpitch, a.gpadl);
            return;
        }
        case PROLOGUE_K4:
            hipLaunchKernelGGL((k_prologue_k4<MODE>), grid, block, 0, s, a.left, a.right, a.gray_l, a.gray_r, a.down_l,
                               a.down_r, a.flags, a.g8_l, a.g8_r, a.flags2, a.H, a.W, a.h, a.w,
                               a.pitch8, a.padl, a.padr, a.epoch, a.gpitch, a.gpadl, a.fp_conv);
            return;
        default:
            hipLaunchKernelGGL((k_prologue<MODE>), grid, block, 0, s, a.left, a.right, a.gray_l, a.gray_r, a.down_l,
                               a.down_r, a.flags, a.g8_l, a.g8_r, a.flags2, a.H, a.W, a.K, a.h, a.w,
                               a.grid_capable, a.pitch8, a.padl, a.padr, a.epoch, a.gpitch, a.gpadl, a.fp_conv);
    }
}
}

void launch_prologue(const PrologueLaunch &x, const PrologueArgs &a, int n, hipStream_t s) {
    switch (x.in_mode) {
        case IN_GRAY_F32: prologue_t<IN_GRAY_F32>(x.kernel, a, n, s); break;
        case IN_RGB_F32: prologue_t<IN_RGB_F32>(x.kernel, a, n, s); break;
        case IN_RGB_U8: prologue_t<IN_RGB_U8>(x.kernel, a, n, s); break;
        default: prologue_t<IN_GRAY_U8>(x.kernel, a, n, s); break;
    }
}

void launch_refine(const RefineLaunch &x, const RefineParams &rp, int n, hipStream_t s) {
    const dim3 block(64, 4);
    const dim3 grid((rp.w + 63) / 64, (rp.h + 3) / 4, n);
    const dim3 vgrid(grid.x, (rp.h + 4 * RV - 1) / (4 * RV), n);
    switch (x.kind) {
        case REFINE_FLOAT: {
            const dim3 fgrid(grid.x * grid.y, 1, n);
            if (x.apron) {
                switch (x.kt) {
                    case 1: hipLaunchKernelGGL((k_refine<1, 5, true>), fgrid, block, 0, s, rp); return;
                    case 2: hipLaunchKernelGGL((k_refine<2, 5, true>), fgrid, block, 0, s, rp); return;
                    case 4: hipLaunchKernelGGL((k_refine<4, 5, true>), fgrid, block, 0, s, rp); return;
                    default: break;
                }
            }
            switch (x.kt) {
                case 1: hipLaunchKernelGGL((k_refine<1, 5, false>), fgrid, block, 0, s, rp); break;
                case 2: hipLaunchKernelGGL((k_refine<2, 5, false>), fgrid, block, 0, s, rp); break;
                case 4: hipLaunchKernelGGL((k_refine<4, 5, false>), fgrid, block, 0, s, rp); break;
                default: hipLaunchKernelGGL((k_refine<0, 0, false>), fgrid, block, 0, s, rp); break;
            }
            return;
        }
#define SMX_LAUNCH_INT(KERNEL, GRID)                                                                            \
    switch (x.kt * 2 + (x.sad_exact ? 1 : 0)) {                                                                 \
        case 3: hipLaunchKernelGGL((KERNEL<1, true>), GRID, block, 0, s, rp); break;                            \
        case 2: hipLaunchKernelGGL((KERNEL<1, false>), GRID, block, 0, s, rp); break;                           \
        case 5: hipLaunchKernelGGL((KERNEL<2, true>), GRID, block, 0, s, rp); break;                            \
        case 4: hipLaunchKernelGGL((KERNEL<2, false>), GRID, block, 0, s, rp); break;                           \
        case 9: hipLaunchKernelGGL((KERNEL<4, true>), GRID, block, 0, s, rp); break;                            \
        default: hipLaunchKernelGGL((KERNEL<4, false>), GRID, block, 0, s, rp); break;                          \
    }
        case REFINE_INT: SMX_LAUNCH_INT(k_refine_int, grid) return;
        case REFINE_INT_V: SMX_LAUNCH_INT(k_refine_int_v, vgrid) return;
        case REFINE_AUTO: SMX_LAUNCH_INT(k_refine_auto, grid) return;
        default: SMX_LAUNCH_INT(k_refine_auto_v, vgrid) return;
#undef SMX_LAUNCH_INT
    }
}

void launch_fill(const FillLaunch &x, const FillParams &fp, int n, hipStream_t s) {
    const dim3 grid((fp.W + 255) / 256, fp.H, n);
    const dim3 grid8((fp.W + 256 * 8 - 1) / (256 * 8), fp.h, n), grid4((fp.W + 256 * 4 - 1) / (256 * 4), fp.h, n);
    switch (x.kernel) {
        case FILL_4:
            switch (x.K * 10 + x.px) {
                case 14: case 18: hipLaunchKernelGGL((k_fill4<1, 4>), grid4, dim3(256), 0, s, fp); break;
                case 24: hipLaunchKernelGGL((k_fill4<2, 4>), grid4, dim3(256), 0, s, fp); break;
                case 28: hipLaunchKernelGGL((k_fill4<2, 8>), grid8, dim3(256), 0, s, fp); break;
                case 44: hipLaunchKernelGGL((k_fill4<4, 4>), grid4, dim3(256), 0, s, fp); break;
                default: hipLaunchKernelGGL((k_fill4<4, 8>), grid8, dim3(256), 0, s, fp); break;
            }
            break;
        case FILL_POW2: hipLaunchKernelGGL(k_fill<true>, grid, dim3(256), 0, s, fp); break;
        default: hipLaunchKernelGGL(k_fill<false>, grid, dim3(256), 0, s, fp); break;
    }
}

void launch_flag_to_bool(const int *flag, int epoch, int *out, hipStream_t s) {
    hipLaunchKernelGGL(k_flag_to_bool, dim3(1), dim3(1), 0, s, flag, epoch, out);
}

void launch_metrics(int n, const float *est, const float *gt, const uint8_t *mask, size_t pixels, float max_disparity,
                    const float thresholds[4], double *out_sums, hipStream_t s) {
    MetricsParams mp{};
    mp.est = est; mp.gt = gt; mp.mask = mask; mp.out = out_sums; mp.pixels = pixels;
    mp.max_disp = max_disparity;
    for (int k = 0; k < 4; ++k) mp.thr[k] = thresholds[k];
    size_t blocks = (pixels + 256 * 8 - 1) / (256 * 8);
    if (blocks > 1024) blocks = 1024;
    hipLaunchKernelGGL(k_metrics, dim3((unsigned)blocks, (unsigned)n), dim3(256), 0, s, mp);
}

void launch_points(const float *disp, int H, int W, float bf, float invalid, float *depth, float *points, int *count_dev,
                   int *workspace, hipStream_t s) {
    int *row_count = workspace, *row_offset = workspace + H;
    hipLaunchKernelGGL(k_depth_count, dim3(H), dim3(256), 0, s, disp, depth, row_count, W, bf, invalid);
    hipLaunchKernelGGL(k_row_scan, dim3(1), dim3(1024), 0, s, row_count, row_offset, count_dev, H);
    hipLaunchKernelGGL(k_points_scatter, dim3(H), dim3(256), 0, s, disp, row_offset, points, W, bf, invalid);
}

}
```

Baseline: 101,900.

## Stage precomputed u16 unit planes in match kernels instead of converting f32 tiles

```diff
diff --git a/stereo-depth_amd/csrc/k_match_capture.h b/stereo-depth_amd/csrc/k_match_capture.h
--- a/stereo-depth_amd/csrc/k_match_capture.h
+++ b/stereo-depth_amd/csrc/k_match_capture.h
@@ -33,8 +33,11 @@
     const bool active = cw0 < w;
     const int x0 = blk.y * TH;
     const int col = cw0 - FA_HALO + lane;
+    constexpr bool UNITS = fast_units_form(TH, PR, false, true);
     const float *Lp = p.Ld + (size_t)b * h * w;
     const float *Rp = p.Rd + (size_t)b * h * w;
+    const unsigned short *Lup = p.Lu + (size_t)b * h * p.upitch;
+    const unsigned short *Rup = p.Ru + (size_t)b * h * p.upitch;
     const float unit = p.unit;
 
     FastLane ln;
@@ -48,7 +51,8 @@
     ln.colidx = ln.store_ok ? col : 0;
     ln.lptr = Lt + wcol + lane;
 
-    fast_stage<(WGCOLS + 63) / 64, FA_WAVES>(Lt, FA_PL, Lp, h, w, x0 - FA_HALO, cwg0 - FA_HALO, TH + 22, WGCOLS, unit, wv, lane);
+    if constexpr (!UNITS)
+        fast_stage<(WGCOLS + 63) / 64, FA_WAVES>(Lt, FA_PL, Lp, h, w, x0 - FA_HALO, cwg0 - FA_HALO, TH + 22, WGCOLS, unit, wv, lane);
     for (int e = tid; e < FA_WAVES * BW; e += 64 * FA_WAVES) bits[e] = 0u;
     __syncthreads();
 
@@ -89,18 +93,26 @@
         vpk[o >> 1] |= V << (16 * (o & 1));
     }
 
-    auto stage_right = [&](int d0, int nd) {
+    auto stage_right = [&](int d0, int nd, bool with_left = false) {
         __syncthreads();
         const int cbase = cwg0 - FA_HALO - (p.dmin + d0 + nd - 1);
-        fast_stage<(PR + 63) / 64, FA_WAVES>(Rt, PR, Rp, h, w, x0 - FA_HALO, cbase, TH + 22, WGCOLS + nd - 1, unit, wv, lane);
+        if constexpr (!UNITS)
+            fast_stage<(PR + 63) / 64, FA_WAVES>(Rt, PR, Rp, h, w, x0 - FA_HALO, cbase, TH + 22, WGCOLS + nd - 1, unit, wv, lane);
+        else if (with_left)
+            fast_stage_units<(PR + 255) / 256, FA_WAVES, true>(Rt, PR, Rup, cbase, WGCOLS + nd - 1, Lt, Lup, cwg0 - FA_HALO, WGCOLS, h, w,
+                                                               p.upitch, x0 - FA_HALO, TH + 22, wv, lane);
+        else
+            fast_stage_units<(PR + 255) / 256, FA_WAVES, false>(Rt, PR, Rup, cbase, WGCOLS + nd - 1, nullptr, nullptr, 0, 0, h, w,
+                                                                p.upitch, x0 - FA_HALO, TH + 22, wv, lane);
         __syncthreads();
     };
 
     float best[TH];
     int arg[TH];
+    stage_right(0, min(ND, Dd), true);
     for (int d0 = 0; d0 < Dd; d0 += ND) {
         const int nd = min(ND, Dd - d0);
-        stage_right(d0, nd);
+        if (d0 > 0) stage_right(d0, nd);
         if (active) {
             const unsigned *mybits = bits + wv * BW;
             auto march = [&](int dda, int ddb, unsigned rows) {
diff --git a/stereo-depth_amd/csrc/k_match_fast.h b/stereo-depth_amd/csrc/k_match_fast.h
--- a/stereo-depth_amd/csrc/k_match_fast.h
+++ b/stereo-depth_amd/csrc/k_match_fast.h
@@ -156,6 +156,62 @@
         }
         ra += rstep;
         ra = ra >= h ? ra - h : ra;
+    }
+}
+
+__host__ __device__ constexpr bool fast_units_form(int th, int pr, bool dsplit, bool argb) {
+#ifdef SMX_FA_STAGE_F32
+    (void)th; (void)pr; (void)dsplit; (void)argb;
+    return false;
+#else
+    return dsplit ? th != FA_TH_SMALL_MID : (pr != 320 || argb);
+#endif
+}
+#ifndef SMX_FA_STAGE_LOADS
+#define SMX_FA_STAGE_LOADS 8
+#endif
+template <int NK, int NW, bool WITH_LEFT>
+__device__ __forceinline__ void fast_stage_units(unsigned short *tile, int pitch, const unsigned short *img, int col0, int cols,
+                                                 unsigned short *ltile, const unsigned short *limg, int lcol0, int lcols,
+                                                 int h, int w, int upitch, int row0, int rows, int wv, int lane) {
+    constexpr int NB = SMX_FA_STAGE_LOADS / (NK + (WITH_LEFT ? 1 : 0));
+    typedef unsigned u32x2 __attribute__((ext_vector_type(2)));
+    unsigned coff[NK], lcoff = 0u;
+    bool in[NK], lin = false;
+#pragma unroll
+    for (int k = 0; k < NK; ++k) {
+        in[k] = 256 * k + 4 * lane < cols;
+        coff[k] = 2u * (unsigned)wrapi(col0 + 256 * k + 4 * lane, w);
+    }
+    if (WITH_LEFT) {
+        lin = 4 * lane < lcols;
+        lcoff = 2u * (unsigned)wrapi(lcol0 + 4 * lane, w);
+    }
+    const int wvu = __builtin_amdgcn_readfirstlane(wv);
+    int ra = wrapi(row0 + wvu, h);
+    const int rstep = NW % h;
+    for (int r0 = wvu; r0 < rows; r0 += NB * NW) {
+        u32x2 v[NB][NK], lv[NB];
+#pragma unroll
+        for (int j = 0; j < NB; ++j) {
+            const size_t roff = (size_t)ra * upitch;
+#pragma unroll
+            for (int k = 0; k < NK; ++k)
+                __builtin_memcpy(&v[j][k], __builtin_assume_aligned((const char *)(img + roff) + coff[k], 2), 8);
+            if (WITH_LEFT) __builtin_memcpy(&lv[j], __builtin_assume_aligned((const char *)(limg + roff) + lcoff, 2), 8);
+            ra += rstep;
+            ra = ra >= h ? ra - h : ra;
+        }
+#pragma unroll
+        for (int j = 0; j < NB; ++j) {
+            const int r = r0 + j * NW;
+            if (r < rows) {
+#pragma unroll
+                for (int k = 0; k < NK; ++k)
+                    if (in[k]) __builtin_memcpy(__builtin_assume_aligned(tile + r * pitch + 256 * k + 4 * lane, 8), &v[j][k], 8);
+                if (WITH_LEFT && lin) __builtin_memcpy(__builtin_assume_aligned(ltile + r * FA_PL + 4 * lane, 8), &lv[j], 8);
+            }
+        }
     }
 }
 
@@ -528,8 +584,11 @@
     const bool active = cw0 < w;
     const int x0 = blk.y * TH;
     const int col = cw0 - FA_HALO + lane;
+    constexpr bool UNITS = fast_units_form(TH, PR, DSPLIT, ARGB);
     const float *Lp = p.Ld + (size_t)b * h * w;
     const float *Rp = p.Rd + (size_t)b * h * w;
+    const unsigned short *Lup = p.Lu + (size_t)b * h * p.upitch;
+    const unsigned short *Rup = p.Ru + (size_t)b * h * p.upitch;
     const float unit = p.unit;
 
     FastLane ln;
@@ -554,19 +613,28 @@
 #pragma unroll
     for (int o = 0; o < (DENSE && DSPLIT ? TH : 1); ++o) dfirst[o] = 0.f;
 
-    fast_stage<(WGCOLS + 63) / 64, NW>(Lt, FA_PL, Lp, h, w, x0 - FA_HALO, cwg0 - FA_HALO, TH + 22, WGCOLS, unit, wv, lane);
+    if constexpr (!UNITS)
+        fast_stage<(WGCOLS + 63) / 64, NW>(Lt, FA_PL, Lp, h, w, x0 - FA_HALO, cwg0 - FA_HALO, TH + 22, WGCOLS, unit, wv, lane);
     for (int e = tid; e < NW * BW; e += 64 * NW) bits[e] = 0u;
 
-    auto stage_right = [&](int d0, int nd) {
+    auto stage_right = [&](int d0, int nd, bool with_left = false) {
         __syncthreads();
         const int cbase = cwg0 - FA_HALO - (p.dmin + d0 + nd - 1);
-        fast_stage<(PR + 63) / 64, NW>(Rt, PR, Rp, h, w, x0 - FA_HALO, cbase, TH + 22, WGCOLS + nd - 1, unit, wv, lane);
+        if constexpr (!UNITS)
+            fast_stage<(PR + 63) / 64, NW>(Rt, PR, Rp, h, w, x0 - FA_HALO, cbase, TH + 22, WGCOLS + nd - 1, unit, wv, lane);
+        else if (with_left)
+            fast_stage_units<(PR + 255) / 256, NW, true>(Rt, PR, Rup, cbase, WGCOLS + nd - 1, Lt, Lup, cwg0 - FA_HALO, WGCOLS, h, w, p.upitch,
+                                                         x0 - FA_HALO, TH + 22, wv, lane);
+        else
+            fast_stage_units<(PR + 255) / 256, NW, false>(Rt, PR, Rup, cbase, WGCOLS + nd - 1, nullptr, nullptr, 0, 0, h, w, p.upitch,
+                                                          x0 - FA_HALO, TH + 22, wv, lane);
         __syncthreads();
     };
 
+    if constexpr (UNITS) stage_right(0, min(ND, Dd), true);
     for (int d0 = 0; d0 < Dd; d0 += ND) {
         const int nd = min(ND, Dd - d0);
-        stage_right(d0, nd);
+        if (!UNITS || d0 > 0) stage_right(d0, nd);
         if (active) {
             const int q4 = ((nd + 2 * NW - 1) / (2 * NW)) * 2;
             const int dd_lo = DSPLIT ? min(nd, wv * q4) : 0;
diff --git a/stereo-depth_amd/csrc/k_prologue.h b/stereo-depth_amd/csrc/k_prologue.h
--- a/stereo-depth_amd/csrc/k_prologue.h
+++ b/stereo-depth_amd/csrc/k_prologue.h
@@ -28,6 +28,24 @@
     }
 }
 
+#ifdef SMX_PROLOGUE_PK8_F32
+#define SMX_PROLOGUE_PK8(MODE) ((MODE) == IN_GRAY_F32)
+#else
+#define SMX_PROLOGUE_PK8(MODE) false
+#endif
+__device__ __forceinline__ void store_unit_u16(uint16_t *plane, unsigned at, uint16_t u) {
+    *(uint16_t *)((char *)plane + (size_t)(2u * at)) = u;
+}
+__device__ __forceinline__ void store_unit_apron(uint16_t *plane, unsigned row, int w, int y, uint16_t u) {
+    if (y < 3) {
+        store_unit_u16(plane, row + (unsigned)(w + y), u);
+        if (w < 3) {
+            if (y + w < 3) store_unit_u16(plane, row + (unsigned)(w + y + w), u);
+            if (y + 2 * w < 3) store_unit_u16(plane, row + (unsigned)(w + y + 2 * w), u);
+        }
+    }
+}
+
 template <int MODE>
 __global__ __launch_bounds__(256) void k_prologue(const void *left, const void *right,
                                                   float *gray_l, float *gray_r,
@@ -35,7 +53,8 @@
                                                   uint8_t *g8_l, uint8_t *g8_r, int *flags2,
                                                   int H, int W, int K, int h, int w, int grid_capable,
                                                   int pitch8, int padl, int padr, int epoch,
-                                                  int gpitch, int gpadl, int fp_conv) {
+                                                  int gpitch, int gpadl, int fp_conv,
+                                                  uint16_t *units_l, uint16_t *units_r, int upitch) {
     const int y = blockIdx.x * 64 + threadIdx.x;
     const int x = blockIdx.y * 4 + threadIdx.y;
     const int b = blockIdx.z;
@@ -93,6 +112,11 @@
             (side ? down_r : down_l)[((size_t)b * h + x) * w + y] = pooled;
             const float s = pooled * unit;
             bad = bad || !(s == rintf(s) && pooled >= 0.0f && pooled <= 255.0f);
+            if (units_l != nullptr) {
+                uint16_t *uplane = (side ? units_r : units_l) + (size_t)b * h * upitch;
+                store_unit_u16(uplane, (unsigned)(x * upitch + y), (unsigned short)s);
+                store_unit_apron(uplane, (unsigned)(x * upitch), w, y, (unsigned short)s);
+            }
         }
     }
     const unsigned long long m = __ballot(bad);
@@ -110,11 +134,13 @@
                                                      uint8_t *g8_l, uint8_t *g8_r, int *flags2,
                                                      int H, int W, int h, int w,
                                                      int pitch8, int padl, int padr, int epoch,
-                                                     int gpitch, int gpadl) {
+                                                     int gpitch, int gpadl,
+                                                     uint16_t *units_l, uint16_t *units_r, int upitch) {
     const int yp = (blockIdx.x * 64 + threadIdx.x) * 2;
     const int x = blockIdx.y * 4 + threadIdx.y;
     const int b = blockIdx.z;
     const size_t plane = (size_t)H * W;
+    constexpr bool PK8 = SMX_PROLOGUE_PK8(MODE);
     bool bad = false, bad8 = false;
     if (x < h && yp < w) {
         const int Y0 = yp * 2;
@@ -158,22 +184,25 @@
             float *dn = (side ? down_r : down_l) + ((size_t)b * h + x) * w + yp;
             dn[0] = pooled[0];
             if (ncol == 4) dn[1] = pooled[1];
+            const float s4[2] = {pooled[0] * 4.0f, pooled[1] * 4.0f};
 #pragma unroll
             for (int k = 0; k < 2; ++k) {
-                if (k == 0 || ncol == 4) {
-                    const float s4 = pooled[k] * 4.0f;
-                    bad = bad || !(s4 == rintf(s4) && pooled[k] >= 0.0f && pooled[k] <= 255.0f);
-                }
-            }
+                if (k == 0 || ncol == 4) bad = bad || !(s4[k] == rintf(s4[k]) && pooled[k] >= 0.0f && pooled[k] <= 255.0f);
+            }
+            const uint32_t upk = (uint32_t)(unsigned short)s4[0] | ((uint32_t)(unsigned short)s4[1] << 16);
             if (pitch8 > 0) {
                 uint8_t *g8 = (side ? g8_r : g8_l);
                 uint32_t w0 = 0u, w1 = 0u;
 #pragma unroll
                 for (int j = 0; j < 4; ++j) {
-                    if (j < ncol) {
-                        if (MODE == IN_GRAY_F32)
-                            bad8 = bad8 || !(v0[j] == rintf(v0[j]) && v0[j] >= 0.f && v0[j] <= 255.f) ||
-                                   (row1_in && !(v1[j] == rintf(v1[j]) && v1[j] >= 0.f && v1[j] <= 255.f));
+                    if (MODE == IN_GRAY_F32 && !PK8 && j < ncol)
+                        bad8 = bad8 || !(v0[j] == rintf(v0[j]) && v0[j] >= 0.f && v0[j] <= 255.f) ||
+                               (row1_in && !(v1[j] == rintf(v1[j]) && v1[j] >= 0.f && v1[j] <= 255.f));
+                    if (PK8) {
+                        w0 = __builtin_amdgcn_cvt_pk_u8_f32(v0[j], j, w0);
+                        w1 = __builtin_amdgcn_cvt_pk_u8_f32(v1[j], j, w1);
+                        bad8 |= ((float)((w0 >> (8 * j)) & 0xffu) != v0[j]) | ((float)((w1 >> (8 * j)) & 0xffu) != v1[j]);
+                    } else if (j < ncol) {
                         w0 |= (uint32_t)(uint8_t)v0[j] << (8 * j);
                         w1 |= (uint32_t)(uint8_t)v1[j] << (8 * j);
                     }
@@ -198,6 +227,16 @@
                     }
                 }
             }
+            if (units_l != nullptr) {
+                uint16_t *uplane = (side ? units_r : units_l) + (size_t)b * h * upitch;
+                const unsigned urow = (unsigned)x * (unsigned)upitch;
+                if (ncol == 4) *(uint32_t *)((char *)uplane + (size_t)(2u * (urow + (unsigned)yp))) = upk;
+                else store_unit_u16(uplane, urow + (unsigned)yp, (uint16_t)upk);
+                if (yp < 3) {
+                    store_unit_apron(uplane, urow, w, yp, (uint16_t)upk);
+                    if (ncol == 4) store_unit_apron(uplane, urow, w, yp + 1, (uint16_t)(upk >> 16));
+                }
+            }
         }
     }
     const unsigned long long m = __ballot(bad);
@@ -215,7 +254,8 @@
                                                      uint8_t *g8_l, uint8_t *g8_r, int *flags2,
                                                      int H, int W, int h, int w,
                                                      int pitch8, int padl, int padr, int epoch,
-                                                     int gpitch, int gpadl, int fp_conv) {
+                                                     int gpitch, int gpadl, int fp_conv,
+                                                     uint16_t *units_l, uint16_t *units_r, int upitch) {
     constexpr bool RGB = MODE == IN_RGB_F32 || MODE == IN_RGB_U8;
     constexpr bool U8 = MODE == IN_GRAY_U8 || MODE == IN_RGB_U8;
     const int y = blockIdx.x * 64 + threadIdx.x;
@@ -223,6 +263,7 @@
     const int b = blockIdx.z;
     const size_t plane = (size_t)H * W;
     const size_t pair_elems = RGB ? 3 * plane : plane;
+    constexpr bool PK8 = SMX_PROLOGUE_PK8(MODE);
     bool bad = false, bad8 = false;
     if (x < h && y < w) {
         const int Y0 = y * 4;
@@ -289,6 +330,11 @@
             (side ? down_r : down_l)[((size_t)b * h + x) * w + y] = pooled;
             const float s16 = pooled * 16.0f;
             bad = bad || !(s16 == rintf(s16) && pooled >= 0.0f && pooled <= 255.0f);
+            if (units_l != nullptr) {
+                uint16_t *uplane = (side ? units_r : units_l) + (size_t)b * h * upitch;
+                store_unit_u16(uplane, (unsigned)(x * upitch + y), (unsigned short)s16);
+                store_unit_apron(uplane, (unsigned)(x * upitch), w, y, (unsigned short)s16);
+            }
             if (!RGB && pitch8 > 0) {
                 uint8_t *g8 = (side ? g8_r : g8_l);
 #pragma unroll
@@ -297,8 +343,13 @@
                     uint32_t wd = 0u;
 #pragma unroll
                     for (int j = 0; j < 4; ++j) {
-                        if (MODE == IN_GRAY_F32) bad8 = bad8 || !(v[i][j] == rintf(v[i][j]) && v[i][j] >= 0.f && v[i][j] <= 255.f);
-                        wd |= (uint32_t)(uint8_t)v[i][j] << (8 * j);
+                        if (MODE == IN_GRAY_F32 && !PK8) bad8 = bad8 || !(v[i][j] == rintf(v[i][j]) && v[i][j] >= 0.f && v[i][j] <= 255.f);
+                        if (PK8) {
+                            wd = __builtin_amdgcn_cvt_pk_u8_f32(v[i][j], j, wd);
+                            bad8 |= (float)((wd >> (8 * j)) & 0xffu) != v[i][j];
+                        } else {
+                            wd |= (uint32_t)(uint8_t)v[i][j] << (8 * j);
+                        }
                     }
                     uint8_t *r8 = g8 + ((size_t)b * H + x * 4 + i) * pitch8;
                     *(uint32_t *)(r8 + padl + Y0) = wd;
diff --git a/stereo-depth_amd/csrc/smx_common.h b/stereo-depth_amd/csrc/smx_common.h
--- a/stereo-depth_amd/csrc/smx_common.h
+++ b/stereo-depth_amd/csrc/smx_common.h
@@ -11,6 +11,8 @@
     g %= n;
     return g < 0 ? g + n : g;
 }
+
+__host__ __device__ constexpr int unit_plane_pitch(int w) { return (w + 3 + 3) & ~3; }
 
 __device__ __forceinline__ int pad_index_ref(int index, int n) {
     if (index >= 0 && index < n) return index;
@@ -144,6 +146,8 @@
 
 struct MatchParams {
     const float *Ld, *Rd;
+    const unsigned short *Lu, *Ru;
+    int upitch;
     float *wta;
     float *costs;
     float *vol;
diff --git a/stereo-depth_amd/csrc/smx_engine.hip b/stereo-depth_amd/csrc/smx_engine.hip
--- a/stereo-depth_amd/csrc/smx_engine.hip
+++ b/stereo-depth_amd/csrc/smx_engine.hip
@@ -67,6 +67,7 @@
     smx::EngineFacts facts;
     float *gray_l = nullptr, *gray_r = nullptr;
     float *down_l = nullptr, *down_r = nullptr;
+    uint16_t *units_l = nullptr, *units_r = nullptr;
     float *wta = nullptr, *refined = nullptr;
     float *costs = nullptr;
     float *vol = nullptr;
@@ -126,7 +127,7 @@
 void free_buffers(smx_engine *e) {
     void *ptrs[] = {e->gray_l, e->gray_r, e->down_l, e->down_r, e->wta,     e->refined,  e->costs,
                     e->vol,    e->flags,  e->gray8_l, e->gray8_r, e->slices, e->cand,    e->stats_dev, e->tickets, e->fast_stats_dev,
-                    e->lr_in_l, e->lr_in_r, e->lr_raw};
+                    e->lr_in_l, e->lr_in_r, e->lr_raw, e->units_l, e->units_r};
     for (void *p : ptrs)
         if (p) (void)hipFree(p);
     if (e->hints) (void)hipHostFree(e->hints);
@@ -175,6 +176,7 @@
     float *gray_l, *gray_r, *down_l, *down_r, *wta, *refined, *costs, *vol;
     int *flags, *flags2;
     uint8_t *gray8_l, *gray8_r;
+    uint16_t *units_l, *units_r;
     unsigned *cand;
 };
 PairView view_from(const smx_engine *e, int first) {
@@ -186,6 +188,8 @@
     v.gray_r = e->gray_r + f * d.H * ef.gpitch;
     v.down_l = e->down_l + f * hw;
     v.down_r = e->down_r + f * hw;
+    v.units_l = e->units_l + f * d.h * ef.upitch;
+    v.units_r = e->units_r + f * d.h * ef.upitch;
     v.wta = e->wta + f * hw;
     v.refined = e->refined + f * hw;
     v.costs = e->costs + f * hw;
@@ -229,7 +233,7 @@
     const smx::EngineFacts &f = e->facts;
     smx::PrologueArgs a{};
     a.left = left; a.right = right; a.gray_l = owns_gray ? v.gray_l : nullptr; a.gray_r = owns_gray ? v.gray_r : nullptr;
-    a.down_l = v.down_l; a.down_r = v.down_r;
+    a.down_l = v.down_l; a.down_r = v.down_r; a.units_l = v.units_l; a.units_r = v.units_r; a.upitch = f.upitch;
     a.flags = v.flags; a.flags2 = v.flags2; a.g8_l = v.gray8_l; a.g8_r = v.gray8_r;
     a.H = d.H; a.W = d.W; a.K = d.K; a.h = d.h; a.w = d.w; a.grid_capable = f.grid_capable ? 1 : 0;
     a.pitch8 = f.pitch8; a.padl = f.padl; a.padr = f.padr; a.epoch = e->epoch; a.gpitch = f.gpitch; a.gpadl = f.gpadl;
@@ -241,7 +245,7 @@
     const smx::EngineFacts &f = e->facts;
     smx::RangeParams b;
     smx::MatchParams &mp = b.mp;
-    mp.Ld = v.down_l; mp.Rd = v.down_r; mp.wta = v.wta; mp.costs = v.costs; mp.vol = v.vol;
+    mp.Ld = v.down_l; mp.Rd = v.down_r; mp.Lu = v.units_l; mp.Ru = v.units_r; mp.upitch = f.upitch; mp.wta = v.wta; mp.costs = v.costs; mp.vol = v.vol;
     mp.flags = v.flags; mp.epoch = e->epoch; mp.B = e->B; mp.h = d.h; mp.w = d.w; mp.dmin = d.dmin; mp.Dd = d.Dd;
     mp.rn = (int)e->cfg.ncc_patch_radius; mp.rs = e->cfg.small_mbm_radius;
     mp.rm = e->cfg.mid_mbm_radius; mp.rl = e->cfg.large_mbm_radius;
@@ -314,7 +318,9 @@
     const GrayView g = gray_view(e, v, pl.owns_gray, first, left, right);
     {
         SlotTimer tm(e, s, lane, SMX_KERNEL_PROLOGUE);
-        smx::launch_prologue(pl.prologue, prologue_args(e, v, pl.owns_gray, left, right), n, s);
+        smx::PrologueArgs pa = prologue_args(e, v, pl.owns_gray, left, right);
+        if (!pl.writes_units) pa.units_l = pa.units_r = nullptr;
+        smx::launch_prologue(pl.prologue, pa, n, s);
     }
     if (pl.status != SMX_OK) return fail(pl.status, "%s", pl.refusal);
     if (pl.exact.slice_floats > f.slices_floats)
@@ -727,6 +733,8 @@
     alloc((void **)&e->gray_r, B * (size_t)d.H * f.gpitch * sizeof(float));
     alloc((void **)&e->down_l, B * hw * sizeof(float));
     alloc((void **)&e->down_r, B * hw * sizeof(float));
+    alloc((void **)&e->units_l, B * (size_t)d.h * f.upitch * sizeof(uint16_t));
+    alloc((void **)&e->units_r, B * (size_t)d.h * f.upitch * sizeof(uint16_t));
     alloc((void **)&e->wta, B * hw * sizeof(float));
     alloc((void **)&e->refined, B * hw * sizeof(float));
     alloc((void **)&e->costs, 3 * B * hw * sizeof(float));
diff --git a/stereo-depth_amd/csrc/smx_launch.h b/stereo-depth_amd/csrc/smx_launch.h
--- a/stereo-depth_amd/csrc/smx_launch.h
+++ b/stereo-depth_amd/csrc/smx_launch.h
@@ -15,7 +15,8 @@
     float *gray_l, *gray_r, *down_l, *down_r;
     int *flags, *flags2;
     uint8_t *g8_l, *g8_r;
-    int H, W, K, h, w, grid_capable, pitch8, padl, padr, epoch, gpitch, gpadl;
+    uint16_t *units_l, *units_r;
+    int H, W, K, h, w, grid_capable, pitch8, padl, padr, epoch, gpitch, gpadl, upitch;
     int fp_conv;
 };
 void launch_prologue(const PrologueLaunch &x, const PrologueArgs &a, int n, hipStream_t s);
diff --git a/stereo-depth_amd/csrc/smx_plan.h b/stereo-depth_amd/csrc/smx_plan.h
--- a/stereo-depth_amd/csrc/smx_plan.h
+++ b/stereo-depth_amd/csrc/smx_plan.h
@@ -37,6 +37,7 @@
     int kt = 0;
     int pitch8 = 0, padl = 0, padr = 0;
     int gpitch = 0, gpadl = 0;
+    int upitch = 0;
     bool prologue_k2 = false;
     bool prologue_k4 = false;
     bool sad_exact = true;
@@ -92,6 +93,7 @@
             f.gpadl = 0;
         }
     }
+    f.upitch = unit_plane_pitch(d.w);
     f.prologue_k2 = K == 2 && (d.W & 1) == 0;
     f.prologue_k4 = K == 4 && (d.W & 3) == 0 && f.grid_capable && (f.gpitch & 3) == 0 && (f.gpadl & 3) == 0 && (f.pitch8 & 3) == 0 &&
                     (f.padl & 3) == 0 && (f.gpadl == 0 || f.gpadl == f.padl);
@@ -143,6 +145,7 @@
     bool gated_dense_first = false;
     bool exact_split = false;
     bool capture_follows = false;
+    bool writes_units = false;
     FastPlan fast{};
     bool dense = false, dense_small = false;
     bool reports = false;
@@ -367,6 +370,7 @@
         p.refine.kind = REFINE_AUTO_V;
     }
     p.fill = fill_launch(f, call.on_lanes, n);
+    p.writes_units = p.route != AGG_EXACT && p.route != AGG_FILTERED;
     return p;
 }
 
diff --git a/stereo-depth_amd/csrc/tu_stages.hip b/stereo-depth_amd/csrc/tu_stages.hip
--- a/stereo-depth_amd/csrc/tu_stages.hip
+++ b/stereo-depth_amd/csrc/tu_stages.hip
@@ -18,18 +18,18 @@
             constexpr int M2 = (MODE == IN_GRAY_U8) ? IN_GRAY_U8 : IN_GRAY_F32;
             hipLaunchKernelGGL((k_prologue_k2<M2>), dim3((a.w + 127) / 128, grid.y, n), block, 0, s, a.left, a.right, a.gray_l, a.gray_r,
                                a.down_l, a.down_r, a.flags, a.g8_l, a.g8_r, a.flags2, a.H, a.W, a.h, a.w,
-                               a.pitch8, a.padl, a.padr, a.epoch, a.gpitch, a.gpadl);
+                               a.pitch8, a.padl, a.padr, a.epoch, a.gpitch, a.gpadl, a.units_l, a.units_r, a.upitch);
             return;
         }
         case PROLOGUE_K4:
             hipLaunchKernelGGL((k_prologue_k4<MODE>), grid, block, 0, s, a.left, a.right, a.gray_l, a.gray_r, a.down_l,
                                a.down_r, a.flags, a.g8_l, a.g8_r, a.flags2, a.H, a.W, a.h, a.w,
-                               a.pitch8, a.padl, a.padr, a.epoch, a.gpitch, a.gpadl, a.fp_conv);
+                               a.pitch8, a.padl, a.padr, a.epoch, a.gpitch, a.gpadl, a.fp_conv, a.units_l, a.units_r, a.upitch);
             return;
         default:
             hipLaunchKernelGGL((k_prologue<MODE>), grid, block, 0, s, a.left, a.right, a.gray_l, a.gray_r, a.down_l,
                                a.down_r, a.flags, a.g8_l, a.g8_r, a.flags2, a.H, a.W, a.K, a.h, a.w,
-                               a.grid_capable, a.pitch8, a.padl, a.padr, a.epoch, a.gpitch, a.gpadl, a.fp_conv);
+                               a.grid_capable, a.pitch8, a.padl, a.padr, a.epoch, a.gpitch, a.gpadl, a.fp_conv, a.units_l, a.units_r, a.upitch);
     }
 }
 }
```

Measured after the change: 103,700 (median of 6 runs). 1.8% higher.
